# uthree/tinyvc

Measured on AMD Instinct MI355X. Metric: audio-samples/sec (16 kHz) end-to-end VC, higher is better.
Workload: dtype f32 (fp32 in / out / accumulate; channel contractions as two-term fp16 splits on v_mfma_f32_32x32x16_f16: 22-bit significands, three part-products per fp32 product)

## Files before the change

### include/tinyvc_hip.h

```cpp
#ifndef TINYVC_HIP_H
#define TINYVC_HIP_H

#include <stddef.h>
#include <stdint.h>

#ifdef __cplusplus
extern "C" {
#endif

typedef struct tvc_ctx tvc_ctx;

enum tvc_status {
    TVC_OK = 0,
    TVC_ERR_ARG = -1,
    TVC_ERR_HIP = -2,
    TVC_ERR_STATE = -3,
    TVC_ERR_WORKSPACE = -4
};

#define TVC_ABI_VERSION 1
int tvc_version(void);

int tvc_ctx_create(int hip_device, tvc_ctx** out);
void tvc_ctx_destroy(tvc_ctx* ctx);
const char* tvc_last_error(const tvc_ctx* ctx);

int tvc_load_tensor(tvc_ctx* ctx, const char* state_dict_key, const float* host_data,
                    const int64_t* shape, int ndim);
int tvc_set_pitch_table(tvc_ctx* ctx, const float* host_freqs, int n);
int tvc_finalize_weights(tvc_ctx* ctx);

int tvc_workspace_bytes(tvc_ctx* ctx, int B, int64_t L, int64_t N, size_t* out_bytes);

int tvc_stft_mag_f32(tvc_ctx* ctx, void* stream, const float* wav, float* spec, int B, int64_t L,
                     void* ws, size_t ws_bytes);
int tvc_energy_f32(tvc_ctx* ctx, void* stream, const float* wav, float* energy, int B, int64_t L,
                   void* ws, size_t ws_bytes);

int64_t tvc_resample_out_len(int64_t n, int orig_freq, int new_freq);
int tvc_resample_f32(tvc_ctx* ctx, void* stream, const float* x, float* y, int rows, int64_t n, int orig_freq,
                     int new_freq);
int tvc_pcm16_to_f32(tvc_ctx* ctx, void* stream, const int16_t* pcm, float* y, int64_t n, float gain_db);
int tvc_f32_to_pcm16(tvc_ctx* ctx, void* stream, const float* x, int16_t* pcm, int64_t n, float gain_db);

int tvc_encoder_f32(tvc_ctx* ctx, void* stream, const float* spec, float* ssl, float* f0,
                    float* logits, int B, int T, void* ws, size_t ws_bytes);

int tvc_pitch_decode_f32(tvc_ctx* ctx, void* stream, const float* logits, float* f0, int B, int T);

int64_t tvc_knn_prepared_elems(int64_t N);
int tvc_knn_prepare_index_f32(tvc_ctx* ctx, void* stream, const float* index, float* prepared,
                              int64_t N);
int64_t tvc_knn_prepared_elems_f16(int64_t N);
int tvc_knn_prepare_index_f16(tvc_ctx* ctx, void* stream, const void* rows_f16, float* prepared,
                              int64_t N);
int tvc_knn_prepare_index_cols_f32(tvc_ctx* ctx, void* stream, const float* feats, int64_t S, const int64_t* cols, int64_t N,
                                   float* prepared, float* index_out);
int tvc_knn_prepare_index_cols_f16(tvc_ctx* ctx, void* stream, const float* feats, int64_t S, const int64_t* cols, int64_t N,
                                   float* prepared, void* index_out_f16);

int tvc_knn_forget(tvc_ctx* ctx, const float* prepared);
int tvc_knn_match_f32(tvc_ctx* ctx, void* stream, const float* src, const float* prepared, int64_t N,
                      float* out, int64_t* idx_out, int B, int T, void* ws, size_t ws_bytes);

int tvc_knn_match_general_f32(tvc_ctx* ctx, void* stream, const float* src, const float* index, int64_t N, int k, int metric,
                              float* out, int64_t* idx_out, float* sim_out, int B, int T, void* ws, size_t ws_bytes);

int tvc_ctx_set_index_assign_chunk(tvc_ctx* ctx, int max_queries);
int tvc_workspace_bytes_index_compact(tvc_ctx* ctx, int64_t N, int64_t K, size_t* out_bytes);
int tvc_index_assign_f32(tvc_ctx* ctx, void* stream, const float* points_prepared, int64_t N, const float* centroids_prepared, int64_t K,
                         int64_t* assign_inout, float* sim_out, int32_t* moved_out, void* ws, size_t ws_bytes);
int tvc_index_update_f32(tvc_ctx* ctx, void* stream, const float* points_prepared, int64_t N, const int64_t* assign, int64_t K,
                         float* centroids_inout, int32_t* counts_out, void* ws, size_t ws_bytes);
int tvc_index_compact_f32(tvc_ctx* ctx, void* stream, const float* points_prepared, int64_t N, const int64_t* init_cols, int64_t K, int iters,
                          float* centroids_out, float* prepared_out, int64_t* assign_out, int32_t* counts_out, int32_t* moved_out, void* ws,
                          size_t ws_bytes);

int tvc_knn_topk_f32(tvc_ctx* ctx, void* stream, const float* src, const float* prepared, int64_t N,
                     float* sims_out, int64_t* idx_out, int B, int T, void* ws, size_t ws_bytes);
int tvc_knn_gather_slots_f32(tvc_ctx* ctx, void* stream, const float* prepared, int64_t N,
                             const int64_t* idx, float* slots, int64_t nslots);
int tvc_knn_finish_f32(tvc_ctx* ctx, void* stream, const float* slots, float* out, int B, int T);

int tvc_shift_frequency_f32(tvc_ctx* ctx, void* stream, const float* f0, float* out, int64_t n,
                            float semitones);

int tvc_noise_angle_from_uniform_f32(tvc_ctx* ctx, void* stream, float* u, int64_t n);

int tvc_decoder_f32(tvc_ctx* ctx, void* stream, const float* content, const float* f0,
                    const float* energy, const float* noise_angle, uint64_t seed, float* wave,
                    int B, int T, void* ws, size_t ws_bytes);
int tvc_decoder_stages_f32(tvc_ctx* ctx, void* stream, const float* content, const float* f0,
                           const float* energy, const float* noise_angle, uint64_t seed,
                           float* wave, float* amps, float* kernel, float* source, int B, int T,
                           void* ws, size_t ws_bytes);

int tvc_filter_net_f32(tvc_ctx* ctx, void* stream, const float* content, const float* f0, const float* energy,
                       const float* source, float* wave, float* const* skips, float* const* ups, int B, int T,
                       void* ws, size_t ws_bytes);

int tvc_dsp_f32(tvc_ctx* ctx, void* stream, const float* f0, const float* amps, const float* kernel,
                const float* noise_angle, uint64_t seed, float* source, int B, int T, void* ws,
                size_t ws_bytes);

int tvc_convert_f32(tvc_ctx* ctx, void* stream, const float* wav, const float* prepared_index,
                    int64_t N, float pitch_shift, const float* noise_angle, uint64_t seed,
                    float* wave, int B, int64_t L, void* ws, size_t ws_bytes);

int tvc_workspace_bytes_ragged(tvc_ctx* ctx, int B, int64_t Lmax, const int64_t* lens, int64_t N, size_t* out_bytes);
int tvc_ragged_plan(int B, int64_t Lmax, const int64_t* lens, int max_frames, int32_t* batch_of_row, int* n_batches);
int tvc_ctx_set_ragged_batch_frames(tvc_ctx* ctx, int max_frames);
int tvc_convert_ragged_f32(tvc_ctx* ctx, void* stream, const float* wav, int64_t Lmax, const int64_t* lens, const float* prepared_index,
                           int64_t N, float pitch_shift, const float* noise_angle, uint64_t seed, float* wave, int B, void* ws,
                           size_t ws_bytes);

int tvc_workspace_bytes_encode_ragged(tvc_ctx* ctx, int B, int64_t Lmax, const int64_t* lens, size_t* out_bytes);
int tvc_encode_ragged_f32(tvc_ctx* ctx, void* stream, const float* wav, int64_t Lmax, const int64_t* lens, float* ssl, float* f0,
                          int B, void* ws, size_t ws_bytes);

int tvc_knn_match_multi_f32(tvc_ctx* ctx, void* stream, const float* src, const float* const* prepared, const int64_t* N,
                            float* out, int64_t* idx_out, int B, int T, void* ws, size_t ws_bytes);
int tvc_workspace_bytes_multi(tvc_ctx* ctx, int B, int64_t L, const int64_t* N, size_t* out_bytes);
int tvc_convert_multi_f32(tvc_ctx* ctx, void* stream, const float* wav, const float* const* prepared, const int64_t* N,
                          float pitch_shift, const float* pitch_shifts, const float* noise_angle, uint64_t seed, float* wave,
                          int B, int64_t L, void* ws, size_t ws_bytes);
int tvc_workspace_bytes_ragged_multi(tvc_ctx* ctx, int B, int64_t Lmax, const int64_t* lens, const int64_t* N, size_t* out_bytes);
int tvc_convert_ragged_multi_f32(tvc_ctx* ctx, void* stream, const float* wav, int64_t Lmax, const int64_t* lens,
                                 const float* const* prepared, const int64_t* N, float pitch_shift, const float* pitch_shifts,
                                 const float* noise_angle, uint64_t seed, float* wave, int B, void* ws, size_t ws_bytes);

#define TVC_BLEND_MAX 4
int tvc_knn_match_blend_f32(tvc_ctx* ctx, void* stream, const float* src, const float* const* prepared, const int64_t* N, int M,
                            const float* weights, float* out, int64_t* idx_out, int B, int T, void* ws, size_t ws_bytes);
int tvc_workspace_bytes_blend(tvc_ctx* ctx, int B, int64_t L, const int64_t* N, int M, size_t* out_bytes);
int tvc_convert_blend_f32(tvc_ctx* ctx, void* stream, const float* wav, const float* const* prepared, const int64_t* N, int M,
                          const float* weights, float pitch_shift, const float* pitch_shifts, const float* noise_angle, uint64_t seed,
                          float* wave, int B, int64_t L, void* ws, size_t ws_bytes);
int tvc_workspace_bytes_ragged_blend(tvc_ctx* ctx, int B, int64_t Lmax, const int64_t* lens, const int64_t* N, int M, size_t* out_bytes);
int tvc_convert_ragged_blend_f32(tvc_ctx* ctx, void* stream, const float* wav, int64_t Lmax, const int64_t* lens,
                                 const float* const* prepared, const int64_t* N, int M, const float* weights, float pitch_shift,
                                 const float* pitch_shifts, const float* noise_angle, uint64_t seed, float* wave, int B, void* ws,
                                 size_t ws_bytes);

int tvc_pitch_match_f32(tvc_ctx* ctx, void* stream, const float* f0, const int64_t* row_start, int rows, const float* target_f0,
                        float pitch_shift, const float* pitch_shifts, float* median_out, int32_t* voiced_out, float* shift_out,
                        float* f0_shifted);
int tvc_workspace_bytes_auto(tvc_ctx* ctx, int B, int64_t L, const int64_t* N, int M, size_t* out_bytes);
int tvc_convert_auto_f32(tvc_ctx* ctx, void* stream, const float* wav, const float* const* prepared, const int64_t* N, int M,
                         const float* weights, const float* target_f0, float pitch_shift, const float* pitch_shifts, float* shift_out,
                         const float* noise_angle, uint64_t seed, float* wave, int B, int64_t L, void* ws, size_t ws_bytes);
int tvc_workspace_bytes_ragged_auto(tvc_ctx* ctx, int B, int64_t Lmax, const int64_t* lens, const int64_t* N, int M, size_t* out_bytes);
int tvc_convert_ragged_auto_f32(tvc_ctx* ctx, void* stream, const float* wav, int64_t Lmax, const int64_t* lens,
                                const float* const* prepared, const int64_t* N, int M, const float* weights, const float* target_f0,
                                float pitch_shift, const float* pitch_shifts, float* shift_out, const float* noise_angle, uint64_t seed,
                                float* wave, int B, void* ws, size_t ws_bytes);

int tvc_sola_f32(tvc_ctx* ctx, void* stream, const float* y, float* sola_buf, const float* fade_in,
                 float* out, int32_t* shift_out, int S, int64_t Ly, int block,
                 int use_phase_vocoder);

int tvc_stream_push_f32(tvc_ctx* ctx, void* stream, float* buf, const float* blocks, int S, int64_t n, int block);

int tvc_profile_enable(tvc_ctx* ctx, int on);
int tvc_profile_read(tvc_ctx* ctx, char* buf, size_t buf_bytes);

#ifdef __cplusplus
}
#endif
#endif
```

### tinyvc_amd/_lib.py

```python
import ctypes
import os
from ctypes import POINTER, c_char_p, c_float, c_int, c_int32, c_int64, c_size_t, c_uint64, c_void_p

_HERE = os.path.dirname(os.path.abspath(__file__))
LIB_PATH = os.environ.get("TVC_LIB_PATH") or os.path.join(_HERE, "libtinyvc_hip.so")

_lib = None

SIGNATURES = {
    "tvc_version": (c_int, []),
    "tvc_ctx_create": (c_int, [c_int, POINTER(c_void_p)]),
    "tvc_ctx_destroy": (None, [c_void_p]),
    "tvc_last_error": (c_char_p, [c_void_p]),
    "tvc_load_tensor": (c_int, [c_void_p, c_char_p, c_void_p, POINTER(c_int64), c_int]),
    "tvc_set_pitch_table": (c_int, [c_void_p, c_void_p, c_int]),
    "tvc_finalize_weights": (c_int, [c_void_p]),
    "tvc_workspace_bytes": (c_int, [c_void_p, c_int, c_int64, c_int64, POINTER(c_size_t)]),
    "tvc_stft_mag_f32": (c_int, [c_void_p, c_void_p, c_void_p, c_void_p, c_int, c_int64, c_void_p, c_size_t]),
    "tvc_energy_f32": (c_int, [c_void_p, c_void_p, c_void_p, c_void_p, c_int, c_int64, c_void_p, c_size_t]),
    "tvc_resample_out_len": (c_int64, [c_int64, c_int, c_int]),
    "tvc_resample_f32": (c_int, [c_void_p, c_void_p, c_void_p, c_void_p, c_int, c_int64, c_int, c_int]),
    "tvc_pcm16_to_f32": (c_int, [c_void_p, c_void_p, c_void_p, c_void_p, c_int64, c_float]),
    "tvc_f32_to_pcm16": (c_int, [c_void_p, c_void_p, c_void_p, c_void_p, c_int64, c_float]),
    "tvc_encoder_f32": (c_int, [c_void_p, c_void_p, c_void_p, c_void_p, c_void_p, c_void_p, c_int, c_int, c_void_p, c_size_t]),
    "tvc_pitch_decode_f32": (c_int, [c_void_p, c_void_p, c_void_p, c_void_p, c_int, c_int]),
    "tvc_knn_prepared_elems": (c_int64, [c_int64]),
    "tvc_knn_prepared_elems_f16": (c_int64, [c_int64]),
    "tvc_knn_prepare_index_f16": (c_int, [c_void_p, c_void_p, c_void_p, c_void_p, c_int64]),
    "tvc_knn_prepare_index_cols_f32": (c_int, [c_void_p, c_void_p, c_void_p, c_int64, c_void_p, c_int64, c_void_p, c_void_p]),
    "tvc_knn_prepare_index_cols_f16": (c_int, [c_void_p, c_void_p, c_void_p, c_int64, c_void_p, c_int64, c_void_p, c_void_p]),
    "tvc_knn_forget": (c_int, [c_void_p, c_void_p]),
    "tvc_ragged_plan": (c_int, [c_int, c_int64, POINTER(c_int64), c_int, POINTER(c_int32), POINTER(c_int)]),
    "tvc_ctx_set_ragged_batch_frames": (c_int, [c_void_p, c_int]),
    "tvc_knn_prepare_index_f32": (c_int, [c_void_p, c_void_p, c_void_p, c_void_p, c_int64]),
    "tvc_knn_match_f32": (c_int, [c_void_p, c_void_p, c_void_p, c_void_p, c_int64, c_void_p, c_void_p, c_int, c_int, c_void_p, c_size_t]),
    "tvc_knn_match_general_f32": (c_int, [c_void_p, c_void_p, c_void_p, c_void_p, c_int64, c_int, c_int, c_void_p, c_void_p, c_void_p, c_int, c_int, c_void_p, c_size_t]),
    "tvc_knn_topk_f32": (c_int, [c_void_p, c_void_p, c_void_p, c_void_p, c_int64, c_void_p, c_void_p, c_int, c_int, c_void_p, c_size_t]),
    "tvc_knn_gather_slots_f32": (c_int, [c_void_p, c_void_p, c_void_p, c_int64, c_void_p, c_void_p, c_int64]),
    "tvc_knn_finish_f32": (c_int, [c_void_p, c_void_p, c_void_p, c_void_p, c_int, c_int]),
    "tvc_shift_frequency_f32": (c_int, [c_void_p, c_void_p, c_void_p, c_void_p, c_int64, c_float]),
    "tvc_noise_angle_from_uniform_f32": (c_int, [c_void_p, c_void_p, c_void_p, c_int64]),
    "tvc_decoder_f32": (c_int, [c_void_p, c_void_p, c_void_p, c_void_p, c_void_p, c_void_p, c_uint64, c_void_p, c_int, c_int, c_void_p, c_size_t]),
    "tvc_decoder_stages_f32": (c_int, [c_void_p, c_void_p, c_void_p, c_void_p, c_void_p, c_void_p, c_uint64, c_void_p, c_void_p, c_void_p, c_void_p, c_int, c_int, c_void_p, c_size_t]),
    "tvc_filter_net_f32": (c_int, [c_void_p, c_void_p, c_void_p, c_void_p, c_void_p, c_void_p, c_void_p, POINTER(c_void_p), POINTER(c_void_p), c_int, c_int, c_void_p, c_size_t]),
    "tvc_dsp_f32": (c_int, [c_void_p, c_void_p, c_void_p, c_void_p, c_void_p, c_void_p, c_uint64, c_void_p, c_int, c_int, c_void_p, c_size_t]),
    "tvc_convert_f32": (c_int, [c_void_p, c_void_p, c_void_p, c_void_p, c_int64, c_float, c_void_p, c_uint64, c_void_p, c_int, c_int64, c_void_p, c_size_t]),
    "tvc_workspace_bytes_ragged": (c_int, [c_void_p, c_int, c_int64, POINTER(c_int64), c_int64, POINTER(c_size_t)]),
    "tvc_convert_ragged_f32": (c_int, [c_void_p, c_void_p, c_void_p, c_int64, POINTER(c_int64), c_void_p, c_int64, c_float, c_void_p, c_uint64, c_void_p, c_int, c_void_p, c_size_t]),
    "tvc_workspace_bytes_encode_ragged": (c_int, [c_void_p, c_int, c_int64, POINTER(c_int64), POINTER(c_size_t)]),
    "tvc_encode_ragged_f32": (c_int, [c_void_p, c_void_p, c_void_p, c_int64, POINTER(c_int64), c_void_p, c_void_p, c_int, c_void_p, c_size_t]),
    "tvc_knn_match_multi_f32": (c_int, [c_void_p, c_void_p, c_void_p, POINTER(c_void_p), POINTER(c_int64), c_void_p, c_void_p, c_int, c_int, c_void_p, c_size_t]),
    "tvc_workspace_bytes_multi": (c_int, [c_void_p, c_int, c_int64, POINTER(c_int64), POINTER(c_size_t)]),
    "tvc_convert_multi_f32": (c_int, [c_void_p, c_void_p, c_void_p, POINTER(c_void_p), POINTER(c_int64), c_float, POINTER(c_float), c_void_p, c_uint64,
                                      c_void_p, c_int, c_int64, c_void_p, c_size_t]),
    "tvc_workspace_bytes_ragged_multi": (c_int, [c_void_p, c_int, c_int64, POINTER(c_int64), POINTER(c_int64), POINTER(c_size_t)]),
    "tvc_convert_ragged_multi_f32": (c_int, [c_void_p, c_void_p, c_void_p, c_int64, POINTER(c_int64), POINTER(c_void_p), POINTER(c_int64), c_float,
                                             POINTER(c_float), c_void_p, c_uint64, c_void_p, c_int, c_void_p, c_size_t]),
    "tvc_knn_match_blend_f32": (c_int, [c_void_p, c_void_p, c_void_p, POINTER(c_void_p), POINTER(c_int64), c_int, c_void_p, c_void_p, c_void_p, c_int, c_int,
                                        c_void_p, c_size_t]),
    "tvc_workspace_bytes_blend": (c_int, [c_void_p, c_int, c_int64, POINTER(c_int64), c_int, POINTER(c_size_t)]),
    "tvc_convert_blend_f32": (c_int, [c_void_p, c_void_p, c_void_p, POINTER(c_void_p), POINTER(c_int64), c_int, c_void_p, c_float, POINTER(c_float), c_void_p,
                                      c_uint64, c_void_p, c_int, c_int64, c_void_p, c_size_t]),
    "tvc_workspace_bytes_ragged_blend": (c_int, [c_void_p, c_int, c_int64, POINTER(c_int64), POINTER(c_int64), c_int, POINTER(c_size_t)]),
    "tvc_convert_ragged_blend_f32": (c_int, [c_void_p, c_void_p, c_void_p, c_int64, POINTER(c_int64), POINTER(c_void_p), POINTER(c_int64), c_int, c_void_p,
                                             c_float, POINTER(c_float), c_void_p, c_uint64, c_void_p, c_int, c_void_p, c_size_t]),
    "tvc_pitch_match_f32": (c_int, [c_void_p, c_void_p, c_void_p, POINTER(c_int64), c_int, c_void_p, c_float, POINTER(c_float), c_void_p, c_void_p, c_void_p,
                                    c_void_p]),
    "tvc_workspace_bytes_auto": (c_int, [c_void_p, c_int, c_int64, POINTER(c_int64), c_int, POINTER(c_size_t)]),
    "tvc_convert_auto_f32": (c_int, [c_void_p, c_void_p, c_void_p, POINTER(c_void_p), POINTER(c_int64), c_int, c_void_p, c_void_p, c_float, POINTER(c_float),
                                     c_void_p, c_void_p, c_uint64, c_void_p, c_int, c_int64, c_void_p, c_size_t]),
    "tvc_workspace_bytes_ragged_auto": (c_int, [c_void_p, c_int, c_int64, POINTER(c_int64), POINTER(c_int64), c_int, POINTER(c_size_t)]),
    "tvc_convert_ragged_auto_f32": (c_int, [c_void_p, c_void_p, c_void_p, c_int64, POINTER(c_int64), POINTER(c_void_p), POINTER(c_int64), c_int, c_void_p,
                                            c_void_p, c_float, POINTER(c_float), c_void_p, c_void_p, c_uint64, c_void_p, c_int, c_void_p, c_size_t]),
    "tvc_ctx_set_index_assign_chunk": (c_int, [c_void_p, c_int]),
    "tvc_workspace_bytes_index_compact": (c_int, [c_void_p, c_int64, c_int64, POINTER(c_size_t)]),
    "tvc_index_assign_f32": (c_int, [c_void_p, c_void_p, c_void_p, c_int64, c_void_p, c_int64, c_void_p, c_void_p, c_void_p, c_void_p, c_size_t]),
    "tvc_index_update_f32": (c_int, [c_void_p, c_void_p, c_void_p, c_int64, c_void_p, c_int64, c_void_p, c_void_p, c_void_p, c_size_t]),
    "tvc_index_compact_f32": (c_int, [c_void_p, c_void_p, c_void_p, c_int64, c_void_p, c_int64, c_int, c_void_p, c_void_p, c_void_p, c_void_p, c_void_p,
                                      c_void_p, c_size_t]),
    "tvc_sola_f32": (c_int, [c_void_p, c_void_p, c_void_p, c_void_p, c_void_p, c_void_p, c_void_p, c_int, c_int64, c_int, c_int]),
    "tvc_stream_push_f32": (c_int, [c_void_p, c_void_p, c_void_p, c_void_p, c_int, c_int64, c_int]),
    "tvc_profile_enable": (c_int, [c_void_p, c_int]),
    "tvc_profile_read": (c_int, [c_void_p, ctypes.c_char_p, c_size_t]),
}


class TinyVCError(RuntimeError):
    pass


def load_library():
    global _lib
    if _lib is not None:
        return _lib
    import torch
    if not os.path.exists(LIB_PATH):
        raise TinyVCError(
            f"{LIB_PATH} is missing: build it with `python -m tinyvc_amd.build` (needs hipcc). "
            "tinyvc_amd has no CPU or eager-PyTorch fallback.")
    lib = ctypes.CDLL(LIB_PATH)
    for name, (res, args) in SIGNATURES.items():
        fn = getattr(lib, name)
        fn.restype = res
        fn.argtypes = args
    _lib = lib
    return lib
```

### tinyvc_amd/csrc/api.hip

```cpp
#include <atomic>
#include <cmath>
#include <mutex>

#include <cstdlib>

#include "knn_blob.h"
#include "tvc_common.h"

using namespace tvc;

static std::mutex g_blob_mu;
static std::map<const void*, int64_t> g_blobs;
constexpr size_t kMaxBlobRecords = 4096;
static void blob_record(const void* p, int64_t N) {
    std::lock_guard<std::mutex> lk(g_blob_mu);
    if (g_blobs.size() >= kMaxBlobRecords && !g_blobs.count(p)) g_blobs.clear();
    g_blobs[p] = N;
}
static void blob_forget(const void* p) {
    std::lock_guard<std::mutex> lk(g_blob_mu);
    g_blobs.erase(p);
}
static int blob_check(tvc_ctx* ctx, hipStream_t s, const void* p, int64_t N, const char* what) {
    {
// ... 562 lines not shown
    return convert_query(ctx, B, Lmax, lens, true, ConvertIndex::one(nullptr, N), out_bytes, "tvc_workspace_bytes_ragged");
}
int tvc_workspace_bytes_multi(tvc_ctx* ctx, int B, int64_t L, const int64_t* N, size_t* out_bytes) {
    return convert_query(ctx, B, L, nullptr, false, ConvertIndex::table(nullptr, N), out_bytes, "tvc_workspace_bytes_multi");
}
int tvc_workspace_bytes_ragged_multi(tvc_ctx* ctx, int B, int64_t Lmax, const int64_t* lens, const int64_t* N, size_t* out_bytes) {
    return convert_query(ctx, B, Lmax, lens, true, ConvertIndex::table(nullptr, N), out_bytes, "tvc_workspace_bytes_ragged_multi");
}

int tvc_convert_f32(tvc_ctx* ctx, void* stream, const float* wav, const float* prepared, int64_t N,
                    float pitch_shift, const float* noise_angle, uint64_t seed, float* wave, int B, int64_t L,
                    void* wsp, size_t ws_bytes) {
    const ConvertCall c{wav, wave, B, L, nullptr, ConvertIndex::one(prepared, N), pitch_shift, nullptr, noise_angle, seed};
    return convert_entry(ctx, stream, c, false, wsp, ws_bytes, "tvc_convert_f32");
}
int tvc_convert_ragged_f32(tvc_ctx* ctx, void* stream, const float* wav, int64_t Lmax, const int64_t* lens, const float* prepared, int64_t N,
                           float pitch_shift, const float* noise_angle, uint64_t seed, float* wave, int B, void* wsp, size_t ws_bytes) {
    const ConvertCall c{wav, wave, B, Lmax, lens, ConvertIndex::one(prepared, N), pitch_shift, nullptr, noise_angle, seed};
    return convert_entry(ctx, stream, c, true, wsp, ws_bytes, "tvc_convert_ragged_f32");
}
int tvc_convert_multi_f32(tvc_ctx* ctx, void* stream, const float* wav, const float* const* prepared, const int64_t* N, float pitch_shift,
                          const float* pitch_shifts, const float* noise_angle, uint64_t seed, float* wave, int B, int64_t L, void* wsp, size_t ws_bytes) {
    const ConvertCall c{wav, wave, B, L, nullptr, ConvertIndex::table(prepared, N), pitch_shift, pitch_shifts, noise_angle, seed};
    return convert_entry(ctx, stream, c, false, wsp, ws_bytes, "tvc_convert_multi_f32");
}
int tvc_convert_ragged_multi_f32(tvc_ctx* ctx, void* stream, const float* wav, int64_t Lmax, const int64_t* lens, const float* const* prepared,
                                 const int64_t* N, float pitch_shift, const float* pitch_shifts, const float* noise_angle, uint64_t seed, float* wave,
                                 int B, void* wsp, size_t ws_bytes) {
    const ConvertCall c{wav, wave, B, Lmax, lens, ConvertIndex::table(prepared, N), pitch_shift, pitch_shifts, noise_angle, seed};
    return convert_entry(ctx, stream, c, true, wsp, ws_bytes, "tvc_convert_ragged_multi_f32");
}

int tvc_knn_match_multi_f32(tvc_ctx* ctx, void* stream, const float* src, const float* const* prepared, const int64_t* N, float* out,
                            int64_t* idx_out, int B, int T, void* wsp, size_t ws_bytes) {
    if (!ctx) return TVC_ERR_ARG;
    if (!src || !out || B <= 0 || T <= 0 || (int64_t)B * T > 0x7fffffff) return fail(ctx, TVC_ERR_ARG, "tvc_knn_match_multi_f32: bad argument");
    hipStream_t s = (hipStream_t)stream;
    TVC_CHECK(rows_check(ctx, s, B, prepared, N, "tvc_knn_match_multi_f32"));
    TVC_HIP(ctx, hipSetDevice(ctx->device));
    std::vector<KnnSegIn> in((size_t)B);
    for (int b = 0; b < B; ++b) in[b] = KnnSegIn{prepared[b], N[b], b * T, T};
    return run_walks(ctx, __func__, wsp, ws_bytes, 1, [&](Ws& ws) { return run_knn_segs(ctx, s, ws, src, in.data(), B, out, idx_out, B, T); });
}

int tvc_workspace_bytes_blend(tvc_ctx* ctx, int B, int64_t L, const int64_t* N, int M, size_t* out_bytes) {
    if (!ctx) return TVC_ERR_ARG;
    TVC_CHECK(blend_check(ctx, B, M, kDryPtr, "tvc_workspace_bytes_blend"));
    return convert_query(ctx, B, L, nullptr, false, ConvertIndex::blend(nullptr, N, M, nullptr), out_bytes, "tvc_workspace_bytes_blend");
}
int tvc_workspace_bytes_ragged_blend(tvc_ctx* ctx, int B, int64_t Lmax, const int64_t* lens, const int64_t* N, int M, size_t* out_bytes) {
    if (!ctx) return TVC_ERR_ARG;
    TVC_CHECK(blend_check(ctx, B, M, kDryPtr, "tvc_workspace_bytes_ragged_blend"));
    return convert_query(ctx, B, Lmax, lens, true, ConvertIndex::blend(nullptr, N, M, nullptr), out_bytes, "tvc_workspace_bytes_ragged_blend");
}
int tvc_convert_blend_f32(tvc_ctx* ctx, void* stream, const float* wav, const float* const* prepared, const int64_t* N, int M, const float* weights,
                          float pitch_shift, const float* pitch_shifts, const float* noise_angle, uint64_t seed, float* wave, int B, int64_t L, void* wsp,
                          size_t ws_bytes) {
    if (!ctx) return TVC_ERR_ARG;
    TVC_CHECK(blend_check(ctx, B, M, weights, "tvc_convert_blend_f32"));
    const ConvertCall c{wav, wave, B, L, nullptr, ConvertIndex::blend(prepared, N, M, weights), pitch_shift, pitch_shifts, noise_angle, seed};
    return convert_entry(ctx, stream, c, false, wsp, ws_bytes, "tvc_convert_blend_f32");
}
int tvc_convert_ragged_blend_f32(tvc_ctx* ctx, void* stream, const float* wav, int64_t Lmax, const int64_t* lens, const float* const* prepared,
                                 const int64_t* N, int M, const float* weights, float pitch_shift, const float* pitch_shifts, const float* noise_angle,
                                 uint64_t seed, float* wave, int B, void* wsp, size_t ws_bytes) {
    if (!ctx) return TVC_ERR_ARG;
    TVC_CHECK(blend_check(ctx, B, M, weights, "tvc_convert_ragged_blend_f32"));
    const ConvertCall c{wav, wave, B, Lmax, lens, ConvertIndex::blend(prepared, N, M, weights), pitch_shift, pitch_shifts, noise_angle, seed};
    return convert_entry(ctx, stream, c, true, wsp, ws_bytes, "tvc_convert_ragged_blend_f32");
}

int tvc_pitch_match_f32(tvc_ctx* ctx, void* stream, const float* f0, const int64_t* row_start, int rows, const float* target_f0, float pitch_shift,
                        const float* pitch_shifts, float* median_out, int32_t* voiced_out, float* shift_out, float* f0_shifted) {
    if (!ctx) return TVC_ERR_ARG;
    if (!f0 || !row_start || rows <= 0 || (!median_out && !voiced_out && !shift_out && !f0_shifted)) return fail(ctx, TVC_ERR_ARG, "tvc_pitch_match_f32: bad argument");
    if (row_start[0] < 0 || row_start[rows] > 0x7fffffff) return fail(ctx, TVC_ERR_ARG, "tvc_pitch_match_f32: row_start beyond 32-bit indexing");
    std::vector<PitchRow> pr((size_t)rows);
    for (int b = 0; b < rows; ++b) {
        if (row_start[b + 1] < row_start[b]) return fail(ctx, TVC_ERR_ARG, "tvc_pitch_match_f32: row_start[%d] > row_start[%d] (rows + 1 ascending column numbers)", b, b + 1);
        pr[b] = PitchRow{(int)row_start[b], (int)(row_start[b + 1] - row_start[b]), b, pitch_shifts ? pitch_shifts[b] : pitch_shift};
    }
    TVC_HIP(ctx, hipSetDevice(ctx->device));
    return run_pitch_match(ctx, (hipStream_t)stream, f0, pr, target_f0, median_out, voiced_out, shift_out, f0_shifted);
}

static int auto_index(tvc_ctx* ctx, int B, const float* const* prepared, const int64_t* N, int M, const float* weights, ConvertIndex* ix, const char* what) {
    if (!ctx) return TVC_ERR_ARG;
    if (!weights) {
        if (M != 1) return fail(ctx, TVC_ERR_ARG, "%s: weights = NULL is one index per row: M must be 1, got %d", what, M);
        *ix = ConvertIndex::table(prepared, N);
        return 0;
    }
    TVC_CHECK(blend_check(ctx, B, M, weights, what));
    *ix = ConvertIndex::blend(prepared, N, M, weights);
    return 0;
}
static int auto_query(tvc_ctx* ctx, int B, int64_t L, const int64_t* lens, bool ragged, const int64_t* N, int M, size_t* out_bytes, const char* what) {
    if (!ctx) return TVC_ERR_ARG;
    TVC_CHECK(blend_check(ctx, B, M, kDryPtr, what));
    TVC_CHECK(convert_query(ctx, B, L, lens, ragged, ConvertIndex::blend(nullptr, N, M, nullptr), out_bytes, what, true));
    if (M == 1) {
        size_t table = 0;
        TVC_CHECK(convert_query(ctx, B, L, lens, ragged, ConvertIndex::table(nullptr, N), &table, what, true));
        if (table > *out_bytes) *out_bytes = table;
    }
    return TVC_OK;
}
int tvc_workspace_bytes_auto(tvc_ctx* ctx, int B, int64_t L, const int64_t* N, int M, size_t* out_bytes) {
    return auto_query(ctx, B, L, nullptr, false, N, M, out_bytes, "tvc_workspace_bytes_auto");
}
int tvc_workspace_bytes_ragged_auto(tvc_ctx* ctx, int B, int64_t Lmax, const int64_t* lens, const int64_t* N, int M, size_t* out_bytes) {
    return auto_query(ctx, B, Lmax, lens, true, N, M, out_bytes, "tvc_workspace_bytes_ragged_auto");
}
int tvc_convert_auto_f32(tvc_ctx* ctx, void* stream, const float* wav, const float* const* prepared, const int64_t* N, int M, const float* weights,
                         const float* target_f0, float pitch_shift, const float* pitch_shifts, float* shift_out, const float* noise_angle, uint64_t seed,
                         float* wave, int B, int64_t L, void* wsp, size_t ws_bytes) {
    ConvertIndex ix;
    TVC_CHECK(auto_index(ctx, B, prepared, N, M, weights, &ix, "tvc_convert_auto_f32"));
    if (!target_f0) return fail(ctx, TVC_ERR_ARG, "tvc_convert_auto_f32: target_f0 is NULL (a device array of B registers in Hz)");
    const ConvertCall c{wav, wave, B, L, nullptr, ix, pitch_shift, pitch_shifts, noise_angle, seed, target_f0, shift_out};
    return convert_entry(ctx, stream, c, false, wsp, ws_bytes, "tvc_convert_auto_f32");
}
int tvc_convert_ragged_auto_f32(tvc_ctx* ctx, void* stream, const float* wav, int64_t Lmax, const int64_t* lens, const float* const* prepared,
                                const int64_t* N, int M, const float* weights, const float* target_f0, float pitch_shift, const float* pitch_shifts,
                                float* shift_out, const float* noise_angle, uint64_t seed, float* wave, int B, void* wsp, size_t ws_bytes) {
    ConvertIndex ix;
    TVC_CHECK(auto_index(ctx, B, prepared, N, M, weights, &ix, "tvc_convert_ragged_auto_f32"));
    if (!target_f0) return fail(ctx, TVC_ERR_ARG, "tvc_convert_ragged_auto_f32: target_f0 is NULL (a device array of B registers in Hz)");
    const ConvertCall c{wav, wave, B, Lmax, lens, ix, pitch_shift, pitch_shifts, noise_angle, seed, target_f0, shift_out};
    return convert_entry(ctx, stream, c, true, wsp, ws_bytes, "tvc_convert_ragged_auto_f32");
}

int tvc_knn_match_blend_f32(tvc_ctx* ctx, void* stream, const float* src, const float* const* prepared, const int64_t* N, int M, const float* weights,
                            float* out, int64_t* idx_out, int B, int T, void* wsp, size_t ws_bytes) {
    if (!ctx) return TVC_ERR_ARG;
    if (!src || !out || B <= 0 || T <= 0) return fail(ctx, TVC_ERR_ARG, "tvc_knn_match_blend_f32: bad argument");
    TVC_CHECK(blend_check(ctx, B, M, weights, "tvc_knn_match_blend_f32"));
    if ((int64_t)B * M * T > 0x7fffffff) return fail(ctx, TVC_ERR_ARG, "tvc_knn_match_blend_f32: more than 2^31 - 1 query columns");
    hipStream_t s = (hipStream_t)stream;
    TVC_CHECK(rows_check(ctx, s, B * M, prepared, N, "tvc_knn_match_blend_f32"));
    TVC_HIP(ctx, hipSetDevice(ctx->device));
    std::vector<KnnSegIn> in;
    for (int m = 0; m < M; ++m)
        for (int b = 0; b < B; ++b) in.push_back(KnnSegIn{prepared[(size_t)b * M + m], N[(size_t)b * M + m], (m * B + b) * T, T});
    return run_walks(ctx, __func__, wsp, ws_bytes, 1, [&](Ws& ws) { return run_knn_blend(ctx, s, ws, src, in.data(), (int)in.size(), M, weights, out, idx_out, B, T); });
}

int tvc_ctx_set_ragged_batch_frames(tvc_ctx* ctx, int max_frames) {
    if (!ctx) return TVC_ERR_ARG;
    if (max_frames < 0) return fail(ctx, TVC_ERR_ARG, "tvc_ctx_set_ragged_batch_frames: the cap is a frame count (0 = the default)");
    ctx->rag_batch_frames = max_frames;
    return TVC_OK;
}
int tvc_ragged_plan(int B, int64_t Lmax, const int64_t* lens, int max_frames, int32_t* batch_of_row, int* n_batches) {
    if (!lens || !batch_of_row || !n_batches || B <= 0 || Lmax <= 0 || Lmax % kHop != 0 || max_frames < 0) return TVC_ERR_ARG;
    std::vector<RagBatchPlan> batches;
    const int rc = ragged_split(nullptr, max_frames, B, Lmax, lens, &batches);
    if (rc) return rc;
    for (size_t i = 0; i < batches.size(); ++i)
        for (int b : batches[i].rows) batch_of_row[b] = (int32_t)i;
    *n_batches = (int)batches.size();
    return TVC_OK;
}

int tvc_workspace_bytes_encode_ragged(tvc_ctx* ctx, int B, int64_t Lmax, const int64_t* lens, size_t* out_bytes) {
    TVC_CHECK(need_ready(ctx, NEED_NONE));
    if (!out_bytes || !lens || B <= 0 || Lmax <= 0 || Lmax % kHop != 0) return fail(ctx, TVC_ERR_ARG, "tvc_workspace_bytes_encode_ragged: need B>0, Lmax%%480==0, lens[B]");
    std::vector<RagBatchPlan> batches;
    std::vector<int> gpre;
    int64_t S = 0;
    TVC_CHECK(encode_ragged_plan(ctx, B, Lmax, lens, &batches, &gpre, &S));
    return measure(kRagGranule, out_bytes, [&](Ws& ws) { return encode_ragged_batches(ctx, nullptr, ws, batches, gpre, kDryPtr, Lmax, kDryPtr, kDryPtr, S); });
}

int tvc_encode_ragged_f32(tvc_ctx* ctx, void* stream, const float* wav, int64_t Lmax, const int64_t* lens, float* ssl, float* f0, int B, void* wsp,
                          size_t ws_bytes) {
    TVC_CHECK(need_ready(ctx, NEED_ENC));
    if (!wav || !lens || !ssl || !f0 || B <= 0 || Lmax <= 0 || Lmax % kHop) return fail(ctx, TVC_ERR_ARG, "tvc_encode_ragged_f32: bad argument (Lmax must be a positive multiple of 480)");
    TVC_HIP(ctx, hipSetDevice(ctx->device));
    hipStream_t s = (hipStream_t)stream;
    std::vector<RagBatchPlan> batches;
    std::vector<int> gpre;
    int64_t S = 0;
    TVC_CHECK(encode_ragged_plan(ctx, B, Lmax, lens, &batches, &gpre, &S));
    return run_walks(ctx, __func__, wsp, ws_bytes, kRagGranule, [&](Ws& ws) { return encode_ragged_batches(ctx, s, ws, batches, gpre, wav, Lmax, ssl, f0, S); });
}

static int compact_check(tvc_ctx* ctx, int64_t N, int64_t K, const char* what) {
    if (K < 4 || K > N) return fail(ctx, TVC_ERR_ARG, "%s: need 4 <= K <= N (K = %lld, N = %lld)", what, (long long)K, (long long)N);
    if (K > kIndexCompactMaxK) return fail(ctx, TVC_ERR_ARG, "%s: K = %lld is above the limit of %lld centroids", what, (long long)K, (long long)kIndexCompactMaxK);
    if (N > 0x7fffff00L) return fail(ctx, TVC_ERR_ARG, "%s: N beyond 32-bit indexing", what);
    return 0;
}

int tvc_ctx_set_index_assign_chunk(tvc_ctx* ctx, int max_queries) {
    if (!ctx) return TVC_ERR_ARG;
    if (max_queries < 0) return fail(ctx, TVC_ERR_ARG, "tvc_ctx_set_index_assign_chunk: the chunk is a count of query columns (0 = the default)");
    ctx->index_assign_chunk = max_queries;
    return TVC_OK;
}

int tvc_workspace_bytes_index_compact(tvc_ctx* ctx, int64_t N, int64_t K, size_t* out_bytes) {
    if (!ctx) return TVC_ERR_ARG;
    if (!out_bytes) return fail(ctx, TVC_ERR_ARG, "tvc_workspace_bytes_index_compact: out_bytes is NULL");
    TVC_CHECK(compact_check(ctx, N, K, "tvc_workspace_bytes_index_compact"));
    return measure(1, out_bytes, [&](Ws& ws) { return run_index_compact(ctx, nullptr, ws, kDryPtr, N, nullptr, K, 1, kDryPtr, kDryPtr, nullptr, nullptr, nullptr); });
}

int tvc_index_assign_f32(tvc_ctx* ctx, void* stream, const float* points_prepared, int64_t N, const float* centroids_prepared, int64_t K,
                         int64_t* assign_inout, float* sim_out, int32_t* moved_out, void* wsp, size_t ws_bytes) {
    if (!ctx) return TVC_ERR_ARG;
    if (!points_prepared || !centroids_prepared || !assign_inout) return fail(ctx, TVC_ERR_ARG, "tvc_index_assign_f32: bad argument");
    TVC_CHECK(compact_check(ctx, N, K, "tvc_index_assign_f32"));
    hipStream_t s = (hipStream_t)stream;
    TVC_CHECK(blob_check(ctx, s, points_prepared, N, "tvc_index_assign_f32 (points)"));
    TVC_CHECK(blob_check(ctx, s, centroids_prepared, K, "tvc_index_assign_f32 (centroids)"));
    TVC_HIP(ctx, hipSetDevice(ctx->device));
    return run_walks(ctx, __func__, wsp, ws_bytes, 1, [&](Ws& ws) { return run_index_assign(ctx, s, ws, points_prepared, N, centroids_prepared, K, assign_inout, sim_out, moved_out); });
}

int tvc_index_update_f32(tvc_ctx* ctx, void* stream, const float* points_prepared, int64_t N, const int64_t* assign, int64_t K, float* centroids_inout,
                         int32_t* counts_out, void* wsp, size_t ws_bytes) {
    if (!ctx) return TVC_ERR_ARG;
    if (!points_prepared || !assign || !centroids_inout) return fail(ctx, TVC_ERR_ARG, "tvc_index_update_f32: bad argument");
    TVC_CHECK(compact_check(ctx, N, K, "tvc_index_update_f32"));
    hipStream_t s = (hipStream_t)stream;
    TVC_CHECK(blob_check(ctx, s, points_prepared, N, "tvc_index_update_f32"));
    TVC_HIP(ctx, hipSetDevice(ctx->device));
    return run_walks(ctx, __func__, wsp, ws_bytes, 1, [&](Ws& ws) { return run_index_update(ctx, s, ws, points_prepared, N, assign, K, centroids_inout, counts_out); });
}

int tvc_index_compact_f32(tvc_ctx* ctx, void* stream, const float* points_prepared, int64_t N, const int64_t* init_cols, int64_t K, int iters,
                          float* centroids_out, float* prepared_out, int64_t* assign_out, int32_t* counts_out, int32_t* moved_out, void* wsp, size_t ws_bytes) {
    if (!ctx) return TVC_ERR_ARG;
    if (!points_prepared || !init_cols || !centroids_out || !prepared_out || iters < 1) return fail(ctx, TVC_ERR_ARG, "tvc_index_compact_f32: bad argument (iters >= 1)");
    TVC_CHECK(compact_check(ctx, N, K, "tvc_index_compact_f32"));
    hipStream_t s = (hipStream_t)stream;
    TVC_CHECK(blob_check(ctx, s, points_prepared, N, "tvc_index_compact_f32"));
    TVC_HIP(ctx, hipSetDevice(ctx->device));
    blob_forget(prepared_out);
    TVC_CHECK(run_walks(ctx, __func__, wsp, ws_bytes, 1, [&](Ws& ws) {
        return run_index_compact(ctx, s, ws, points_prepared, N, init_cols, K, iters, centroids_out, prepared_out, assign_out, counts_out, moved_out);
    }));
    blob_record(prepared_out, K);
    return TVC_OK;
}

int tvc_profile_enable(tvc_ctx* ctx, int on) {
    if (!ctx) return TVC_ERR_ARG;
    ctx->profiling = on < 0 ? 0 : (on > 2 ? 1 : on);
    return TVC_OK;
}

int tvc_profile_read(tvc_ctx* ctx, char* buf, size_t buf_bytes) {
    if (!ctx || !buf || buf_bytes < 2) return TVC_ERR_ARG;
    std::vector<std::pair<std::string, double>> agg;
    for (auto& r : ctx->regions) {
        float ms = 0.f;
        if (r.a && r.b && hipEventSynchronize(r.b) == hipSuccess && hipEventElapsedTime(&ms, r.a, r.b) == hipSuccess) {
            bool found = false;
            for (auto& a : agg)
                if (a.first == r.name) {
                    a.second += ms;
                    found = true;
                }
            if (!found) agg.push_back({r.name, ms});
        }
        if (r.a) ctx->event_pool.push_back(r.a);
        if (r.b) ctx->event_pool.push_back(r.b);
    }
    ctx->regions.clear();
    std::string out;
    for (auto& a : agg) {
        char tmp[160];
        snprintf(tmp, sizeof(tmp), "%s=%.6f;", a.first.c_str(), a.second);
        out += tmp;
    }
    snprintf(buf, buf_bytes, "%s", out.c_str());
    return TVC_OK;
}

int tvc_sola_f32(tvc_ctx* ctx, void* stream, const float* y, float* sola_buf, const float* fade_in, float* out,
                 int32_t* shift_out, int S, int64_t Ly, int block, int use_phase_vocoder) {
    if (!ctx) return TVC_ERR_ARG;
    if (!y || !sola_buf || !fade_in || !out || S <= 0 || block <= 0 || Ly < block + kSolaCross + kSolaSearch + kSolaDelay)
        return fail(ctx, TVC_ERR_ARG, "tvc_sola_f32: bad argument (Ly must cover block+1920+1920+3840)");
    TVC_HIP(ctx, hipSetDevice(ctx->device));
    return run_sola(ctx, (hipStream_t)stream, y, sola_buf, fade_in, out, shift_out, S, Ly, block, use_phase_vocoder);
}

int tvc_stream_push_f32(tvc_ctx* ctx, void* stream, float* buf, const float* blocks, int S, int64_t n, int block) {
    if (!ctx) return TVC_ERR_ARG;
    if (!buf || !blocks || S <= 0 || block <= 0 || n < block || n > INT32_MAX - 32768)
        return fail(ctx, TVC_ERR_ARG, "tvc_stream_push_f32: bad argument (block <= n <= 2^31 - 32769)");
    TVC_HIP(ctx, hipSetDevice(ctx->device));
    return run_stream_push(ctx, (hipStream_t)stream, buf, blocks, S, (int)n, block);
}

}
```

### tinyvc_amd/csrc/cnx_s3.h

```cpp
#pragma once
#include "gemm_epi.h"
#include "split_fp16.h"

namespace tvc {

struct CnxArgs {
    float* x;
    float* h;
    int T, rs;
    RagDev rg;
    const uint4* A6;
    const float* wsc;
    const float* bias;
    int MT, mt_per_wg;
    const float *dw_w, *dw_b, *ln_g, *ln_b;
    int dil;
    float* gp;
    int gp_tiles;
    int gp_sum;
    const float* grn_g;
    float* amax_y;
};

constexpr int CNX_GP_INLINE = 16;
constexpr int CNX_PD = 4;
typedef float f32x4s_t __attribute__((ext_vector_type(4)));

struct CnxNoPost {
    __device__ __forceinline__ void operator()(int) const {}
};
template <int NT, int NC, int KSL, class Post = CnxNoPost>
__device__ __forceinline__ void cnx_mma(f32x16 (&hi)[NT], f32x16 (&lo)[NT], u32x4 (&ring)[CNX_PD][2], const uint4* __restrict__ A6, int MT, int mt, int k_begin,
                                        int mt_next, int k_next, const uint4* Ys, int lane, const Post& post = Post()) {
    static_assert(KSL % CNX_PD == 0, "ring depth divides the K walk");
    const int l31 = lane & 31, lh = lane >> 5;
    const uint4* yb = Ys + lh * NC + l31;
    u32x4 bq[2][NT][2];
#pragma unroll
    for (int j = 0; j < NT; ++j)
#pragma unroll
        for (int p = 0; p < 2; ++p) bq[0][j][p] = *reinterpret_cast<const u32x4*>(yb + (p * 2) * NC + j * 32);
#pragma unroll
    for (int k0 = 0; k0 < KSL; k0 += CNX_PD) {
#pragma unroll
        for (int u = 0; u < CNX_PD; ++u) {
            const int k = k0 + u, fb = u & 1;
            const f16x8 a0 = __builtin_bit_cast(f16x8, ring[u][0]), a1 = __builtin_bit_cast(f16x8, ring[u][1]);
            int kn = k + CNX_PD, mtl = mt, kg = k_begin;
            if (kn >= KSL) {
                kn -= KSL;
                mtl = mt_next;
                kg = k_next;
            }
            const uint4* ab = A6 + ((long)(kg + kn) * MT + mtl) * kPU4;
            ring[u][0] = ldg_so4(ab, 16u * (unsigned)lane);
            ring[u][1] = ldg_so4(ab, 16u * (unsigned)(64 + lane));
            const int kb = k + 1 < KSL ? k + 1 : 0;
#pragma unroll
            for (int j = 0; j < NT; ++j)
#pragma unroll
                for (int p = 0; p < 2; ++p) bq[fb ^ 1][j][p] = *reinterpret_cast<const u32x4*>(yb + ((kb * 2 + p) * 2) * NC + j * 32);
#pragma unroll
            for (int j = 0; j < NT; ++j) lo[j] = TVC_MFMA16(a1, __builtin_bit_cast(f16x8, bq[fb][j][0]), lo[j]);
#pragma unroll
            for (int j = 0; j < NT; ++j) hi[j] = TVC_MFMA16(a0, __builtin_bit_cast(f16x8, bq[fb][j][0]), hi[j]);
#pragma unroll
            for (int j = 0; j < NT; ++j) lo[j] = TVC_MFMA16(a0, __builtin_bit_cast(f16x8, bq[fb][j][1]), lo[j]);
            post(k);
            __builtin_amdgcn_sched_barrier(0);
        }
    }
}

template <int C, int NT>
struct Cnx1 {
    static constexpr int WAVES = 8, NTHR = WAVES * 64, NC = 32 * NT, KS = C / 16, CPT = C / 16, VW = NT;
    static constexpr int YS_U4 = KS * 4 * NC;
    static constexpr int LDS_BYTES = YS_U4 * 16 + (C * 8 + 2 * C + 16 * NC) * 4;
    static_assert(LDS_BYTES <= 160 * 1024, "LDS");
};

template <int C, int NT>
__global__ __launch_bounds__((Cnx1<C, NT>::NTHR)) void cnx1_kernel(CnxArgs a) {
    using CF = Cnx1<C, NT>;
    constexpr int NC = CF::NC, KS = CF::KS, CPT = CF::CPT, VW = CF::VW, WAVES = CF::WAVES, NTHR = CF::NTHR;
    extern __shared__ __attribute__((aligned(16))) uint4 smem_c1[];
    uint4* Ys = smem_c1;
    float* scr = reinterpret_cast<float*>(smem_c1);
    float* Wl = reinterpret_cast<float*>(smem_c1 + CF::YS_U4);
    float* Gl = Wl + C * 8;
    float* red = Gl + 2 * C;
    const int tid = threadIdx.x, lane = tid & 63, l31 = lane & 31, lh = lane >> 5;
    const int wave = __builtin_amdgcn_readfirstlane(tid >> 6);
    const int b = blockIdx.y;
    int Tb = a.T;
    long xoff = (long)b * C * a.T, hoff = (long)b * 2 * C * a.T;
    if (a.rg.tb) {
        Tb = a.rg.tb[b];
        xoff = hoff = a.rg.pre[b];
    }
    const int ntu = (Tb + NC - 1) / NC;
    if ((int)blockIdx.x >= ntu) return;
    const int TW = (Tb + ntu - 1) / ntu;
    const int t0 = blockIdx.x * TW;
    const int tw = Tb - t0 < TW ? Tb - t0 : TW;
    const int rs = a.rs;
    const float* xb = a.x + xoff;

    for (int i = tid; i < C; i += NTHR) {
#pragma unroll
        for (int j = 0; j < 7; ++j) Wl[i * 8 + j] = a.dw_w[i * 7 + j];
        Wl[i * 8 + 7] = a.dw_b[i];
        Gl[i] = a.ln_g[i];
        Gl[C + i] = a.ln_b[i];
    }
    __syncthreads();

    const int col = NT == 2 ? lane : l31;
    const int tc = t0 + (col < tw ? col : tw - 1);
    unsigned tt[7];
#pragma unroll
    for (int j = 0; j < 7; ++j) {
        int q = tc + (j - 3) * a.dil;
        q = q < 0 ? 0 : (q >= Tb ? Tb - 1 : q);
        tt[j] = 4u * (unsigned)q;
    }
    float v[VW][CPT];
#pragma unroll
    for (int u = 0; u < VW; ++u) {
        const int vw = NT == 2 ? wave + 8 * u : wave + 8 * lh;
        float sum = 0.f;
#pragma unroll
        for (int i = 0; i < CPT; ++i) {
            const int c = vw + i * 16;
            const f32x4s_t w0 = *reinterpret_cast<const f32x4s_t*>(Wl + c * 8), w1 = *reinterpret_cast<const f32x4s_t*>(Wl + c * 8 + 4);
            const float wj[7] = {w0[0], w0[1], w0[2], w0[3], w1[0], w1[1], w1[2]};
            float acc = w1[3];
            if (NT == 2) {
                const float* xr = xb + (long)c * rs;
#pragma unroll
                for (int j = 0; j < 7; ++j) acc = fmaf(wj[j], ldg_so(xr, tt[j]), acc);
            } else {
                const char* xr = reinterpret_cast<const char*>(xb + (long)c * rs);
#pragma unroll
                for (int j = 0; j < 7; ++j) acc = fmaf(wj[j], *reinterpret_cast<const float*>(xr + tt[j]), acc);
            }
            v[u][i] = acc;
            sum += acc;
            scr[c * NC + col] = acc;
        }
        red[vw * NC + col] = sum;
    }
    __syncthreads();
    float tot = 0.f;
#pragma unroll
    for (int w = 0; w < 16; ++w) tot += red[w * NC + col];
    const float mean = tot / (float)C;
    __syncthreads();
#pragma unroll
    for (int u = 0; u < VW; ++u) {
        const int vw = NT == 2 ? wave + 8 * u : wave + 8 * lh;
        float sq = 0.f;
#pragma unroll
        for (int i = 0; i < CPT; ++i) {
            const float d = v[u][i] - mean;
            sq = fmaf(d, d, sq);
        }
        red[vw * NC + col] = sq;
    }
    __syncthreads();
    float tot2 = 0.f;
#pragma unroll
    for (int w = 0; w < 16; ++w) tot2 += red[w * NC + col];
    const float var = tot2 / (float)C;
    const float rstd = 1.f / sqrtf(var + 1e-5f);

    for (int i = wave; i < KS; i += WAVES) {
        constexpr int NQ = NT == 2 ? 16 : 8;
        const int c0 = 16 * i + (NT == 2 ? 0 : 8 * lh);
        float y[NQ];
#pragma unroll
        for (int q = 0; q < NQ; ++q) y[q] = scr[(c0 + q) * NC + col];
#pragma unroll
        for (int q = 0; q < NQ; ++q) y[q] = fmaf((y[q] - mean) * rstd, Gl[c0 + q], Gl[C + c0 + q]);
#pragma unroll
        for (int hh = 0; hh < NQ / 8; ++hh) {
            const float y8[8] = {y[8 * hh], y[8 * hh + 1], y[8 * hh + 2], y[8 * hh + 3], y[8 * hh + 4], y[8 * hh + 5], y[8 * hh + 6], y[8 * hh + 7]};
            uint4 p1, p2;
            split8(y8, p1, p2);
            const int half = NT == 2 ? hh : lh;
            Ys[((i * 2 + 0) * 2 + half) * NC + col] = p1;
            Ys[((i * 2 + 1) * 2 + half) * NC + col] = p2;
        }
    }
    __syncthreads();

    const int mt_lo = blockIdx.z * a.mt_per_wg;
    const int mt_hi = mt_lo + a.mt_per_wg < a.MT ? mt_lo + a.mt_per_wg : a.MT;
    int mt = mt_lo + wave;
    if (mt >= mt_hi) return;
    u32x4 ring[CNX_PD][2];
#pragma unroll
    for (int u = 0; u < CNX_PD; ++u) {
        const uint4* ab = a.A6 + ((long)u * a.MT + mt) * kPU4;
        ring[u][0] = ldg_so4(ab, 16u * (unsigned)lane);
        ring[u][1] = ldg_so4(ab, 16u * (unsigned)(64 + lane));
    }
    float* hb = a.h + hoff;
    constexpr int NPEND = NT * 16, EPS = ((NPEND + KS - 1) / KS + 1) / 2 * 2;
    float pend[NPEND];
    int pmt = mt;
    unsigned oo[NT];
#pragma unroll
    for (int j = 0; j < NT; ++j) {
        const int n = j * 32 + l31;
        oo[j] = 4u * (unsigned)(4 * lh * rs + t0 + (n < tw ? n : tw - 1));
    }
    bool live[NT];
#pragma unroll
    for (int j = 0; j < NT; ++j) live[j] = j * 32 + l31 < tw;
    float sq[16];
    float* gpb = a.gp + ((long)b * a.gp_tiles + blockIdx.x) * (2 * C) + ((l31 >> 1) & 3) + 8 * (l31 >> 3) + 4 * lh;
    auto finish2 = [&](int e) __attribute__((always_inline)) {
        const int j = e >> 4;
        f32x2e v = {pend[e], pend[e + 1]};
        asm volatile("" : "+v"(v));
        const f32x2e o = gelu_pair(v);
#pragma unroll
        for (int i = 0; i < 2; ++i) {
            const int r = (e + i) & 15;
            stg_so(hb + (long)(pmt * 32 + (r & 3) + 8 * (r >> 2)) * rs, oo[j], o[i]);
            if (j == 0) sq[r] = live[0] ? o[i] * o[i] : 0.f;
            else sq[r] = live[j] ? fmaf(o[i], o[i], sq[r]) : sq[r];
        }
        if (e == NPEND - 2) {
            const bool b4 = l31 & 16, b3 = l31 & 8, b2 = l31 & 4, b1 = l31 & 2;
            float w8[8], w4[4], w2[2];
#pragma unroll
            for (int i = 0; i < 8; ++i) w8[i] = (b4 ? sq[i + 8] : sq[i]) + __shfl_xor(b4 ? sq[i] : sq[i + 8], 16);
#pragma unroll
            for (int i = 0; i < 4; ++i) w4[i] = (b3 ? w8[i + 4] : w8[i]) + __shfl_xor(b3 ? w8[i] : w8[i + 4], 8);
#pragma unroll
            for (int i = 0; i < 2; ++i) w2[i] = (b2 ? w4[i + 2] : w4[i]) + __shfl_xor(b2 ? w4[i] : w4[i + 2], 4);
            float w1 = (b1 ? w2[1] : w2[0]) + __shfl_xor(b1 ? w2[0] : w2[1], 2);
            w1 += __shfl_xor(w1, 1);
            gpb[pmt * 32] = w1;
        }
    };
    auto post = [&](int k) __attribute__((always_inline)) {
#pragma unroll
        for (int e = EPS * k; e < EPS * k + EPS; e += 2)
            if (e < NPEND) finish2(e);
    };
    auto walk = [&](auto& poster) __attribute__((always_inline)) {
        const int mtn = mt + WAVES < mt_hi ? mt + WAVES : mt;
        float bv[16];
#pragma unroll
        for (int r = 0; r < 16; ++r) bv[r] = a.bias[mt * 32 + (r & 3) + 8 * (r >> 2) + 4 * lh];
        f32x16 hi[NT], lo[NT];
#pragma unroll
        for (int j = 0; j < NT; ++j)
#pragma unroll
            for (int r = 0; r < 16; ++r) hi[j][r] = lo[j][r] = 0.f;
        cnx_mma<NT, NC, KS>(hi, lo, ring, a.A6, a.MT, mt, 0, mtn, 0, Ys, lane, poster);
        const float cw = a.wsc[mt] * 1.f, cl = cw * kLoInv;
#pragma unroll
        for (int j = 0; j < NT; ++j)
#pragma unroll
            for (int r = 0; r < 16; ++r) pend[j * 16 + r] = comb(hi[j][r], lo[j][r], cw, cl) + bv[r];
        pmt = mt;
    };
    {
        CnxNoPost none;
        walk(none);
    }
    while (mt + WAVES < mt_hi) {
        mt += WAVES;
        walk(post);
    }
#pragma unroll
    for (int e = 0; e < NPEND; e += 2) finish2(e);
}

template <int C, int KPASS>
struct Cnx2 {
    static constexpr int K = 2 * C, NT = 2, NC = 64, KSL = K / 16 / KPASS;
    static constexpr int WAVES = KPASS == 2 ? C / 32 : 8, NTHR = WAVES * 64;
    static constexpr int YS_U4 = KSL * 4 * NC;
    static constexpr int GPP = K / 8 / KPASS;
    static constexpr int ITEMS = GPP * NC, XPER = (ITEMS + NTHR - 1) / NTHR;
    static constexpr int LDS_BYTES = YS_U4 * 16 + (K + 32) * 4;
    static_assert(ITEMS % NTHR == 0, "staging items divide");
    static_assert(LDS_BYTES <= 160 * 1024, "LDS");
};

template <int C, int KPASS>
__global__ __launch_bounds__((Cnx2<C, KPASS>::NTHR)) void cnx2_kernel(CnxArgs a) {
    using CF = Cnx2<C, KPASS>;
    constexpr int K = CF::K, NT = CF::NT, NC = CF::NC, KSL = CF::KSL, WAVES = CF::WAVES, XPER = CF::XPER;
    extern __shared__ __attribute__((aligned(16))) uint4 smem_c2[];
    uint4* Ys = smem_c2;
    float* Fl = reinterpret_cast<float*>(smem_c2 + CF::YS_U4);
    float* red = Fl + K;
    const int tid = threadIdx.x, lane = tid & 63;
    const int wave = __builtin_amdgcn_readfirstlane(tid >> 6);
    const int b = blockIdx.y;
    int Tb = a.T;
    long xoff = (long)b * C * a.T, hoff = (long)b * K * a.T;
    if (a.rg.tb) {
        Tb = a.rg.tb[b];
        xoff = hoff = a.rg.pre[b];
    }
    const int ntu = (Tb + NC - 1) / NC;
    if ((int)blockIdx.x >= ntu) return;
    const int TW = (Tb + ntu - 1) / ntu;
    const int t0 = blockIdx.x * TW;
    const int tw = Tb - t0 < TW ? Tb - t0 : TW;
    const int rs = a.rs;

    const float* g = a.gp + (long)b * a.gp_tiles * K;
    const int gtiles = a.gp_sum ? 1 : ntu;
    constexpr int GPT = K / 256;
    float gv[GPT], gm[GPT];
    if (tid < 256) {
#pragma unroll
        for (int i = 0; i < GPT; ++i) {
            float ss = g[tid + 256 * i];
            for (int t = 1; t < gtiles; ++t) ss += g[(long)t * K + tid + 256 * i];
            gv[i] = ss;
            gm[i] = a.grn_g[tid + 256 * i];
        }
    }
    const float* hb = a.h + hoff;
    const int scol = lane;
    const unsigned so = 4u * (unsigned)(t0 + (scol < tw ? scol : tw - 1));
    float xr[XPER][8];
    Bfp sx{1.f, 1.f};
    auto fetch = [&](int pass) __attribute__((always_inline)) {
#pragma unroll
        for (int i = 0; i < XPER; ++i) {
            const int gg = pass * CF::GPP + wave + i * WAVES;
#pragma unroll
            for (int q = 0; q < 8; ++q) xr[i][q] = ldg_so(hb + (long)(8 * gg + q) * rs, so);
        }
    };
    auto deposit = [&](int pass) __attribute__((always_inline)) {
#pragma unroll
        for (int i = 0; i < XPER; ++i) {
            const int gl = wave + i * WAVES, gg = pass * CF::GPP + gl;
            const f32x4s_t k0 = *reinterpret_cast<const f32x4s_t*>(Fl + 8 * gg), k1 = *reinterpret_cast<const f32x4s_t*>(Fl + 8 * gg + 4);
            xr[i][0] *= k0[0]; xr[i][1] *= k0[1]; xr[i][2] *= k0[2]; xr[i][3] *= k0[3];
            xr[i][4] *= k1[0]; xr[i][5] *= k1[1]; xr[i][6] *= k1[2]; xr[i][7] *= k1[3];
#pragma unroll
            for (int q = 0; q < 8; ++q) xr[i][q] *= sx.s;
            uint4 p1, p2;
            split8(xr[i], p1, p2);
            Ys[(((gl >> 1) * 2 + 0) * 2 + (gl & 1)) * NC + scol] = p1;
            Ys[(((gl >> 1) * 2 + 1) * 2 + (gl & 1)) * NC + scol] = p2;
        }
    };
    fetch(0);
    if (tid < 256) {
        float s = 0.f;
#pragma unroll
        for (int i = 0; i < GPT; ++i) gv[i] = sqrtf(gv[i]);
#pragma unroll
        for (int i = 0; i < GPT; ++i) s += gv[i];
#pragma unroll
        for (int o = 32; o > 0; o >>= 1) s += __shfl_xor(s, o);
        if (lane == 0) red[wave] = s;
    }
    slab_barrier();
    const float mean = (red[0] + red[1] + red[2] + red[3]) / (float)K;
    const float den = mean + 1e-6f;
    if (tid < 256) {
        float mx = 0.f;
#pragma unroll
        for (int i = 0; i < GPT; ++i) {
            const float f = fmaf(gm[i], gv[i] / den, 1.f);
            Fl[tid + 256 * i] = f;
            mx = fmaxf(mx, gv[i] * fabsf(f));
        }
#pragma unroll
        for (int o = 32; o > 0; o >>= 1) mx = fmaxf(mx, __shfl_xor(mx, o));
        if (lane == 0) red[4 + wave] = mx;
    }
    slab_barrier();
    sx = bfp_from_amax(fmaxf(fmaxf(red[4], red[5]), fmaxf(red[6], red[7])));
    sx.s = __builtin_bit_cast(float, __builtin_amdgcn_readfirstlane(__builtin_bit_cast(int, sx.s)));
    sx.inv = __builtin_bit_cast(float, __builtin_amdgcn_readfirstlane(__builtin_bit_cast(int, sx.inv)));
    deposit(0);
    if (KPASS == 2) fetch(1);
    slab_barrier();

    const int mt_lo = blockIdx.z * a.mt_per_wg;
    const int mt_hi = mt_lo + a.mt_per_wg < a.MT ? mt_lo + a.mt_per_wg : a.MT;
    int mt = mt_lo + wave;
    const bool has = mt < mt_hi;
    if (!has) mt = mt_lo;
    u32x4 ring[CNX_PD][2];
#pragma unroll
    for (int u = 0; u < CNX_PD; ++u) {
        const uint4* ab = a.A6 + ((long)u * a.MT + mt) * kPU4;
        ring[u][0] = ldg_so4(ab, 16u * (unsigned)lane);
        ring[u][1] = ldg_so4(ab, 16u * (unsigned)(64 + lane));
    }
    float* xb = a.x + xoff;
    float mx_out = 0.f;
    bool work = has;
    while (KPASS == 2 || work) {
        const int mtn = (KPASS == 1 && mt + WAVES < mt_hi) ? mt + WAVES : mt;
        f32x16 hi[NT], lo[NT];
#pragma unroll
        for (int j = 0; j < NT; ++j)
#pragma unroll
            for (int r = 0; r < 16; ++r) hi[j][r] = lo[j][r] = 0.f;
        if (KPASS == 1) {
            cnx_mma<NT, NC, KSL>(hi, lo, ring, a.A6, a.MT, mt, 0, mtn, 0, Ys, lane);
        } else {
            if (has) cnx_mma<NT, NC, KSL>(hi, lo, ring, a.A6, a.MT, mt, 0, mt, KSL, Ys, lane);
            slab_barrier();
            deposit(1);
            slab_barrier();
            if (!has) break;
            cnx_mma<NT, NC, KSL>(hi, lo, ring, a.A6, a.MT, mt, KSL, mt, KSL, Ys, lane);
        }
        const float cw = a.wsc[mt] * sx.inv, cl = cw * kLoInv;
        int el = tid;
        asm volatile("" : "+v"(el));
        const int l31 = el & 31, lh = (el >> 5) & 1;
        float bv[16];
#pragma unroll
        for (int r = 0; r < 16; ++r) bv[r] = a.bias[mt * 32 + (r & 3) + 8 * (r >> 2) + 4 * lh];
#pragma unroll
        for (int j = 0; j < NT; ++j) {
            const int n = j * 32 + l31;
            const unsigned oo = 4u * (unsigned)(4 * lh * rs + t0 + (n < tw ? n : tw - 1));
            float res[16];
#pragma unroll
            for (int r = 0; r < 16; ++r) res[r] = ldg_so(xb + (long)(mt * 32 + (r & 3) + 8 * (r >> 2)) * rs, oo);
            float mx = 0.f;
#pragma unroll
            for (int r = 0; r < 16; ++r) {
                float o = comb(hi[j][r], lo[j][r], cw, cl) + bv[r];
                o += res[r];
                res[r] = o;
                mx = fmaxf(mx, fabsf(o));
            }
            if (n < tw) {
#pragma unroll
                for (int r = 0; r < 16; ++r) stg_so(xb + (long)(mt * 32 + (r & 3) + 8 * (r >> 2)) * rs, oo, res[r]);
                mx_out = fmaxf(mx_out, mx);
            }
        }
        if (KPASS == 2) break;
        work = mt + WAVES < mt_hi;
        mt += WAVES;
    }
    if (a.amax_y) amax_flush_wg(a.amax_y + b, mx_out, red + 8);
}

}
```

### tinyvc_amd/csrc/decoder.hip

```cpp
#include "conv3s.h"
#include "conv_s2.h"
#include "film_s2.h"
#include "gemm_s2.h"
#include "small_kernels.h"
#include "tvc_common.h"

namespace tvc {


__device__ __forceinline__ float div24k(float x) {
    const float r = 1.0f / 24000.0f;
    const float q0 = __fmul_rn(x, r);
    return fmaf(fmaf(-q0, 24000.0f, x), r, q0);
}

__device__ __forceinline__ double wave_incl_scan(double v, int lane) {
#pragma unroll
    for (int o = 1; o < 64; o <<= 1) {
        double u = __shfl_up(v, o);
        if (lane >= o) v += u;
    }
    return v;
}

static __global__ __launch_bounds__(256) void harm_frame_sum_kernel(const float* __restrict__ f0, double* __restrict__ csum,
                                                                    int T, float scale, RagDev rg) {
    const int b = blockIdx.y, lane = threadIdx.x & 63;
    const int t = 4 * blockIdx.x + (threadIdx.x >> 6);
    const int rs = T;
    long fbase = (long)b * T, cbase = (long)b * kHarm * T;
    if (rg.tb) {
        T = rg.tb[b];
        fbase = cbase = rg.pre[b];
        scale = __fdiv_rn((float)T, (float)(T * kHop));
    }
    if (t >= T) return;
    const float* f = f0 + fbase;
    double acc[kHarm];
#pragma unroll
    for (int m = 0; m < kHarm; ++m) acc[m] = 0.0;
    if (lane < kHop / 8) {
#pragma unroll
        for (int k = 0; k < 8; ++k) {
            Lerp c = lerp_coord(t * kHop + 8 * lane + k, scale, T);
            float fs = lerp_eval(c, f[c.i0], f[c.i1]);
#pragma unroll
            for (int m = 0; m < kHarm; ++m) acc[m] += (double)div24k(__fmul_rn(fs, (float)(m + 1)));
        }
    }
#pragma unroll
    for (int m = 0; m < kHarm; ++m) {
        double v = acc[m];
#pragma unroll
        for (int o = 32; o > 0; o >>= 1) v += __shfl_xor(v, o);
        if (lane == m) csum[cbase + (long)m * rs + t] = v;
    }
}

static __global__ __launch_bounds__(64) void harm_frame_scan_kernel(double* __restrict__ csum, int T, RagDev rg) {
    double* p = csum + ((long)blockIdx.y * kHarm + blockIdx.x) * T;
    if (rg.tb) {
        p = csum + (long)blockIdx.x * T + rg.pre[blockIdx.y];
        T = rg.tb[blockIdx.y];
    }
    const int lane = threadIdx.x;
    double carry = 0.0;
    for (int base = 0; base < T; base += 64) {
        int i = base + lane;
        double v = i < T ? p[i] : 0.0;
        double inc = wave_incl_scan(v, lane);
        if (i < T) p[i] = carry + (inc - v);
        carry += __shfl(inc, 63);
    }
}

static __global__ __launch_bounds__(256) void harm_synth_kernel(const float* __restrict__ f0, const float* __restrict__ amps,
                                                                const double* __restrict__ coff, float* __restrict__ source,
                                                                int T, float scale_size, float scale_amp, RagDev rg) {
    const int b = blockIdx.y, lane = threadIdx.x & 63;
    const int t = 4 * blockIdx.x + (threadIdx.x >> 6);
    const int rs = T;
    const long Ls = (long)T * kHop;
    long fbase = (long)b * T, abase = (long)b * kHarm * T, sbase = (long)b * 16 * Ls;
    if (rg.tb) {
        T = rg.tb[b];
        fbase = abase = rg.pre[b];
        sbase = (long)rg.pre[b] * kHop;
        scale_size = __fdiv_rn((float)T, (float)(T * kHop));
    }
    if (t >= T) return;
    const bool act = lane < kHop / 8;
    const float* f = f0 + fbase;
    const int p0 = t * kHop + 8 * (act ? lane : 0);
    float fs[8], uv[8];
    Lerp ca[8];
#pragma unroll
    for (int e = 0; e < 8; ++e) {
        const Lerp c = lerp_coord(p0 + e, scale_size, T);
        const float a0 = f[c.i0], a1 = f[c.i1];
        fs[e] = lerp_eval(c, a0, a1);
        uv[e] = lerp_eval(c, a0 > 20.f ? 1.f : 0.f, a1 > 20.f ? 1.f : 0.f);
        ca[e] = lerp_coord(p0 + e, scale_amp, T);
    }
    for (int m = 0; m < kHarm; ++m) {
        double d[8], sum = 0.0;
#pragma unroll
        for (int e = 0; e < 8; ++e) {
            d[e] = act ? (double)div24k(__fmul_rn(fs[e], (float)(m + 1))) : 0.0;
            sum += d[e];
        }
        const double inc = wave_incl_scan(sum, lane);
        double run = coff[abase + (long)m * rs + t] + (inc - sum);
        if (act) {
            const float* am = amps + abase + (long)m * rs;
            float o[8];
#pragma unroll
            for (int e = 0; e < 8; ++e) {
                run += d[e];
                const float I = (float)run;
                const float frac = I - floorf(I);
                const float theta = __fmul_rn(6.2831854820251465f, frac);
                const float hsin = __fmul_rn(sincos_small(theta).x, uv[e]);
                const float amp = lerp_eval(ca[e], am[ca[e].i0], am[ca[e].i1]);
                o[e] = __fmul_rn(hsin, amp);
            }
            float4* dst = reinterpret_cast<float4*>(source + sbase + (long)m * Ls + p0);
            dst[0] = make_float4(o[0], o[1], o[2], o[3]);
            dst[1] = make_float4(o[4], o[5], o[6], o[7]);
        }
    }
}

static __global__ __launch_bounds__(256) void noise_ola_kernel(const float* __restrict__ frames, float* __restrict__ source, int B, int T, float* __restrict__ smax, RagDev rg) {
    __shared__ float red[4];
    const long Ls = (long)T * kHop;
    const long b = blockIdx.y;
    long fbase = b * T, sbase = (b * 16 + 15) * Ls;
    if (rg.tb) {
        T = rg.tb[b];
        fbase = rg.pre[b];
        sbase = 15 * Ls + (long)rg.pre[b] * kHop;
    }
    const long L = (long)T * kHop;
    float mx = 0.f;
    for (long i = blockIdx.x * (long)blockDim.x + threadIdx.x; i < L; i += (long)gridDim.x * blockDim.x) {
        int p = (int)i;
        int q = p + kNfft / 2;
        int f_hi = q / kHop;
        if (f_hi > T) f_hi = T;
        int f_lo = (q - (kNfft - 1) + kHop - 1) / kHop;
        if (q - (kNfft - 1) <= 0) f_lo = 0;
        float s = 0.f;
        for (int f = f_lo > 1 ? f_lo : 1; f <= f_hi; ++f)
            s = __fadd_rn(s, frames[(fbase + (f - 1)) * kNfft + (q - f * kHop)]);
        const float v = s / (float)(f_hi - f_lo + 1);
        source[sbase + p] = v;
        mx = fmaxf(mx, fabsf(v));
    }
    amax_flush_wg(smax + b, mx, red);
}

static int run_source_net(tvc_ctx* ctx, hipStream_t s, Ws& ws, const float* content, const float* f0,
                          const float* energy, float* amps, float* kern, int B, int T, const float* cmax, float* xmax_zeroed, hipEvent_t amps_ready = nullptr) {
    const int ncols = B * T;
    float* ef = ws.get<float>((size_t)B * T);
    float* x = ws.get<float>((size_t)B * kSrcCh * T);
    const int NB = ctx->rag ? ctx->rag->B : B;
    float* xmax = xmax_zeroed ? xmax_zeroed : ws.get<float>((size_t)NB);
    if (!ws.dry) {
        hipLaunchKernelGGL(window_max_kernel, dim3(grid_for((long)ncols * 64)), dim3(256), 0, s, energy, ef, (long)B, T, kHop);
        EpiSumCond ep{x, ctx->src_content_in.bias, ef, f0, ctx->src_e_w, ctx->src_e_b, ctx->src_f_w, ctx->src_f_b, kSrcCh, T, ncols};
        int rc = 0;
        if (!gemm_s2_try(&rc, ctx, s, ctx->src_content_in, content, B, kSslDim, T, 0, ep, cmax)) rc = gemm_s_launch<2, 4, 2>(ctx, s, ctx->src_content_in, content, B, kSslDim, T, 0, ep, cmax);
        TVC_CHECK(rc);
    }
    if (!ws.dry && !xmax_zeroed) TVC_HIP(ctx, hipMemsetAsync(xmax, 0, (size_t)NB * sizeof(float), s));
    for (int i = 0; i < 3; ++i) TVC_CHECK(run_convnext(ctx, s, ws, ctx->src_mid[i], x, B, T, i == 2 ? xmax : nullptr));
    if (ws.dry) return 0;
    EpiBias<ACT_ELU1, false> ea{amps, ctx->src_to_amps.bias, nullptr, kHarm, T, ncols, (long)kHarm * T, 0};
    TVC_CHECK((gemm_s_launch<1, 4, 2>(ctx, s, ctx->src_to_amps, x, B, kSrcCh, T, 0, ea, xmax)));
    if (amps_ready) TVC_HIP(ctx, hipEventRecord(amps_ready, s));
    EpiBias<ACT_ELU1, false> ek{kern, ctx->src_to_kernel.bias, nullptr, kBins, T, ncols, (long)kBins * T, 0};
    TVC_CHECK((gemm_s_launch<2, 4, 2>(ctx, s, ctx->src_to_kernel, x, B, kSrcCh, T, 0, ek, xmax)));
    return launch_check(ctx, "source_net");
}

static int run_harm_sums(tvc_ctx* ctx, hipStream_t s, const float* f0, double* csum, int B, int T) {
    const long L = (long)T * kHop;
    const int NB = ctx->rag ? ctx->rag->B : B;
    const int Tg = ctx->rag ? ctx->rag->Tlong : T;
    RagDev rg;
    TVC_CHECK(rag_view(ctx, s, 1, 0, &rg, nullptr));
    const float scale_size = (float)T / (float)L;
    hipLaunchKernelGGL(harm_frame_sum_kernel, dim3((Tg + 3) / 4, NB), dim3(256), 0, s, f0, csum, T, scale_size, rg);
    hipLaunchKernelGGL(harm_frame_scan_kernel, dim3(kHarm, NB), dim3(64), 0, s, csum, T, rg);
    return launch_check(ctx, "harm_sums");
}

int run_dsp(tvc_ctx* ctx, hipStream_t s, Ws& ws, const float* f0, const float* amps, const float* kern, const float* angle, uint64_t seed, float* source, int B, int T,
            float* smax, double* csum, const DspFork* fk) {
    const long L = (long)T * kHop;
    if (!csum) csum = ws.get<double>((size_t)B * kHarm * T);
    float* frames = ws.get<float>((size_t)B * T * kNfft);
    const int NB = ctx->rag ? ctx->rag->B : B;
    const int Tg = ctx->rag ? ctx->rag->Tlong : T;
    float* smax_own = smax ? nullptr : ws.get<float>((size_t)NB);
    if (ws.dry) return 0;
    if (!smax) {
        smax = smax_own;
        TVC_HIP(ctx, hipMemsetAsync(smax, 0, (size_t)NB * sizeof(float), s));
    }
    RagDev rg;
    TVC_CHECK(rag_view(ctx, s, 1, 0, &rg, nullptr));
    const float scale_size = (float)T / (float)L;
    const float scale_amp = (float)(1.0 / (double)kHop);
    hipStream_t sh = s;
    if (fk) {
        sh = fk->side;
        TVC_HIP(ctx, hipStreamWaitEvent(sh, fk->amps_ready, 0));
    } else {
        TVC_CHECK(run_harm_sums(ctx, s, f0, csum, B, T));
    }
    hipLaunchKernelGGL(harm_synth_kernel, dim3((Tg + 3) / 4, NB), dim3(256), 0, sh, f0, amps, csum, source, T, scale_size, scale_amp, rg);
    TVC_CHECK(run_amax_rows(ctx, sh, amps, B, kHarm, T, smax));
    TVC_CHECK(run_noise_ifft(ctx, s, kern, angle, seed, frames, B, T, ctx->rag && angle));
    hipLaunchKernelGGL(noise_ola_kernel, dim3(grid_for((long)Tg * kHop / 4, 256, NB >= 32 ? 16 : 512 / NB), NB), dim3(256), 0, s, frames, source, B, T, smax, rg);
    return launch_check(ctx, "dsp");
}

static int plain_conv(tvc_ctx* ctx, hipStream_t s, const PackedW& w, const float* x, int B, int Cin, int len, int dil, float* y, const BfpSlots& bfp, int lin = 0,
                      float lscale = 0.f) {
    int rc = 0;
    if ((lin > 0 ? conv_s2_try<true>(&rc, ctx, s, w, x, B, Cin, len, dil, y, bfp, lin, lscale) : conv_s2_try<false>(&rc, ctx, s, w, x, B, Cin, len, dil, y, bfp)))
        return rc;
    if (lin > 0)
        return conv3s_launch<true, C3EpiBias<false>, false, true>(ctx, s, w, x, B, Cin, len, dil, C3EpiBias<false>{y, w.bias, nullptr, w.M, len}, bfp, nullptr, nullptr,
                                                                   nullptr, 0, lin, lscale);
    return conv3s_launch<true>(ctx, s, w, x, B, Cin, len, dil, C3EpiBias<false>{y, w.bias, nullptr, w.M, len}, bfp);
}

static int film_conv(tvc_ctx* ctx, hipStream_t s, const PackedW& w, const PackedW& fw, const FilmU& fu, const float* h, const float* cond, int B, int C, int len, int dil,
                     float* out, const float* bsc, const float* bsh, const float* res, int res_lin, float res_scale, const BfpSlots& bfp) {
    int rc = 0;
    if (rag_min_len(ctx, len) >= FS2::BN && film_s2_try(&rc, ctx, s, fu, h, cond, B, C, len, dil, out, res, res_lin, res_scale, bfp)) return rc;
    return conv3s_launch<true, C3EpiFilmFused, true>(ctx, s, w, h, B, C, len, dil, C3EpiFilmFused{out, w.bias, bsc, bsh, res, C, len, res_lin, res_scale}, bfp, &fw, &fw,
                                                     cond, C);
}

static int conv_film_half(tvc_ctx* ctx, hipStream_t s, const PackedW& ca, const PackedW& cb, const PackedW& fw, const FilmU& fu, const float* x, int lin, float lscale,
                          int da, int db, float* h, const float* cond, int B, int C, int len, float* out, const float* bsc, const float* bsh, const float* res,
                          int res_lin, float res_scale, const float* ma_in, float* mh, const float* mcond, float* mout) {
    const bool pre = rag_min_len(ctx, len) >= FS2::BN && fu.img && fu.C == C && fu.hb_w > 0.f && C % 96 == 0 && C <= 384 && ma_in && mcond && res && db >= 1 && db <= FS2::MAXD &&
                     (long)C * len * 4 < (1L << 32) && (res_lin <= 0 || (long)C * res_lin * 4 < (1L << 32));
    if (pre) {
        int rc = 0;
        const BfpSlots in{ma_in, nullptr, nullptr};
        const bool ok = lin > 0 ? conv_s2_try<true, true>(&rc, ctx, s, ca, x, B, C, len, da, h, in, lin, lscale, fu.hb_w, fu.hb_b)
                                : conv_s2_try<false, true>(&rc, ctx, s, ca, x, B, C, len, da, h, in, 0, 0.f, fu.hb_w, fu.hb_b);
        if (ok) {
            TVC_CHECK(rc);
            if (!film_s2_try(&rc, ctx, s, fu, h, cond, B, C, len, db, out, res, res_lin, res_scale, BfpSlots{ma_in, mcond, mout}, true, fu.hb_w, fu.hb_b))
                return fail(ctx, TVC_ERR_STATE, "filter_net: the FiLM conv refused the pre-split operand its producer wrote");
            return rc;
        }
    }
    TVC_CHECK(plain_conv(ctx, s, ca, x, B, C, len, da, h, BfpSlots{ma_in, nullptr, mh}, lin, lscale));
    return film_conv(ctx, s, cb, fw, fu, h, cond, B, C, len, db, out, bsc, bsh, res, res_lin, res_scale, BfpSlots{mh, mcond, mout});
}

static __global__ void g8_to_planar_kernel(const float* __restrict__ x, float* __restrict__ y, long B, long l, int C) {
    const long n = B * C * l;
    for (long i = blockIdx.x * (long)blockDim.x + threadIdx.x; i < n; i += (long)gridDim.x * blockDim.x) {
        const long t = i % l, bc = i / l, c = bc % C, b = bc / C;
        y[i] = x[((b * (C / 8) + c / 8) * l + t) * 8 + (c & 7)];
    }
}

static int filter_input_gemm(tvc_ctx* ctx, hipStream_t s, const float* content, const float* f0, float* x, int B, int T, const float* cmax) {
    EpiSumCond ep{x, ctx->flt_content_in.bias, nullptr, f0, nullptr, nullptr, ctx->flt_f_w, ctx->flt_f_b, 384, T, B * T};
    int rc = 0;
    if (!gemm_s2_try(&rc, ctx, s, ctx->flt_content_in, content, B, kSslDim, T, 0, ep, cmax)) rc = gemm_s_launch<2, 4, 2>(ctx, s, ctx->flt_content_in, content, B, kSslDim, T, 0, ep, cmax);
    return rc;
}

int run_filter(tvc_ctx* ctx, hipStream_t s, Ws& ws, const float* content, const float* f0,
               const float* energy, const float* source, float* wave, int B, int T, const FilterTaps* taps, const float* cmax, const float* smax, float* zeroed_slots, bool x_slot_set,
               float* x_pre, bool x_pre_filled) {
    const long L = (long)T * kHop;
    static const int ch[5] = {384, 192, 96, 48, 24};
    const long len_dn[5] = {L, L / 5, L / 20, L / 80, L / 240};
    float* skip[5];
    for (int i = 0; i < 5; ++i) skip[i] = ws.get<float>((size_t)B * ch[4 - i] * len_dn[i]);
    float* x = x_pre ? x_pre : ws.get<float>((size_t)B * ch[0] * T);
    float* xi_pre[5] = {nullptr, nullptr, nullptr, nullptr, nullptr};
    for (int i = 1; i <= 4; ++i) xi_pre[i] = ws.get<float>((size_t)B * ctx->downs[i - 1].cin * len_dn[i]);
    for (int i = 1; i < 4; ++i)
        if (len_dn[i] % ctx->downs[i].factor != 0 || (ctx->downs[i].factor == 4 && len_dn[i] % 4 != 0))
            return fail(ctx, TVC_ERR_ARG, "filter_net: level lengths must divide by the next Downsample factor");

    enum { S_CONTENT = 0, S_SRC, S_X, S_SKIP0, S_DH1 = S_SKIP0 + 5, S_DH2 = S_DH1 + 4, S_UHA = S_DH2 + 4, S_UX1 = S_UHA + 5, S_UHB = S_UX1 + 5, S_UXU = S_UHB + 5,
           S_LEV = S_UXU + 5, S_COUNT = S_LEV + 5 };
    const int NB = ctx->rag ? ctx->rag->B : B;
    static_assert(S_COUNT == kFilterSlots && S_X == kFilterSlotX, "tvc_common.h kFilterSlots / kFilterSlotX");
    float* slots = zeroed_slots ? zeroed_slots : ws.get<float>((size_t)S_COUNT * NB);
    auto slot = [&](int i) { return slots + (size_t)i * NB; };

    if (!ws.dry) {
        ProfScope ps(ctx, s, ws, "filter.in+down0");
        if (!zeroed_slots) TVC_HIP(ctx, hipMemsetAsync(slots, 0, (size_t)S_COUNT * NB * sizeof(float), s));
        if (!cmax) {
            TVC_CHECK(run_amax_rows(ctx, s, content, B, kSslDim, T, slot(S_CONTENT)));
            cmax = slot(S_CONTENT);
        }
        if (!smax) {
            TVC_CHECK(run_amax_rows(ctx, s, source, B, 16, L, slot(S_SRC)));
            TVC_CHECK(run_amax_rows(ctx, s, energy, B, 1, L, slot(S_SRC)));
            smax = slot(S_SRC);
        }
        if (!x_pre_filled) TVC_CHECK(filter_input_gemm(ctx, s, content, f0, x, B, T, cmax));
        if (!(zeroed_slots && x_slot_set)) TVC_CHECK(run_slot_affine(ctx, s, slot(S_X), cmax, 1, ctx->flt_in_bw, ctx->flt_in_bb, NB));
        TVC_CHECK(run_down0_split(ctx, s, ctx->flt_down0s, source, energy, skip[0], taps ? taps->skips[0] : nullptr, xi_pre[1], B, (int)L, smax, slot(S_SKIP0)));
    }
    for (int i = 1; i <= 4; ++i) {
        const DownW& d = ctx->downs[i - 1];
        const int len = (int)len_dn[i];
        size_t mk = ws.mark();
        float* xi = xi_pre[i];
        float* h1 = d.cin == 24 ? nullptr : ws.get<float>((size_t)B * d.cin * len);
        float* h2 = d.cin == 24 ? nullptr : ws.get<float>((size_t)B * d.cin * len);
        if (!ws.dry) {
// ... 157 lines not shown
```

### tinyvc_amd/csrc/encoder.hip

```cpp
#include "conv3s.h"
#include "gemm_s2.h"
#include "cnx_s3.h"
#include "small_kernels.h"
#include "tvc_common.h"

namespace tvc {

constexpr int ENC_MTB = 4, ENC_NWV = 4, ENC_BPC = 2;

template <bool DW, int CPT>
static __global__ __launch_bounds__(1024) void dwconv_ln_kernel(const float* x, float* y,
                                                               const float* __restrict__ dw_w, const float* __restrict__ dw_b,
                                                               const float* __restrict__ g, const float* __restrict__ bta,
                                                               int C, int T, int dil, RagDev rg) {
    constexpr int NW = 16;
    const int rs = T;
    long ubase = (long)blockIdx.y * C * T;
    if (rg.tb) {
        T = rg.tb[blockIdx.y];
        ubase = rg.pre[blockIdx.y];
        if ((int)blockIdx.x * 64 >= T) return;
    }
    __shared__ float red[NW][64];
    constexpr bool STAGE = CPT >= 16;
    __shared__ __attribute__((aligned(16))) float Wl[STAGE ? 16 * CPT * 8 : 8];
    __shared__ float Gl[2][STAGE ? 16 * CPT : 1];
    if (STAGE) {
        for (int i = threadIdx.x; i < C; i += 1024) {
            if (DW) {
#pragma unroll
                for (int j = 0; j < 7; ++j) Wl[i * 8 + j] = dw_w[i * 7 + j];
                Wl[i * 8 + 7] = dw_b[i];
            }
            Gl[0][i] = g[i];
            Gl[1][i] = bta[i];
        }
        __syncthreads();
    }
    const int lane = threadIdx.x & 63, wave = threadIdx.x >> 6;
    const int t = blockIdx.x * 64 + lane;
    const bool ok = t < T;
    const int tc = ok ? t : T - 1;
    const float* xb = x + ubase;
    float* yb = y + ubase;

    int tt[7];
#pragma unroll
    for (int j = 0; j < 7; ++j) {
        int q = tc + (j - 3) * dil;
        tt[j] = q < 0 ? 0 : (q >= T ? T - 1 : q);
    }
    float v[CPT];
    float sum = 0.f;
#pragma unroll
    for (int i = 0; i < CPT; ++i) {
        const int c = wave + i * NW;
        if (DW) {
            const float* xr = xb + (long)c * rs;
            float wj[7], a;
            if (STAGE) {
                const float4 w0 = *reinterpret_cast<const float4*>(Wl + c * 8), w1 = *reinterpret_cast<const float4*>(Wl + c * 8 + 4);
                wj[0] = w0.x; wj[1] = w0.y; wj[2] = w0.z; wj[3] = w0.w; wj[4] = w1.x; wj[5] = w1.y; wj[6] = w1.z;
                a = w1.w;
            } else {
#pragma unroll
                for (int j = 0; j < 7; ++j) wj[j] = dw_w[c * 7 + j];
                a = dw_b[c];
            }
#pragma unroll
            for (int j = 0; j < 7; ++j) a = fmaf(wj[j], xr[tt[j]], a);
            v[i] = a;
        } else {
            v[i] = xb[(long)c * rs + tc];
        }
        sum += v[i];
    }
    red[wave][lane] = sum;
    __syncthreads();
    float tot = 0.f;
#pragma unroll
    for (int w = 0; w < NW; ++w) tot += red[w][lane];
    const float mean = tot / (float)C;
    __syncthreads();
    float sq = 0.f;
#pragma unroll
    for (int i = 0; i < CPT; ++i) {
        const float d = v[i] - mean;
        sq = fmaf(d, d, sq);
    }
    red[wave][lane] = sq;
    __syncthreads();
    float tot2 = 0.f;
#pragma unroll
    for (int w = 0; w < NW; ++w) tot2 += red[w][lane];
    const float var = tot2 / (float)C;
    const float rstd = 1.f / sqrtf(var + 1e-5f);
    if (!ok) return;
#pragma unroll
    for (int i = 0; i < CPT; ++i) {
        const int c = wave + i * NW;
        yb[(long)c * rs + t] = fmaf((v[i] - mean) * rstd, STAGE ? Gl[0][c] : g[c], STAGE ? Gl[1][c] : bta[c]);
    }
}
template <bool DW>
static int dwconv_ln_launch(tvc_ctx* ctx, hipStream_t s, const float* x, float* y, const float* dw_w, const float* dw_b, const float* g,
                            const float* bta, int B, int C, int T, int dil) {
    RagDev rg;
    TVC_CHECK(rag_view(ctx, s, 1, 0, &rg, nullptr));
    const dim3 grid(((ctx->rag ? ctx->rag->Tlong : T) + 63) / 64, ctx->rag ? ctx->rag->B : B), blk(1024);
    if (C == 384) hipLaunchKernelGGL((dwconv_ln_kernel<DW, 24>), grid, blk, 0, s, x, y, dw_w, dw_b, g, bta, C, T, dil, rg);
    else if (C == 128) hipLaunchKernelGGL((dwconv_ln_kernel<DW, 8>), grid, blk, 0, s, x, y, dw_w, dw_b, g, bta, C, T, dil, rg);
    else return fail(ctx, TVC_ERR_ARG, "dwconv_ln: unsupported channel count %d", C);
    return 0;
}

static __global__ void grn_norm_kernel(const float* __restrict__ h, float* __restrict__ gx, long rows, int T, RagDev rg, int C2) {
    const int lane = threadIdx.x & 63;
    long wave = (blockIdx.x * (long)blockDim.x + threadIdx.x) >> 6;
    long nwaves = ((long)gridDim.x * blockDim.x) >> 6;
    for (long r = wave; r < rows; r += nwaves) {
        const float* p = h + r * T;
        int n = T;
        if (rg.tb) {
            const int b = (int)(r / C2), c = (int)(r - (long)b * C2);
            p = h + (long)c * T + rg.pre[b];
            n = rg.tb[b];
        }
        float s = 0.f;
        for (int t = lane; t < n; t += 64) s = fmaf(p[t], p[t], s);
#pragma unroll
        for (int o = 32; o > 0; o >>= 1) s += __shfl_xor(s, o);
        if (lane == 0) gx[r] = sqrtf(s);
    }
}

static __global__ __launch_bounds__(256) void grn_finalize_kernel(const float* __restrict__ gx, const float* __restrict__ gamma,
                                                                  float* __restrict__ nx, int C2, float* __restrict__ hmax) {
    __shared__ float red[4];
    __shared__ float redm[4];
    const int b = blockIdx.x;
    const float* g = gx + (long)b * C2;
    float s = 0.f;
    for (int c = threadIdx.x; c < C2; c += 256) s += g[c];
#pragma unroll
    for (int o = 32; o > 0; o >>= 1) s += __shfl_xor(s, o);
    if ((threadIdx.x & 63) == 0) red[threadIdx.x >> 6] = s;
    __syncthreads();
    const float mean = (red[0] + red[1] + red[2] + red[3]) / (float)C2;
    const float den = mean + 1e-6f;
    float mx = 0.f;
    for (int c = threadIdx.x; c < C2; c += 256) {
        const float f = fmaf(gamma[c], g[c] / den, 1.f);
        nx[(long)b * C2 + c] = f;
        mx = fmaxf(mx, g[c] * fabsf(f));
    }
#pragma unroll
    for (int o = 32; o > 0; o >>= 1) mx = fmaxf(mx, __shfl_xor(mx, o));
    if ((threadIdx.x & 63) == 0) redm[threadIdx.x >> 6] = mx;
    __syncthreads();
    if (threadIdx.x == 0) hmax[b] = fmaxf(fmaxf(redm[0], redm[1]), fmaxf(redm[2], redm[3]));
}

int run_layernorm(tvc_ctx* ctx, hipStream_t s, float* x, const float* g, const float* b, int B, int C, int T) {
    TVC_CHECK(dwconv_ln_launch<false>(ctx, s, x, x, nullptr, nullptr, g, b, B, C, T, 1));
    return launch_check(ctx, "layernorm");
}

static __global__ void grn_tiles_kernel(float* __restrict__ gp, int gp_tiles, int K, int T, RagDev rg) {
    const int b = blockIdx.y, c = blockIdx.x * blockDim.x + threadIdx.x;
    if (c >= K) return;
    const int Tb = rg.tb ? rg.tb[b] : T, n = (Tb + 63) / 64;
    float* g = gp + (long)b * gp_tiles * K + c;
    float s = g[0];
    for (int t = 1; t < n; ++t) s += g[(long)t * K];
    g[0] = s;
}

template <int C>
static bool cnx_try(int* rc, tvc_ctx* ctx, hipStream_t s, const ConvNeXtW& w, float* x, float* h, float* gx, int B, int T, float* amax_out) {
    if (w.C != C || !(w.ln_bound < 32768.f) || w.c2.MT6 != 2 * C / 32 || w.c3.MT6 != C / 32 || w.c2.S6 < C / 16 || w.c3.S6 < 2 * C / 16) return false;
    const int NB = ctx->rag ? ctx->rag->B : B, Tl = ctx->rag ? ctx->rag->Tlong : T, rs = T;
    if ((long)rs * 8 * 4 >= (1L << 31)) return false;
    constexpr int KP = C == 384 ? 2 : 1;
    if ((*rc = lds_optin<cnx1_kernel<C, 1>>(ctx, Cnx1<C, 1>::LDS_BYTES, "cnx")) ||
        (*rc = lds_optin<cnx1_kernel<C, 2>>(ctx, Cnx1<C, 2>::LDS_BYTES, "cnx")) ||
        (*rc = lds_optin<cnx2_kernel<C, KP>>(ctx, Cnx2<C, KP>::LDS_BYTES, "cnx")))
        return true;
    CnxArgs a{};
    a.x = x;
    a.h = h;
    a.T = T;
    a.rs = rs;
    if ((*rc = rag_view(ctx, s, 1, 0, &a.rg, nullptr)) != 0) return true;
    auto split = [&](int MT, int tiles) {
        int d = 1;
        for (int c = 1; c <= MT; ++c)
            if (MT % c == 0 && (long)tiles * c <= ctx->ncu) d = c;
        return d;
    };
    {
        a.A6 = reinterpret_cast<const uint4*>(w.c2.A6);
        a.wsc = w.c2.wscale;
        a.bias = w.c2.bias;
        a.MT = w.c2.MT6;
        a.dw_w = w.dw_w;
        a.dw_b = w.dw_b;
        a.ln_g = w.ln_g;
        a.ln_b = w.ln_b;
        a.dil = w.dilation;
        const int nt = Tl <= 32 ? 1 : 2, tx = (Tl + 32 * nt - 1) / (32 * nt);
        a.gp = gx;
        a.gp_tiles = tx;
        const int d = split(a.MT, tx * NB);
        a.mt_per_wg = a.MT / d;
        const dim3 grid((unsigned)tx, (unsigned)NB, (unsigned)d);
        constexpr int nthr = Cnx1<C, 2>::NTHR, lds1 = Cnx1<C, 1>::LDS_BYTES, lds2 = Cnx1<C, 2>::LDS_BYTES;
        if (nt == 1) hipLaunchKernelGGL((cnx1_kernel<C, 1>), grid, dim3(nthr), lds1, s, a);
        else hipLaunchKernelGGL((cnx1_kernel<C, 2>), grid, dim3(nthr), lds2, s, a);
    }
    a.gp_sum = a.gp_tiles > CNX_GP_INLINE;
    if (a.gp_sum) hipLaunchKernelGGL(grn_tiles_kernel, dim3((2 * C + 255) / 256, (unsigned)NB), dim3(256), 0, s, gx, a.gp_tiles, 2 * C, T, a.rg);
    {
        a.A6 = reinterpret_cast<const uint4*>(w.c3.A6);
        a.wsc = w.c3.wscale;
        a.bias = w.c3_bias_grn;
        a.MT = w.c3.MT6;
        a.grn_g = w.grn_g;
        a.amax_y = amax_out;
        const int tx = (Tl + 63) / 64;
        const int d = split(a.MT, tx * NB);
        a.mt_per_wg = a.MT / d;
        constexpr int nthr = Cnx2<C, KP>::NTHR, lds = Cnx2<C, KP>::LDS_BYTES;
        hipLaunchKernelGGL((cnx2_kernel<C, KP>), dim3((unsigned)tx, (unsigned)NB, (unsigned)d), dim3(nthr), lds, s, a);
    }
    *rc = launch_check(ctx, "convnext (fused)");
    return true;
}

int run_convnext(tvc_ctx* ctx, hipStream_t s, Ws& ws, const ConvNeXtW& w, float* x, int B, int T, float* amax_out) {
    const int C = w.C, C2 = 2 * w.C, ncols = B * T;
    const int NB = ctx->rag ? ctx->rag->B : B;
    size_t mk = ws.mark();
    float* y = ws.get<float>((size_t)B * C * T);
    float* h = ws.get<float>((size_t)B * C2 * T);
    const int Tlong = ctx->rag ? ctx->rag->Tlong : T;
    float* gx = ws.get<float>((size_t)NB * C2 * ((Tlong + 63) / 64));
    float* nx = ws.get<float>((size_t)NB * C2);
    float* ymax = ws.get<float>((size_t)NB);
    float* hmax = ws.get<float>((size_t)NB);
    ws.release(mk);
    if (ws.dry) return 0;
    {
        int rc = 0;
        if (C == 384 ? cnx_try<384>(&rc, ctx, s, w, x, h, gx, B, T, amax_out) : (C == 128 && cnx_try<128>(&rc, ctx, s, w, x, h, gx, B, T, amax_out))) return rc;
    }
    {
        TVC_CHECK(dwconv_ln_launch<true>(ctx, s, x, y, w.dw_w, w.dw_b, w.ln_g, w.ln_b, B, C, T, w.dilation));
    }
    {
        const float* ym = nullptr;
        if (!(w.ln_bound < 32768.f)) {
            TVC_HIP(ctx, hipMemsetAsync(ymax, 0, (size_t)NB * sizeof(float), s));
            TVC_CHECK(run_amax_rows(ctx, s, y, B, C, T, ymax));
            ym = ymax;
        }
        EpiBias<ACT_GELU, false> ep{h, w.c2.bias, nullptr, C2, T, ncols, (long)C2 * T, 0};
        int rc = 0;
        if (!gemm_s2_try(&rc, ctx, s, w.c2, y, B, C, T, 0, ep, ym)) rc = gemm_s_launch<ENC_MTB, ENC_NWV, ENC_BPC>(ctx, s, w.c2, y, B, C, T, 0, ep, ym);
        TVC_CHECK(rc);
    }
    {
        RagDev rg;
        TVC_CHECK(rag_view(ctx, s, 1, 0, &rg, nullptr));
        hipLaunchKernelGGL(grn_norm_kernel, dim3(grid_for((long)NB * C2 * 64)), dim3(256), 0, s, h, gx, (long)NB * C2, T, rg, C2);
        hipLaunchKernelGGL(grn_finalize_kernel, dim3(NB), dim3(256), 0, s, gx, w.grn_g, nx, C2, hmax);
    }
    {
        EpiBias<ACT_NONE, true> ep{x, w.c3_bias_grn, x, C, T, ncols, (long)C * T, (long)C * T};
        int rc = 0;
        if (!gemm_s2_try<EpiBias<ACT_NONE, true>, true>(&rc, ctx, s, w.c3, h, B, C2, T, 0, ep, hmax, nx))
            rc = gemm_s_launch<ENC_MTB, ENC_NWV, ENC_BPC, EpiBias<ACT_NONE, true>, true>(ctx, s, w.c3, h, B, C2, T, 0, ep, hmax, nx);
        TVC_CHECK(rc);
    }
    if (amax_out) TVC_CHECK(run_amax_rows(ctx, s, x, B, C, T, amax_out));
    return launch_check(ctx, "convnext");
}

struct EpiSplit {
    static constexpr bool kIgemm = true;
    float* y0;
    float* y1;
    const float* bias;
    int M0, M1, T, ncols;
    __device__ __forceinline__ void store(int n, int m, const float v[4]) const {
        if (n >= ncols) return;
        int b = n / T, t = n - b * T;
#pragma unroll
        for (int r = 0; r < 4; ++r) {
            int mm = m + r;
            float o = v[r] + bias[mm < M0 + M1 ? mm : 0];
            if (mm < M0)
                y0[((long)b * M0 + mm) * T + t] = o;
            else if (mm < M0 + M1)
                y1[((long)b * M1 + mm - M0) * T + t] = o;
        }
    }
};

struct PTop4 {
    float v[4];
    int i[4];
    __device__ __forceinline__ void init() {
#pragma unroll
        for (int j = 0; j < 4; ++j) { v[j] = -INFINITY; i[j] = 0x7fffffff; }
    }
    __device__ __forceinline__ static bool better(float a, int ia, float b, int ib) { return a > b || (a == b && ia < ib); }
    __device__ __forceinline__ void insert(float x, int ix) {
        if (!better(x, ix, v[3], i[3])) return;
        if (better(x, ix, v[0], i[0])) { v[3] = v[2]; i[3] = i[2]; v[2] = v[1]; i[2] = i[1]; v[1] = v[0]; i[1] = i[0]; v[0] = x; i[0] = ix; }
        else if (better(x, ix, v[1], i[1])) { v[3] = v[2]; i[3] = i[2]; v[2] = v[1]; i[2] = i[1]; v[1] = x; i[1] = ix; }
        else if (better(x, ix, v[2], i[2])) { v[3] = v[2]; i[3] = i[2]; v[2] = x; i[2] = ix; }
        else { v[3] = x; i[3] = ix; }
    }
};

constexpr int kPdWaves = 16;
static __global__ __launch_bounds__(kPdWaves * 64) void pitch_decode_kernel(const float* __restrict__ logits, const float* __restrict__ freq,
                                                                  float* __restrict__ f0, int B, int T, float* __restrict__ f0s, float shift,
                                                                  const float* __restrict__ shifts, const int* __restrict__ col2b) {
    __shared__ float sv[kPdWaves][4][64];
    __shared__ int si[kPdWaves][4][64];
    const int lane = threadIdx.x & 63, wave = threadIdx.x >> 6;
    const long ncols = (long)B * T;
    const long n = blockIdx.x * 64L + lane;
    const bool ok = n < ncols;
    const long nn = ok ? n : ncols - 1;
    const int b = (int)(nn / T), t = (int)(nn - (long)b * T);
    const float* p = logits + (long)b * kPitchClasses * T + t;
    PTop4 top;
    top.init();
    constexpr int CPW = kPitchClasses / kPdWaves;
    float xv[CPW];
#pragma unroll
    for (int j = 0; j < CPW; ++j) xv[j] = p[(long)(wave * CPW + j) * T];
#pragma unroll
    for (int j = 0; j < CPW; ++j) {
        const float x = xv[j];
        top.insert(x != x ? INFINITY : x, wave * CPW + j);
    }
#pragma unroll
    for (int e = 0; e < 4; ++e) { sv[wave][e][lane] = top.v[e]; si[wave][e][lane] = top.i[e]; }
    __syncthreads();
    if (wave != 0 || !ok) return;
    for (int w = 1; w < kPdWaves; ++w)
#pragma unroll
        for (int e = 0; e < 4; ++e) top.insert(sv[w][e][lane], si[w][e][lane]);
#pragma unroll
    for (int e = 0; e < 4; ++e) top.i[e] = (unsigned)top.i[e] < (unsigned)kPitchClasses ? top.i[e] : 0;
    const float v0 = top.v[0];
    float e0 = 1.f, e1 = (float)exp((double)(top.v[1] - v0)), e2 = (float)exp((double)(top.v[2] - v0)), e3 = (float)exp((double)(top.v[3] - v0));
    float den = ((e0 + e1) + e2) + e3;
    float acc = __fmul_rn(e0 / den, freq[top.i[0]]);
    acc = __fadd_rn(acc, __fmul_rn(e1 / den, freq[top.i[1]]));
    acc = __fadd_rn(acc, __fmul_rn(e2 / den, freq[top.i[2]]));
    acc = __fadd_rn(acc, __fmul_rn(e3 / den, freq[top.i[3]]));
    const float fv = acc <= 20.f ? 0.f : acc;
    f0[n] = fv;
    if (f0s) f0s[n] = shift_frequency_one(fv, shifts ? shifts[col2b ? col2b[n] : b] : shift);
}

int run_pitch_decode(tvc_ctx* ctx, hipStream_t s, const float* logits, float* f0, int B, int T) {
    if (!ctx->pitch_freq) return fail(ctx, TVC_ERR_STATE, "pitch table not uploaded (tvc_set_pitch_table + tvc_finalize_weights)");
    const long ncols = (long)B * T;
    hipLaunchKernelGGL(pitch_decode_kernel, dim3((unsigned)((ncols + 63) / 64)), dim3(kPdWaves * 64), 0, s, logits, ctx->pitch_freq, f0, B, T, (float*)nullptr, 0.f, (const float*)nullptr, (const int*)nullptr);
    return launch_check(ctx, "pitch_decode");
}

int run_encoder(tvc_ctx* ctx, hipStream_t s, Ws& ws, const float* spec, float* ssl, float* f0,
                float* logits, int B, int T, const float* spec_bound, float* zeroed_slots, float* f0_shifted, float shift, const float* shifts) {
    const int ncols = B * T;
    float* xs = ws.get<float>((size_t)B * kSslCh * T);
    float* xp = ws.get<float>((size_t)B * kPitchCh * T);
    float* lg = logits ? logits : ws.get<float>((size_t)B * kPitchClasses * T);
    const int NB = ctx->rag ? ctx->rag->B : B;
    float* slots = zeroed_slots ? zeroed_slots : ws.get<float>((size_t)3 * NB);
    float *spec_max = slots, *xs_max = slots + NB, *xp_max = slots + 2 * NB;
    if (!ws.dry) {
        if (!zeroed_slots) TVC_HIP(ctx, hipMemsetAsync(slots, 0, (size_t)3 * NB * sizeof(float), s));
        if (spec_bound) spec_max = const_cast<float*>(spec_bound);
        else TVC_CHECK(run_amax_rows(ctx, s, spec, B, kBins, T, spec_max));
        EpiSplit ep{xs, xp, ctx->enc_in.bias, kSslCh, kPitchCh, T, ncols};
        TVC_CHECK((gemm_s_launch_ragged<ENC_MTB, ENC_NWV, ENC_BPC>(ctx, s, ctx->enc_in, spec, B, kBins, T, (long)kBins * T, ep, spec_max)));
        TVC_CHECK(run_layernorm(ctx, s, xs, ctx->ssl_ln_g, ctx->ssl_ln_b, B, kSslCh, T));
        TVC_CHECK(run_layernorm(ctx, s, xp, ctx->pit_ln_g, ctx->pit_ln_b, B, kPitchCh, T));
    }
    const int gtiles = ((ctx->rag ? ctx->rag->Tlong : T) + 63) / 64;
    const size_t ssl_scratch = ((size_t)B * kSslCh * T * 3 + (size_t)NB * kSslCh * 2 * (gtiles + 1)) * sizeof(float) + (size_t)NB * 8 + 4096;
    char* ssl_blk = ws.get<char>(ssl_scratch);
    Ws wssl(ssl_blk, ssl_scratch, ws.dry);
    SideFork fk(ctx, s);
    TVC_CHECK(fk.fork(ws, ctx->ev_fork, ctx->ev_join));
    const hipStream_t sp = fk.side;
    for (int i = 0; i < 4; ++i) TVC_CHECK(run_convnext(ctx, sp, ws, ctx->pit_mid[i], xp, B, T, i == 3 ? xp_max : nullptr));
    if (!ws.dry) {
        EpiBias<ACT_NONE, false> ep{lg, ctx->pit_out.bias, nullptr, kPitchClasses, T, ncols, (long)kPitchClasses * T, 0};
        int rc = 0;
        if (!gemm_s2_try(&rc, ctx, sp, ctx->pit_out, xp, B, kPitchCh, T, 0, ep, xp_max)) rc = gemm_s_launch<ENC_MTB, ENC_NWV, ENC_BPC>(ctx, sp, ctx->pit_out, xp, B, kPitchCh, T, 0, ep, xp_max);
        TVC_CHECK(rc);
        hipLaunchKernelGGL(pitch_decode_kernel, dim3((ncols + 63) / 64), dim3(kPdWaves * 64), 0, sp, lg, ctx->pitch_freq, f0, B, T, f0_shifted, shift, shifts,
                           shifts && ctx->rag ? ctx->rag->d_col2b : (const int*)nullptr);
    }
    TVC_CHECK(fk.end());
    for (int i = 0; i < 6; ++i) TVC_CHECK(run_convnext(ctx, s, wssl, ctx->ssl_mid[i], xs, B, T, i == 5 ? xs_max : nullptr));
    if (wssl.peak > wssl.cap) return fail(ctx, TVC_ERR_WORKSPACE, "encoder: SSL scratch block too small");
    if (ws.dry) return 0;
    {
        EpiBias<ACT_NONE, false> ep{ssl, ctx->ssl_out.bias, nullptr, kSslDim, T, ncols, (long)kSslDim * T, 0};
        int rc = 0;
        if (!gemm_s2_try(&rc, ctx, s, ctx->ssl_out, xs, B, kSslCh, T, 0, ep, xs_max)) rc = gemm_s_launch<ENC_MTB, ENC_NWV, ENC_BPC>(ctx, s, ctx->ssl_out, xs, B, kSslCh, T, 0, ep, xs_max);
        TVC_CHECK(rc);
    }
    TVC_CHECK(fk.join());
    return launch_check(ctx, "encoder");
}

}
```

### tinyvc_amd/csrc/tvc_common.h

```cpp
#pragma once
#include <hip/hip_runtime.h>

#include <atomic>
#include <cstdarg>
#include <cstdint>
#include <cstdio>
#include <cstring>
#include <map>
#include <string>
#include <vector>

#include "../../include/tinyvc_hip.h"
#include "ragged.h"

namespace tvc {

constexpr int kSampleRate = 24000;
constexpr int kNfft = 1920;
constexpr int kHop = 480;
constexpr int kBins = 961;
constexpr int kSslDim = 768;
constexpr int kSslCh = 384;
constexpr int kPitchCh = 128;
constexpr int kPitchClasses = 512;
constexpr int kSrcCh = 128;
constexpr int kHarm = 15;
constexpr int kSolaCross = 1920, kSolaSearch = 1920, kSolaDelay = 3840;
constexpr int kSolaGroups = 8, kSolaPartFloats = 16384;

struct PackedW {
    const float* bias = nullptr;
    const float* A6 = nullptr;
    const float* wscale = nullptr;
    const float* wjoint = nullptr;
    int M = 0, K = 0, Mpad = 0, Kpad = 0, cin = 0, taps = 1, MT6 = 0, S6 = 0;
};

struct ConvNeXtW {
    const float* dw_w = nullptr;
    const float* dw_b = nullptr;
    const float* ln_g = nullptr;
    const float* ln_b = nullptr;
    PackedW c2, c3;
    const float* grn_g = nullptr;
    const float* grn_b = nullptr;
    const float* c3_bias_grn = nullptr;
    float ln_bound = 0.f;
    int C = 0, dilation = 1;
};

constexpr int K24_PIECES = 10;
struct Up24sBlob {
    static constexpr int PIECES = 28;
    static constexpr int BA = 0, BB = 32, BSC = 64, BSH = 96;
    static constexpr int W75 = 128, B75 = 296;
    static constexpr int SA = 297, SB = 298, SSC = 299, SSH = 300;
    static constexpr int L1A = 301, BMA = 302;
    static constexpr int FLOATS = 304;
};
struct Down0sBlob {
    static constexpr int PIECES = K24_PIECES;
    static constexpr int BIAS = 0;
    static constexpr int BW = 29, BB = 30;
    static constexpr int SCALE = 31;
    static constexpr int FLOATS = 32;
};
struct Conv24sBlob {
    static constexpr int BIAS = 0;
    static constexpr int SCALE = 62;
    static constexpr int FLOATS = 64;
};

struct DownW {
    PackedW res, c1, c2, c3;
    const float* c3res_bias = nullptr;
    const float* s24c1 = nullptr;
    const float* s24c2 = nullptr;
    const float* s24c3r = nullptr;
    float b1_w = 0.f, b1_b = 0.f, b2_w = 0.f, b2_b = 0.f;
    int cin = 0, cout = 0, factor = 1;
};
struct FilmU {
    static constexpr int TAB_BIAS = 0, TAB_SCALE = 1, TAB_BSC = 2, TAB_BSH = 3, TAB_SSC = 4, TAB_SSH = 5;
    const float* img = nullptr;
    const float* tab = nullptr;
    int C = 0;
    float hb_w = 0.f, hb_b = 0.f;
};
struct UpW {
    PackedW c1, c2, c3, c4, c5, film1, film2;
    FilmU fu1, fu2;
    const float* s24a = nullptr;
    const float* s24b = nullptr;
    float c5_bw = 0.f, c5_bb = 0.f;
    int cin = 0, cout = 0, factor = 1;
};

struct HostTensor {
    std::vector<float> data;
    std::vector<int64_t> shape;
};

struct ArenaBuilder {
    std::vector<float> buf;
    std::vector<std::pair<const float**, size_t>> fix;
    size_t put(const float** slot, const float* v, size_t n);
    size_t put(const float** slot, const std::vector<float>& v) { return put(slot, v.data(), v.size()); }
    void resolve(const float* arena) const {
        for (auto& f : fix) *f.first = arena + f.second;
    }
};

}

struct tvc_prof_region {
    std::string name;
    hipEvent_t a = nullptr, b = nullptr;
};

struct tvc_ctx {
    int device = 0;
    int ncu = 0;
    int profiling = 0;
    std::vector<tvc_prof_region> regions;
    std::vector<hipEvent_t> event_pool;
    hipStream_t side = nullptr;
    hipEvent_t ev_fork = nullptr, ev_join = nullptr;
    hipEvent_t ev_fork2 = nullptr, ev_join2 = nullptr, ev_amps = nullptr;
    tvc::RagHost* rag = nullptr;
    int rag_batch_frames = 0;
    int index_assign_chunk = 0;
    bool enc_ready = false, dec_ready = false;
    char enc_missing[160] = {0}, dec_missing[160] = {0};
    std::map<std::string, tvc::HostTensor> host;
    std::vector<float> pitch_table;
    float* arena = nullptr;
    float* const_arena = nullptr;
    size_t arena_floats = 0;
    char err[512] = {0};

    const float* fft_tw960 = nullptr;
    const float* fft_tw1920 = nullptr;
    const float* fft_hann = nullptr;
    const float* pitch_freq = nullptr;
    const float* sola_part = nullptr;

    tvc::PackedW enc_in;
    const float* ssl_ln_g = nullptr;
    const float* ssl_ln_b = nullptr;
    const float* pit_ln_g = nullptr;
    const float* pit_ln_b = nullptr;
    tvc::ConvNeXtW ssl_mid[6], pit_mid[4], src_mid[3];
    tvc::PackedW ssl_out, pit_out;
    tvc::PackedW src_content_in, src_to_amps, src_to_kernel;
    const float* src_e_w = nullptr;
    const float* src_e_b = nullptr;
    const float* src_f_w = nullptr;
    const float* src_f_b = nullptr;
    tvc::PackedW flt_content_in;
    const float* flt_down0s = nullptr;
    float down0_bw = 0.f, down0_bb = 0.f;
    float flt_in_bw = 0.f, flt_in_bb = 0.f;
    const float* flt_f_w = nullptr;
    const float* flt_f_b = nullptr;
    tvc::DownW downs[4];
    tvc::UpW ups[5];
};

namespace tvc {

inline int fail(tvc_ctx* ctx, int code, const char* fmt, ...) {
    if (ctx) {
        va_list ap;
        va_start(ap, fmt);
        vsnprintf(ctx->err, sizeof(ctx->err), fmt, ap);
        va_end(ap);
    }
    return code;
}

#define TVC_HIP(ctx, call)                                                                       \
    do {                                                                                         \
        hipError_t e_ = (call);                                                                  \
        if (e_ != hipSuccess)                                                                    \
            return tvc::fail(ctx, TVC_ERR_HIP, "%s failed: %s (%s:%d)", #call, hipGetErrorString(e_), \
                             __FILE__, __LINE__);                                                \
    } while (0)

#define TVC_CHECK(expr)        \
    do {                       \
        int rc_ = (expr);      \
        if (rc_ != 0) return rc_; \
    } while (0)

struct Ws {
    char* base;
    size_t cap, off = 0, peak = 0;
    bool dry;
    Ws(void* p, size_t c, bool d) : base((char*)p), cap(c), dry(d) {}
    template <class T>
    T* get(size_t n) {
        size_t bytes = (n * sizeof(T) + 255) & ~size_t(255);
        size_t o = off;
        off += bytes;
        if (off > peak) peak = off;
        if (dry) return (T*)(uintptr_t)256;
        return (T*)(base + o);
    }
    size_t mark() const { return off; }
    void release(size_t m) { off = m; }
};

struct ProfScope {
    tvc_ctx* ctx;
    hipStream_t s;
    int idx = -1;
    ProfScope(tvc_ctx* c, hipStream_t st, const Ws& ws, const char* name) : ctx(c), s(st) {
        if (!c || !c->profiling || ws.dry) return;
        if (c->profiling == 2 && std::strncmp(name, "filter_net", 10) != 0) return;
        tvc_prof_region r;
        r.name = name;
        auto take = [&](hipEvent_t* e) {
            if (!c->event_pool.empty()) {
                *e = c->event_pool.back();
                c->event_pool.pop_back();
                return true;
            }
            return hipEventCreate(e) == hipSuccess;
        };
        if (!take(&r.a) || !take(&r.b)) return;
        (void)hipEventRecord(r.a, s);
        c->regions.push_back(r);
        idx = (int)c->regions.size() - 1;
    }
    ~ProfScope() {
        if (idx >= 0) (void)hipEventRecord(ctx->regions[idx].b, s);
    }
};

struct SideFork {
    tvc_ctx* ctx;
    hipStream_t s, side;
    hipEvent_t ev_join = nullptr;
    bool ended = false;
    SideFork(tvc_ctx* c, hipStream_t st) : ctx(c), s(st), side(st) {}
    bool forked() const { return ev_join != nullptr; }
    int fork(const Ws& ws, hipEvent_t ev_fork, hipEvent_t join) {
        hipStreamCaptureStatus cap = hipStreamCaptureStatusNone;
        if (ws.dry || !ctx->side || !ev_fork || !join || hipStreamIsCapturing(s, &cap) != hipSuccess || cap != hipStreamCaptureStatusNone) return 0;
        TVC_HIP(ctx, hipEventRecord(ev_fork, s));
        TVC_HIP(ctx, hipStreamWaitEvent(ctx->side, ev_fork, 0));
        side = ctx->side;
        ev_join = join;
        return 0;
    }
    int end() {
        if (forked() && !ended) TVC_HIP(ctx, hipEventRecord(ev_join, side));
        ended = true;
        return 0;
    }
    hipError_t record_and_wait() {
        hipEvent_t e = ev_join;
        ev_join = nullptr;
        const hipError_t r = e && !ended ? hipEventRecord(e, side) : hipSuccess;
        return e && r == hipSuccess ? hipStreamWaitEvent(s, e, 0) : r;
    }
    int join() { TVC_HIP(ctx, record_and_wait()); return 0; }
    ~SideFork() { (void)record_and_wait(); }
};

inline int launch_check(tvc_ctx* ctx, const char* what) {
    hipError_t e = hipGetLastError();
    if (e != hipSuccess) return fail(ctx, TVC_ERR_HIP, "launch %s: %s", what, hipGetErrorString(e));
    return 0;
}

template <auto... K>
int lds_optin(tvc_ctx* ctx, int bytes, const char* what) {
    static std::atomic<bool> ready_dev[64];
    std::atomic<bool>& ready = ready_dev[ctx->device & 63];
    if (ready.load(std::memory_order_acquire)) return 0;
    for (const void* k : {(const void*)K...}) {
        const hipError_t e = hipFuncSetAttribute(k, hipFuncAttributeMaxDynamicSharedMemorySize, bytes);
        if (e != hipSuccess) return fail(ctx, TVC_ERR_HIP, "%s setup: %s", what, hipGetErrorString(e));
    }
    ready.store(true, std::memory_order_release);
    return 0;
}

void pack_constants(tvc_ctx*, ArenaBuilder*);
void pack_checkpoint(tvc_ctx*, ArenaBuilder*, std::string* missing_enc, std::string* missing_dec);

int run_stft(tvc_ctx*, hipStream_t, Ws&, const float* wav, float* spec, int B, int64_t L);
int run_stft_fft(tvc_ctx*, hipStream_t, const float* wav, float* spec, int B, int64_t L);
int run_noise_ifft(tvc_ctx*, hipStream_t, const float* kern, const float* angle, uint64_t seed, float* frames, int B, int T, bool angle_padded = false);
int run_energy(tvc_ctx*, hipStream_t, Ws&, const float* wav, float* energy, int B, int64_t L, float* emax = nullptr, float* spec_bound = nullptr,
               float* zero = nullptr, int nz = 0);
int run_knn_amax_rows(tvc_ctx*, hipStream_t, const std::vector<const float*>& blobs, float* out);
int run_slot_affine(tvc_ctx*, hipStream_t, float* out, const float* in, int in_stride, float a, float c, int n);
int run_slot_prep(tvc_ctx*, hipStream_t, float* zero, int nz, float* o1, const float* in1, int s1, float a1, float c1, float* o2, const float* in2, int s2, float a2,
                  float c2, float* o3, float a3, float c3, int n);
constexpr int kBlobMagic = 0x54564B4E, kBlobVersion = 2;
constexpr int kFilterSlotX = 2;
constexpr int kFilterSlots = 41;
int run_encoder(tvc_ctx*, hipStream_t, Ws&, const float* spec, float* ssl, float* f0,
                float* logits, int B, int T, const float* spec_bound = nullptr, float* zeroed_slots = nullptr,
                float* f0_shifted = nullptr, float shift = 0.f,
                const float* shifts = nullptr);
int run_pitch_decode(tvc_ctx*, hipStream_t, const float* logits, float* f0, int B, int T);
int run_knn(tvc_ctx*, hipStream_t, Ws&, const float* src, const float* prepared, int64_t N,
            float* out, int64_t* idx_out, int B, int T);
struct KnnSegIn {
    const float* blob;
    int64_t N;
    int col0, ncols;
};
int run_knn_segs(tvc_ctx*, hipStream_t, Ws&, const float* src, const KnnSegIn* in, int nin, float* out, int64_t* idx_out, int B, int T);
int run_knn_blend(tvc_ctx*, hipStream_t, Ws&, const float* src, const KnnSegIn* in, int nin, int M, const float* weights, float* out, int64_t* idx_out,
                  int B, int T);
int run_knn_blend_bound(tvc_ctx*, hipStream_t, const std::vector<const float*>& blobs, const std::vector<int>& rows, int M, const float* weights, float* out);

struct ConvertIndex {
    const float* blob = nullptr;
    int64_t N = 0;
    const float* const* blobs = nullptr;
    const int64_t* Ns = nullptr;
    bool per_row = false;
    int M = 0;
    const float* weights = nullptr;
    static ConvertIndex one(const float* blob, int64_t N) { return {blob, N, nullptr, nullptr, false, 0, nullptr}; }
    static ConvertIndex table(const float* const* blobs, const int64_t* Ns) { return {nullptr, 0, blobs, Ns, true, 0, nullptr}; }
    static ConvertIndex blend(const float* const* blobs, const int64_t* Ns, int M, const float* weights) { return {nullptr, 0, blobs, Ns, true, M, weights}; }
};
struct ConvertCall {
    const float* wav = nullptr;
    float* wave = nullptr;
    int B = 0;
    int64_t L = 0;
    const int64_t* lens = nullptr;
    ConvertIndex index;
    float shift = 0.f;
    const float* shifts = nullptr;
    const float* angle = nullptr;
    uint64_t seed = 0;
    const float* target_f0 = nullptr;
    float* shift_out = nullptr;
};
int convert_impl(tvc_ctx*, hipStream_t, Ws&, const ConvertCall& c);
int run_knn_topk(tvc_ctx*, hipStream_t, Ws&, const float* src, const float* prepared, int64_t N,
                 float* sims_out, int64_t* idx_out, int B, int T);
int run_knn_general(tvc_ctx*, hipStream_t, Ws&, const float* src, const float* index, int64_t N, int k, int metric, float* out, int64_t* idx_out,
                    float* val_out, int B, int T);
int run_knn_slots(tvc_ctx*, hipStream_t, const float* prepared, int64_t N, const int64_t* idx, float* slots, int64_t nslots);
int run_knn_finish(tvc_ctx*, hipStream_t, const float* slots, float* out, int B, int T);
int run_shift(tvc_ctx*, hipStream_t, const float* f0, float* out, int64_t n, float semitones);
struct PitchRow {
    int start, len, idx;
    float offset;
};
int run_pitch_match(tvc_ctx*, hipStream_t, const float* f0, const std::vector<PitchRow>& rows, const float* target, float* median_out, int* voiced_out,
                    float* shift_out, float* f0s);
int run_uniform_to_angle(tvc_ctx*, hipStream_t, float* u, int64_t n);
int run_decoder(tvc_ctx*, hipStream_t, Ws&, const float* content, const float* f0,
                const float* energy, const float* angle, uint64_t seed, float* wave, float* amps_out,
                float* kernel_out, float* source_out, int B, int T, const float* content_bound = nullptr, const float* energy_bound = nullptr,
                int content_bound_stride = 0);
struct FilterTaps {
    float* skips[5] = {nullptr, nullptr, nullptr, nullptr, nullptr};
    float* ups[4] = {nullptr, nullptr, nullptr, nullptr};
};
int run_filter(tvc_ctx*, hipStream_t, Ws&, const float* content, const float* f0, const float* energy,
               const float* source, float* wave, int B, int T, const FilterTaps* taps = nullptr, const float* cmax = nullptr, const float* smax = nullptr,
               float* zeroed_slots = nullptr, bool x_slot_set = false, float* x_pre = nullptr, bool x_pre_filled = false);
struct DspFork {
    hipStream_t side;
    hipEvent_t amps_ready;
};
int run_dsp(tvc_ctx*, hipStream_t, Ws&, const float* f0, const float* amps, const float* kern, const float* angle, uint64_t seed, float* source, int B, int T,
            float* smax = nullptr, double* csum = nullptr, const DspFork* fk = nullptr);
int run_sola(tvc_ctx*, hipStream_t, const float* y, float* sola_buf, const float* fade_in, float* out, int32_t* shift_out,
             int S, int64_t Ly, int block, int use_pv);
int run_stream_push(tvc_ctx* ctx, hipStream_t s, float* buf, const float* blocks, int S, int n, int m);
int64_t resample_out_len(int64_t n, int orig_freq, int new_freq);
int run_resample(tvc_ctx*, hipStream_t, const float* x, float* y, int rows, int64_t n, int orig_freq, int new_freq);
int run_pcm16_to_f32(tvc_ctx*, hipStream_t, const int16_t* pcm, float* y, int64_t n, float gain_db);
int run_f32_to_pcm16(tvc_ctx*, hipStream_t, const float* x, int16_t* pcm, int64_t n, float gain_db);
void frontdoor_release(tvc_ctx*);
int run_prepare_index(tvc_ctx*, hipStream_t, const float* index, float* prepared, int64_t N);
int run_prepare_index_f16(tvc_ctx*, hipStream_t, const void* rows_f16, float* prepared, int64_t N);
int run_prepare_index_cols(tvc_ctx*, hipStream_t, const float* feats, int64_t S, const int64_t* cols, int64_t N, float* prepared, float* index_out);
int run_prepare_index_cols_f16(tvc_ctx*, hipStream_t, const float* feats, int64_t S, const int64_t* cols, int64_t N, float* prepared, void* index_out_f16);

constexpr int kIndexAssignChunk = 32768;
constexpr int64_t kIndexCompactMaxK = 1 << 20;
int run_index_assign(tvc_ctx*, hipStream_t, Ws&, const float* points, int64_t N, const float* cent_blob, int64_t K, int64_t* assign, float* sim_out, int32_t* moved);
int run_index_update(tvc_ctx*, hipStream_t, Ws&, const float* points, int64_t N, const int64_t* assign, int64_t K, float* centroids, int32_t* counts_out);
int run_index_compact(tvc_ctx*, hipStream_t, Ws&, const float* points, int64_t N, const int64_t* init_cols, int64_t K, int iters, float* centroids, float* prepared_out,
                      int64_t* assign_out, int32_t* counts_out, int32_t* moved_out);

int run_up24_split(tvc_ctx*, hipStream_t, const UpW& u, const float* x, const float* cond_planes, float cbw, float cbb, float* x1, float* out, int B, int len,
                   const float* amax_x, const float* amax_c, float* amax_x1);
int run_down0_split(tvc_ctx*, hipStream_t, const float* blob, const float* source, const float* energy, float* planes, float* out_fp32, float* y2, int B, int len,
                    const float* amax_x, float* amax_y);
int run_down24_fused(tvc_ctx*, hipStream_t, const DownW& d, const float* xi, float* out, float* y2, int B, int len, const float* amax_xi, float* amax_out);
int run_conv48s(tvc_ctx*, hipStream_t, const PackedW& w, const float* x, const PackedW* film, const float* bsc, const float* bsh, const float* cond,
                const float* res, float* out, int B, int len, int dil, const float* amax_x, const float* amax_c, float* amax_y,
                const PackedW* c5 = nullptr, float* out5 = nullptr);

int run_conv48_pair(tvc_ctx*, hipStream_t, const PackedW& wa, const PackedW& wb, const float* x, int lin, float lscale, const PackedW* film, const float* bsc,
                    const float* bsh, const float* cond, float* out, int B, int len, int da, int db, const float* amax_x, const float* amax_c,
                    float* amax_y);

int run_convnext(tvc_ctx*, hipStream_t, Ws&, const ConvNeXtW& w, float* x, int B, int T, float* amax_out = nullptr);

}
```

### tinyvc_amd/engine.py

```python
import ctypes
import math
import threading
import weakref

import torch

from . import _lib, spec

_F32 = torch.float32


def _ptr(t):
    return ctypes.c_void_p(t.data_ptr()) if t is not None else None


def _floats(xs):
    return (ctypes.c_float * len(xs))(*xs) if xs is not None else None


def _check_dev(t, name, device):
    if not isinstance(t, torch.Tensor):
        raise TypeError(f"{name} must be a torch.Tensor")
    if t.device.type != "cuda":
        raise _lib.TinyVCError(
            f"{name} is on {t.device}: tinyvc_amd runs on an AMD GPU only (no CPU fallback). "
            "Move the model and inputs to 'cuda'.")
    if device is not None and t.device != device:
        raise _lib.TinyVCError(f"{name} is on {t.device}, engine is on {device}")


def _prep(t, name, device):
    _check_dev(t, name, device)
    if t.dtype != _F32:
        t = t.float()
    return t.contiguous()


def pitch_shifts(pitch_shift, B):
    if isinstance(pitch_shift, torch.Tensor):
        if pitch_shift.dim() == 0:
            return float(pitch_shift), None
        if pitch_shift.dim() != 1:
            raise ValueError("pitch_shift: a float or a 1-D sequence of one shift per row")
        pitch_shift = pitch_shift.detach().cpu().tolist()
    if not hasattr(pitch_shift, "__len__"):
        return float(pitch_shift), None
    sh = [float(x) for x in pitch_shift]
    if len(sh) != B:
        raise ValueError(f"pitch_shift: {len(sh)} shifts for a batch of {B}")
    return 0.0, sh


_CONVERT = {
    ("shared", False): ("tvc_workspace_bytes", "tvc_convert_f32"),
    ("shared", True): ("tvc_workspace_bytes_ragged", "tvc_convert_ragged_f32"),
    ("table", False): ("tvc_workspace_bytes_multi", "tvc_convert_multi_f32"),
    ("table", True): ("tvc_workspace_bytes_ragged_multi", "tvc_convert_ragged_multi_f32"),
    ("blend", False): ("tvc_workspace_bytes_blend", "tvc_convert_blend_f32"),
    ("blend", True): ("tvc_workspace_bytes_ragged_blend", "tvc_convert_ragged_blend_f32"),
    ("auto", False): ("tvc_workspace_bytes_auto", "tvc_convert_auto_f32"),
    ("auto", True): ("tvc_workspace_bytes_ragged_auto", "tvc_convert_ragged_auto_f32"),
}
_MATCH = {
    "shared": ("tvc_workspace_bytes", "tvc_knn_match_f32"),
    "table": ("tvc_workspace_bytes_multi", "tvc_knn_match_multi_f32"),
    "blend": ("tvc_workspace_bytes_blend", "tvc_knn_match_blend_f32"),
}


def pitch_class_table():
    ids = torch.arange(spec.PITCH_CLASSES).to(torch.float)
    x = spec.PITCH_FMIN * (2 ** (ids / spec.PITCH_CPO))
    x[x <= spec.PITCH_FMIN] = 0
    return x.contiguous()


def _forget_blob(engine_ref, ptr):
    eng = engine_ref()
    if eng is not None and getattr(eng, "ctx", None):
        eng.lib.tvc_knn_forget(eng.ctx, ctypes.c_void_p(ptr))


class Engine:

    def __init__(self, device):
        device = torch.device(device)
        if device.type != "cuda":
            raise _lib.TinyVCError(f"tinyvc_amd needs a GPU device, got {device}")
        if device.index is None:
            device = torch.device("cuda", torch.cuda.current_device())
        self.device = device
        self.lib = _lib.load_library()
        h = ctypes.c_void_p()
        rc = self.lib.tvc_ctx_create(device.index, ctypes.byref(h))
        if rc != 0 or not h:
            raise _lib.TinyVCError(f"tvc_ctx_create(device={device.index}) failed with {rc}")
        self.ctx = h
        self._ws = None
        self._seed = 0x1234ABCD
        self.weights_key = None

    def __del__(self):
        try:
            if getattr(self, "ctx", None):
                self.lib.tvc_ctx_destroy(self.ctx)
                self.ctx = None
        except Exception:
            pass

    def _ok(self, rc, what):
        if rc != 0:
            msg = self.lib.tvc_last_error(self.ctx)
            raise _lib.TinyVCError(f"{what} failed ({rc}): {msg.decode() if msg else ''}")

    def _stream(self):
        return ctypes.c_void_p(torch.cuda.current_stream(self.device).cuda_stream)

    def _grow_ws(self, nbytes):
        if self._ws is None or self._ws.numel() < nbytes:
            self._ws = None
            self._ws = torch.empty(nbytes, dtype=torch.uint8, device=self.device)
        return self._ws

    def _query_ws(self, query, *args):
        need = ctypes.c_size_t()
        self._ok(getattr(self.lib, query)(self.ctx, *args, ctypes.byref(need)), query)
        ws = self._grow_ws(need.value)
        return _ptr(ws), ctypes.c_size_t(ws.numel())

    def workspace(self, B, L, N):
        self._query_ws("tvc_workspace_bytes", int(B), int(L), int(max(N, 4)))
        return self._ws

    def _wsargs(self, B, L, N=4):
        ws = self.workspace(B, L, N)
        return _ptr(ws), ctypes.c_size_t(ws.numel())

    def set_ragged_batch_frames(self, max_frames):
        self._ok(self.lib.tvc_ctx_set_ragged_batch_frames(self.ctx, int(max_frames)), "tvc_ctx_set_ragged_batch_frames")

    def set_index_assign_chunk(self, max_queries):
        self._ok(self.lib.tvc_ctx_set_index_assign_chunk(self.ctx, int(max_queries)), "tvc_ctx_set_index_assign_chunk")

    def next_seed(self):
        self._seed = (self._seed * 6364136223846793005 + 1442695040888963407) & 0xFFFFFFFFFFFFFFFF
        return self._seed

    def profile(self, on=True):
        self._ok(self.lib.tvc_profile_enable(self.ctx, int(on)), "tvc_profile_enable")

    def profile_read(self):
        buf = ctypes.create_string_buffer(8192)
        self._ok(self.lib.tvc_profile_read(self.ctx, buf, len(buf)), "tvc_profile_read")
        out = {}
        for item in buf.value.decode().split(";"):
            if "=" in item:
                k, v = item.split("=")
                out[k] = float(v)
        return out

    def load_weights(self, tensors):
        keep = []
        for k, v in tensors.items():
            t = v.detach().to("cpu", _F32).contiguous()
            keep.append(t)
            shape = (ctypes.c_int64 * t.dim())(*t.shape)
            self._ok(self.lib.tvc_load_tensor(self.ctx, k.encode(), ctypes.c_void_p(t.data_ptr()), shape, t.dim()), f"tvc_load_tensor({k})")
        tab = pitch_class_table()
        self._ok(self.lib.tvc_set_pitch_table(self.ctx, ctypes.c_void_p(tab.data_ptr()), tab.numel()), "tvc_set_pitch_table")
        self._ok(self.lib.tvc_finalize_weights(self.ctx), "tvc_finalize_weights")

    def stft_mag(self, wav):
        wav = _prep(wav, "wave", self.device)
        B, L = wav.shape
        if L % spec.HOP:
            raise ValueError("waveform length must be a multiple of 480 (autopad_waveform)")
        out = torch.empty(B, spec.FFT_BIN, L // spec.HOP, dtype=_F32, device=self.device)
        p, n = self._wsargs(B, L)
        self._ok(self.lib.tvc_stft_mag_f32(self.ctx, self._stream(), _ptr(wav), _ptr(out), B, L, p, n), "tvc_stft_mag_f32")
        return out

    def energy(self, wav):
        wav = _prep(wav, "wave", self.device)
        B, L = wav.shape
        out = torch.empty(B, 1, L, dtype=_F32, device=self.device)
        p, n = self._wsargs(B, max(L - L % spec.HOP, spec.HOP))
        self._ok(self.lib.tvc_energy_f32(self.ctx, self._stream(), _ptr(wav), _ptr(out), B, L, p, n), "tvc_energy_f32")
        return out

    def resample(self, wav, orig_freq, new_freq):
        orig_freq, new_freq = int(orig_freq), int(new_freq)
        wav = _prep(wav, "wave", self.device)
        if orig_freq == new_freq:
            return wav
        shape = wav.shape
        x = wav.reshape(-1, shape[-1])
        n_out = self.lib.tvc_resample_out_len(x.shape[1], orig_freq, new_freq)
        y = torch.empty(x.shape[0], n_out, dtype=_F32, device=self.device)
        self._ok(self.lib.tvc_resample_f32(self.ctx, self._stream(), _ptr(x), _ptr(y), x.shape[0], x.shape[1], orig_freq, new_freq), "tvc_resample_f32")
        return y.reshape(shape[:-1] + (n_out,))

    def pcm16_to_f32(self, pcm, gain_db=0.0):
        _check_dev(pcm, "pcm", self.device)
        if pcm.dtype != torch.int16:
            raise ValueError("pcm must be int16")
        pcm = pcm.contiguous()
        y = torch.empty(pcm.shape, dtype=_F32, device=self.device)
        if pcm.numel():
            self._ok(self.lib.tvc_pcm16_to_f32(self.ctx, self._stream(), _ptr(pcm), _ptr(y), pcm.numel(), float(gain_db)), "tvc_pcm16_to_f32")
        return y

    def f32_to_pcm16(self, x, gain_db=0.0):
        x = _prep(x, "wave", self.device)
        pcm = torch.empty(x.shape, dtype=torch.int16, device=self.device)
        if x.numel():
            self._ok(self.lib.tvc_f32_to_pcm16(self.ctx, self._stream(), _ptr(x), _ptr(pcm), x.numel(), float(gain_db)), "tvc_f32_to_pcm16")
        return pcm

    def encoder(self, spec_t, want_logits=False):
        x = _prep(spec_t, "spec", self.device)
        B, C, T = x.shape
        if C != spec.FFT_BIN:
            raise ValueError(f"spec must have {spec.FFT_BIN} bins, got {C}")
        ssl = torch.empty(B, spec.SSL_DIM, T, dtype=_F32, device=self.device)
        f0 = torch.empty(B, 1, T, dtype=_F32, device=self.device)
        logits = torch.empty(B, spec.PITCH_CLASSES, T, dtype=_F32, device=self.device) if want_logits else None
        p, n = self._wsargs(B, T * spec.HOP)
        self._ok(self.lib.tvc_encoder_f32(self.ctx, self._stream(), _ptr(x), _ptr(ssl), _ptr(f0), _ptr(logits), B, T, p, n), "tvc_encoder_f32")
        return ssl, f0, logits

    def pitch_decode(self, logits):
        lg = _prep(logits, "logits", self.device)
        B, C, T = lg.shape
        if C != spec.PITCH_CLASSES:
            raise ValueError(f"logits must have {spec.PITCH_CLASSES} classes")
        f0 = torch.empty(B, 1, T, dtype=_F32, device=self.device)
        self._ok(self.lib.tvc_pitch_decode_f32(self.ctx, self._stream(), _ptr(lg), _ptr(f0), B, T), "tvc_pitch_decode_f32")
        return f0

    def knn_prepare(self, index):
        _check_dev(index, "index", self.device)
        half = index.dtype == torch.float16
        idx = index if half else _prep(index, "index", self.device)
        if idx.dim() == 3:
            if idx.shape[0] != 1:
                raise ValueError("knn_prepare takes one index ([1, 768, N])")
            idx = idx[0]
        if idx.shape[0] != spec.SSL_DIM:
            raise ValueError(f"index must be [768, N], got {tuple(idx.shape)}")
        N = idx.shape[1]
        if N < 4:
            raise RuntimeError("selected index k out of range")
        if half:
            rows = idx.t().contiguous()
            blob = torch.empty(self.lib.tvc_knn_prepared_elems_f16(N), dtype=_F32, device=self.device)
            self._ok(self.lib.tvc_knn_prepare_index_f16(self.ctx, self._stream(), _ptr(rows), _ptr(blob), N), "tvc_knn_prepare_index_f16")
            return self._owned(blob), N
        blob = torch.empty(self.lib.tvc_knn_prepared_elems(N), dtype=_F32, device=self.device)
        self._ok(self.lib.tvc_knn_prepare_index_f32(self.ctx, self._stream(), _ptr(idx.contiguous()), _ptr(blob), N), "tvc_knn_prepare_index_f32")
        return self._owned(blob), N

    def knn_prepare_columns(self, feats, cols, half=False, want_index=True):
        feats = _prep(feats, "feats", self.device)
        if feats.dim() != 2 or feats.shape[0] != spec.SSL_DIM:
            raise ValueError(f"feats must be [768, S], got {tuple(feats.shape)}")
        cols = cols.to(device=self.device, dtype=torch.int64).contiguous()
        if cols.dim() != 1:
            raise ValueError("cols must be a 1-D list of columns")
        S, N = feats.shape[1], cols.numel()
        if N < 1:
            raise ValueError("cols selects no vector")
        index = torch.empty(1, spec.SSL_DIM, N, dtype=torch.float16 if half else _F32, device=self.device) if want_index else None
        if half:
            blob = torch.empty(self.lib.tvc_knn_prepared_elems_f16(N), dtype=_F32, device=self.device)
            self._ok(self.lib.tvc_knn_prepare_index_cols_f16(self.ctx, self._stream(), _ptr(feats), S, _ptr(cols), N, _ptr(blob), _ptr(index)),
                     "tvc_knn_prepare_index_cols_f16")
        else:
            blob = torch.empty(self.lib.tvc_knn_prepared_elems(N), dtype=_F32, device=self.device)
            self._ok(self.lib.tvc_knn_prepare_index_cols_f32(self.ctx, self._stream(), _ptr(feats), S, _ptr(cols), N, _ptr(blob), _ptr(index)),
                     "tvc_knn_prepare_index_cols_f32")
        return self._owned(blob), N, index

    def encode_ragged(self, wav, lengths):
        wav, B, Lmax = self._rows(wav, ragged=True)
        lens = self._lens(lengths, B)
        p, n = self._query_ws("tvc_workspace_bytes_encode_ragged", B, Lmax, lens)
        pre = [0]
        for length in lengths:
            pre.append(pre[-1] + int(length) // spec.HOP)
        ssl = torch.empty(spec.SSL_DIM, pre[-1], dtype=_F32, device=self.device)
        f0 = torch.empty(pre[-1], dtype=_F32, device=self.device)
        self._ok(self.lib.tvc_encode_ragged_f32(self.ctx, self._stream(), _ptr(wav), Lmax, lens, _ptr(ssl), _ptr(f0), B, p, n), "tvc_encode_ragged_f32")
# ... 379 lines not shown
```

Before: 728.2 million.

## Fuse ConvNeXt layer boundaries into a single kernel across encoder chains

Replaces per-layer ConvNeXt dispatch with a chain runner that fuses each layer's second pointwise/GRN stage with the next layer's depthwise conv, LayerNorm and first pointwise stage in one boundary kernel. The input tile stays resident in LDS, and the h and GRN-partial buffers are double-buffered. The aim is to drop one launch and one full activation round-trip per layer boundary. A heuristic limits fusion to cases with enough tiles and dilation halos that fit, and a context knob plus API can turn it off. The cost is larger workspace and more complex kernels, with possible occupancy and register pressure.

```diff
diff --git a/include/tinyvc_hip.h b/include/tinyvc_hip.h
--- a/include/tinyvc_hip.h
+++ b/include/tinyvc_hip.h
@@ -110,6 +110,8 @@
 int tvc_workspace_bytes_ragged(tvc_ctx* ctx, int B, int64_t Lmax, const int64_t* lens, int64_t N, size_t* out_bytes);
 int tvc_ragged_plan(int B, int64_t Lmax, const int64_t* lens, int max_frames, int32_t* batch_of_row, int* n_batches);
 int tvc_ctx_set_ragged_batch_frames(tvc_ctx* ctx, int max_frames);
+int tvc_ctx_set_cnx_fuse(tvc_ctx* ctx, int on);
+int tvc_cnx_boundary_fuses(const int32_t* frames, int n, int dilation);
 int tvc_convert_ragged_f32(tvc_ctx* ctx, void* stream, const float* wav, int64_t Lmax, const int64_t* lens, const float* prepared_index,
                            int64_t N, float pitch_shift, const float* noise_angle, uint64_t seed, float* wave, int B, void* ws,
                            size_t ws_bytes);
diff --git a/tinyvc_amd/_lib.py b/tinyvc_amd/_lib.py
--- a/tinyvc_amd/_lib.py
+++ b/tinyvc_amd/_lib.py
@@ -32,6 +32,8 @@
     "tvc_knn_forget": (c_int, [c_void_p, c_void_p]),
     "tvc_ragged_plan": (c_int, [c_int, c_int64, POINTER(c_int64), c_int, POINTER(c_int32), POINTER(c_int)]),
     "tvc_ctx_set_ragged_batch_frames": (c_int, [c_void_p, c_int]),
+    "tvc_ctx_set_cnx_fuse": (c_int, [c_void_p, c_int]),
+    "tvc_cnx_boundary_fuses": (c_int, [POINTER(c_int32), c_int, c_int]),
     "tvc_knn_prepare_index_f32": (c_int, [c_void_p, c_void_p, c_void_p, c_void_p, c_int64]),
     "tvc_knn_match_f32": (c_int, [c_void_p, c_void_p, c_void_p, c_void_p, c_int64, c_void_p, c_void_p, c_int, c_int, c_void_p, c_size_t]),
     "tvc_knn_match_general_f32": (c_int, [c_void_p, c_void_p, c_void_p, c_void_p, c_int64, c_int, c_int, c_void_p, c_void_p, c_void_p, c_int, c_int, c_void_p, c_size_t]),
diff --git a/tinyvc_amd/csrc/api.hip b/tinyvc_amd/csrc/api.hip
--- a/tinyvc_amd/csrc/api.hip
+++ b/tinyvc_amd/csrc/api.hip
@@ -738,6 +738,18 @@
     ctx->rag_batch_frames = max_frames;
     return TVC_OK;
 }
+int tvc_ctx_set_cnx_fuse(tvc_ctx* ctx, int on) {
+    if (!ctx) return TVC_ERR_ARG;
+    if (on < 0 || on > 2) return fail(ctx, TVC_ERR_ARG, "tvc_ctx_set_cnx_fuse: 0 = off, 1 = where it pays (the default), 2 = wherever it fits");
+    ctx->cnx_fuse = on;
+    return TVC_OK;
+}
+int tvc_cnx_boundary_fuses(const int32_t* frames, int n, int dilation) {
+    if (!frames || n <= 0 || dilation < 1) return TVC_ERR_ARG;
+    for (int i = 0; i < n; ++i)
+        if (frames[i] < 1) return TVC_ERR_ARG;
+    return cnx_fuse_fits(frames, n, dilation) ? 1 : 0;
+}
 int tvc_ragged_plan(int B, int64_t Lmax, const int64_t* lens, int max_frames, int32_t* batch_of_row, int* n_batches) {
     if (!lens || !batch_of_row || !n_batches || B <= 0 || Lmax <= 0 || Lmax % kHop != 0 || max_frames < 0) return TVC_ERR_ARG;
     std::vector<RagBatchPlan> batches;
diff --git a/tinyvc_amd/csrc/cnx_s3.h b/tinyvc_amd/csrc/cnx_s3.h
--- a/tinyvc_amd/csrc/cnx_s3.h
+++ b/tinyvc_amd/csrc/cnx_s3.h
@@ -4,22 +4,51 @@
 
 namespace tvc {
 
-struct CnxArgs {
-    float* x;
-    float* h;
-    int T, rs;
-    RagDev rg;
+struct CnxMat {
     const uint4* A6;
     const float* wsc;
     const float* bias;
     int MT, mt_per_wg;
+};
+
+struct CnxArgs {
+    const float* xi;
+    float* xo;
+    const float* hi;
+    float* ho;
+    int T, rs;
+    RagDev rg;
+    CnxMat c2, c3;
     const float *dw_w, *dw_b, *ln_g, *ln_b;
     int dil;
-    float* gp;
+    const float* gpi;
+    float* gpo;
     int gp_tiles;
     int gp_sum;
     const float* grn_g;
     float* amax_y;
+};
+
+struct CnxTile {
+    int Tb, ntu, t0, tw;
+    long xoff, hoff;
+    template <int C>
+    __device__ __forceinline__ bool set(const CnxArgs& a, int NC) {
+        const int b = blockIdx.y;
+        Tb = a.T;
+        xoff = (long)b * C * a.T;
+        hoff = (long)b * 2 * C * a.T;
+        if (a.rg.tb) {
+            Tb = a.rg.tb[b];
+            xoff = hoff = a.rg.pre[b];
+        }
+        ntu = (Tb + NC - 1) / NC;
+        if ((int)blockIdx.x >= ntu) return false;
+        const int TW = (Tb + ntu - 1) / ntu;
+        t0 = blockIdx.x * TW;
+        tw = Tb - t0 < TW ? Tb - t0 : TW;
+        return true;
+    }
 };
 
 constexpr int CNX_GP_INLINE = 16;
@@ -76,37 +105,13 @@
 struct Cnx1 {
     static constexpr int WAVES = 8, NTHR = WAVES * 64, NC = 32 * NT, KS = C / 16, CPT = C / 16, VW = NT;
     static constexpr int YS_U4 = KS * 4 * NC;
-    static constexpr int LDS_BYTES = YS_U4 * 16 + (C * 8 + 2 * C + 16 * NC) * 4;
+    static constexpr int SIDE_FLOATS = C * 8 + 2 * C + 16 * NC;
+    static constexpr int LDS_BYTES = YS_U4 * 16 + SIDE_FLOATS * 4;
     static_assert(LDS_BYTES <= 160 * 1024, "LDS");
 };
 
-template <int C, int NT>
-__global__ __launch_bounds__((Cnx1<C, NT>::NTHR)) void cnx1_kernel(CnxArgs a) {
-    using CF = Cnx1<C, NT>;
-    constexpr int NC = CF::NC, KS = CF::KS, CPT = CF::CPT, VW = CF::VW, WAVES = CF::WAVES, NTHR = CF::NTHR;
-    extern __shared__ __attribute__((aligned(16))) uint4 smem_c1[];
-    uint4* Ys = smem_c1;
-    float* scr = reinterpret_cast<float*>(smem_c1);
-    float* Wl = reinterpret_cast<float*>(smem_c1 + CF::YS_U4);
-    float* Gl = Wl + C * 8;
-    float* red = Gl + 2 * C;
-    const int tid = threadIdx.x, lane = tid & 63, l31 = lane & 31, lh = lane >> 5;
-    const int wave = __builtin_amdgcn_readfirstlane(tid >> 6);
-    const int b = blockIdx.y;
-    int Tb = a.T;
-    long xoff = (long)b * C * a.T, hoff = (long)b * 2 * C * a.T;
-    if (a.rg.tb) {
-        Tb = a.rg.tb[b];
-        xoff = hoff = a.rg.pre[b];
-    }
-    const int ntu = (Tb + NC - 1) / NC;
-    if ((int)blockIdx.x >= ntu) return;
-    const int TW = (Tb + ntu - 1) / ntu;
-    const int t0 = blockIdx.x * TW;
-    const int tw = Tb - t0 < TW ? Tb - t0 : TW;
-    const int rs = a.rs;
-    const float* xb = a.x + xoff;
-
+template <int C, int NTHR>
+__device__ __forceinline__ void cnx1_stage_weights(const CnxArgs& a, float* Wl, float* Gl, int tid) {
     for (int i = tid; i < C; i += NTHR) {
 #pragma unroll
         for (int j = 0; j < 7; ++j) Wl[i * 8 + j] = a.dw_w[i * 7 + j];
@@ -114,7 +119,21 @@
         Gl[i] = a.ln_g[i];
         Gl[C + i] = a.ln_b[i];
     }
-    __syncthreads();
+}
+
+template <int C, int NT, bool LTAP>
+__device__ __forceinline__ void cnx1_body(const CnxArgs& a, const CnxTile& t, uint4* Ys, float* Wl, float* Gl, float* red, int cb) {
+    using CF = Cnx1<C, NT>;
+    constexpr int NC = CF::NC, KS = CF::KS, CPT = CF::CPT, VW = CF::VW, WAVES = CF::WAVES;
+    static_assert(!LTAP || NT == 2, "the resident input tile is 64 columns wide");
+    float* scr = reinterpret_cast<float*>(Ys);
+    const int tid = threadIdx.x, lane = tid & 63, l31 = lane & 31, lh = lane >> 5;
+    const int wave = __builtin_amdgcn_readfirstlane(tid >> 6);
+    const int b = blockIdx.y;
+    const int Tb = t.Tb, t0 = t.t0, tw = t.tw;
+    const long hoff = t.hoff;
+    const int rs = a.rs;
+    const float* xb = a.xi + t.xoff;
 
     const int col = NT == 2 ? lane : l31;
     const int tc = t0 + (col < tw ? col : tw - 1);
@@ -123,7 +142,7 @@
     for (int j = 0; j < 7; ++j) {
         int q = tc + (j - 3) * a.dil;
         q = q < 0 ? 0 : (q >= Tb ? Tb - 1 : q);
-        tt[j] = 4u * (unsigned)q;
+        tt[j] = 4u * (unsigned)(LTAP ? q - cb : q);
     }
     float v[VW][CPT];
 #pragma unroll
@@ -136,7 +155,11 @@
             const f32x4s_t w0 = *reinterpret_cast<const f32x4s_t*>(Wl + c * 8), w1 = *reinterpret_cast<const f32x4s_t*>(Wl + c * 8 + 4);
             const float wj[7] = {w0[0], w0[1], w0[2], w0[3], w1[0], w1[1], w1[2]};
             float acc = w1[3];
-            if (NT == 2) {
+            if (LTAP) {
+                const char* xr = reinterpret_cast<const char*>(scr + c * NC);
+#pragma unroll
+                for (int j = 0; j < 7; ++j) acc = fmaf(wj[j], *reinterpret_cast<const float*>(xr + tt[j]), acc);
+            } else if (NT == 2) {
                 const float* xr = xb + (long)c * rs;
 #pragma unroll
                 for (int j = 0; j < 7; ++j) acc = fmaf(wj[j], ldg_so(xr, tt[j]), acc);
@@ -147,11 +170,17 @@
             }
             v[u][i] = acc;
             sum += acc;
-            scr[c * NC + col] = acc;
+            if (!LTAP) scr[c * NC + col] = acc;
         }
         red[vw * NC + col] = sum;
     }
     __syncthreads();
+    if (LTAP) {
+#pragma unroll
+        for (int u = 0; u < VW; ++u)
+#pragma unroll
+            for (int i = 0; i < CPT; ++i) scr[(wave + 8 * u + i * 16) * NC + col] = v[u][i];
+    }
     float tot = 0.f;
 #pragma unroll
     for (int w = 0; w < 16; ++w) tot += red[w * NC + col];
@@ -195,18 +224,19 @@
     }
     __syncthreads();
 
-    const int mt_lo = blockIdx.z * a.mt_per_wg;
-    const int mt_hi = mt_lo + a.mt_per_wg < a.MT ? mt_lo + a.mt_per_wg : a.MT;
+    const CnxMat& m = a.c2;
+    const int mt_lo = blockIdx.z * m.mt_per_wg;
+    const int mt_hi = mt_lo + m.mt_per_wg < m.MT ? mt_lo + m.mt_per_wg : m.MT;
     int mt = mt_lo + wave;
     if (mt >= mt_hi) return;
     u32x4 ring[CNX_PD][2];
 #pragma unroll
     for (int u = 0; u < CNX_PD; ++u) {
-        const uint4* ab = a.A6 + ((long)u * a.MT + mt) * kPU4;
+        const uint4* ab = m.A6 + ((long)u * m.MT + mt) * kPU4;
         ring[u][0] = ldg_so4(ab, 16u * (unsigned)lane);
         ring[u][1] = ldg_so4(ab, 16u * (unsigned)(64 + lane));
     }
-    float* hb = a.h + hoff;
+    float* hb = a.ho + hoff;
     constexpr int NPEND = NT * 16, EPS = ((NPEND + KS - 1) / KS + 1) / 2 * 2;
     float pend[NPEND];
     int pmt = mt;
@@ -220,7 +250,7 @@
 #pragma unroll
     for (int j = 0; j < NT; ++j) live[j] = j * 32 + l31 < tw;
     float sq[16];
-    float* gpb = a.gp + ((long)b * a.gp_tiles + blockIdx.x) * (2 * C) + ((l31 >> 1) & 3) + 8 * (l31 >> 3) + 4 * lh;
+    float* gpb = a.gpo + ((long)b * a.gp_tiles + blockIdx.x) * (2 * C) + ((l31 >> 1) & 3) + 8 * (l31 >> 3) + 4 * lh;
     auto finish2 = [&](int e) __attribute__((always_inline)) {
         const int j = e >> 4;
         f32x2e v = {pend[e], pend[e + 1]};
@@ -256,14 +286,14 @@
         const int mtn = mt + WAVES < mt_hi ? mt + WAVES : mt;
         float bv[16];
 #pragma unroll
-        for (int r = 0; r < 16; ++r) bv[r] = a.bias[mt * 32 + (r & 3) + 8 * (r >> 2) + 4 * lh];
+        for (int r = 0; r < 16; ++r) bv[r] = m.bias[mt * 32 + (r & 3) + 8 * (r >> 2) + 4 * lh];
         f32x16 hi[NT], lo[NT];
 #pragma unroll
         for (int j = 0; j < NT; ++j)
 #pragma unroll
             for (int r = 0; r < 16; ++r) hi[j][r] = lo[j][r] = 0.f;
-        cnx_mma<NT, NC, KS>(hi, lo, ring, a.A6, a.MT, mt, 0, mtn, 0, Ys, lane, poster);
-        const float cw = a.wsc[mt] * 1.f, cl = cw * kLoInv;
+        cnx_mma<NT, NC, KS>(hi, lo, ring, m.A6, m.MT, mt, 0, mtn, 0, Ys, lane, poster);
+        const float cw = m.wsc[mt] * 1.f, cl = cw * kLoInv;
 #pragma unroll
         for (int j = 0; j < NT; ++j)
 #pragma unroll
@@ -282,10 +312,26 @@
     for (int e = 0; e < NPEND; e += 2) finish2(e);
 }
 
-template <int C, int KPASS>
+template <int C, int NT>
+__global__ __launch_bounds__((Cnx1<C, NT>::NTHR)) void cnx1_kernel(CnxArgs a) {
+    using CF = Cnx1<C, NT>;
+    extern __shared__ __attribute__((aligned(16))) uint4 smem_c1[];
+    uint4* Ys = smem_c1;
+    float* Wl = reinterpret_cast<float*>(smem_c1 + CF::YS_U4);
+    float* Gl = Wl + C * 8;
+    float* red = Gl + 2 * C;
+    CnxTile t;
+    if (!t.set<C>(a, CF::NC)) return;
+    cnx1_stage_weights<C, CF::NTHR>(a, Wl, Gl, threadIdx.x);
+    __syncthreads();
+    cnx1_body<C, NT, false>(a, t, Ys, Wl, Gl, red, 0);
+}
+
+template <int C, int KPASS, int WV = (KPASS == 2 ? C / 32 : 8)>
 struct Cnx2 {
     static constexpr int K = 2 * C, NT = 2, NC = 64, KSL = K / 16 / KPASS;
-    static constexpr int WAVES = KPASS == 2 ? C / 32 : 8, NTHR = WAVES * 64;
+    static constexpr int WAVES = WV, NTHR = WAVES * 64;
+    static constexpr int R = KPASS == 2 ? (C / 32 + WAVES - 1) / WAVES : 1;
     static constexpr int YS_U4 = KSL * 4 * NC;
     static constexpr int GPP = K / 8 / KPASS;
     static constexpr int ITEMS = GPP * NC, XPER = (ITEMS + NTHR - 1) / NTHR;
@@ -294,31 +340,21 @@
     static_assert(LDS_BYTES <= 160 * 1024, "LDS");
 };
 
-template <int C, int KPASS>
-__global__ __launch_bounds__((Cnx2<C, KPASS>::NTHR)) void cnx2_kernel(CnxArgs a) {
-    using CF = Cnx2<C, KPASS>;
-    constexpr int K = CF::K, NT = CF::NT, NC = CF::NC, KSL = CF::KSL, WAVES = CF::WAVES, XPER = CF::XPER;
-    extern __shared__ __attribute__((aligned(16))) uint4 smem_c2[];
-    uint4* Ys = smem_c2;
-    float* Fl = reinterpret_cast<float*>(smem_c2 + CF::YS_U4);
+template <int C, int KPASS, int WV, bool KEEP, bool OUT>
+__device__ __forceinline__ void cnx2_body(const CnxArgs& a, const CnxTile& t, uint4* Ys, float* Fl, int cb, int cn, int mt_lo, int mt_hi,
+                                          f32x16 (&keep)[Cnx2<C, KPASS, WV>::R][2]) {
+    using CF = Cnx2<C, KPASS, WV>;
+    constexpr int K = CF::K, NT = CF::NT, NC = CF::NC, KSL = CF::KSL, WAVES = CF::WAVES, XPER = CF::XPER, R = CF::R;
     float* red = Fl + K;
     const int tid = threadIdx.x, lane = tid & 63;
     const int wave = __builtin_amdgcn_readfirstlane(tid >> 6);
     const int b = blockIdx.y;
-    int Tb = a.T;
-    long xoff = (long)b * C * a.T, hoff = (long)b * K * a.T;
-    if (a.rg.tb) {
-        Tb = a.rg.tb[b];
-        xoff = hoff = a.rg.pre[b];
-    }
-    const int ntu = (Tb + NC - 1) / NC;
-    if ((int)blockIdx.x >= ntu) return;
-    const int TW = (Tb + ntu - 1) / ntu;
-    const int t0 = blockIdx.x * TW;
-    const int tw = Tb - t0 < TW ? Tb - t0 : TW;
+    const int ntu = t.ntu, own = t.t0 - cb, tw = t.tw;
+    const long xoff = t.xoff, hoff = t.hoff;
     const int rs = a.rs;
-
-    const float* g = a.gp + (long)b * a.gp_tiles * K;
+    const CnxMat& m = a.c3;
+
+    const float* g = a.gpi + (long)b * a.gp_tiles * K;
     const int gtiles = a.gp_sum ? 1 : ntu;
     constexpr int GPT = K / 256;
     float gv[GPT], gm[GPT];
@@ -331,14 +367,15 @@
             gm[i] = a.grn_g[tid + 256 * i];
         }
     }
-    const float* hb = a.h + hoff;
+    const float* hb = a.hi + hoff;
     const int scol = lane;
-    const unsigned so = 4u * (unsigned)(t0 + (scol < tw ? scol : tw - 1));
+    const unsigned so = 4u * (unsigned)(cb + (scol < cn ? scol : cn - 1));
     float xr[XPER][8];
     Bfp sx{1.f, 1.f};
-    auto fetch = [&](int pass) __attribute__((always_inline)) {
-#pragma unroll
-        for (int i = 0; i < XPER; ++i) {
+    constexpr int XEARLY = R > 1 ? XPER * 2 / 3 : XPER;
+    auto fetch = [&](int pass, int i0, int i1) __attribute__((always_inline)) {
+#pragma unroll
+        for (int i = i0; i < i1; ++i) {
             const int gg = pass * CF::GPP + wave + i * WAVES;
 #pragma unroll
             for (int q = 0; q < 8; ++q) xr[i][q] = ldg_so(hb + (long)(8 * gg + q) * rs, so);
@@ -359,7 +396,7 @@
             Ys[(((gl >> 1) * 2 + 1) * 2 + (gl & 1)) * NC + scol] = p2;
         }
     };
-    fetch(0);
+    fetch(0, 0, XPER);
     if (tid < 256) {
         float s = 0.f;
 #pragma unroll
@@ -390,52 +427,34 @@
     sx.s = __builtin_bit_cast(float, __builtin_amdgcn_readfirstlane(__builtin_bit_cast(int, sx.s)));
     sx.inv = __builtin_bit_cast(float, __builtin_amdgcn_readfirstlane(__builtin_bit_cast(int, sx.inv)));
     deposit(0);
-    if (KPASS == 2) fetch(1);
+    if (KPASS == 2) fetch(1, 0, XEARLY);
     slab_barrier();
 
-    const int mt_lo = blockIdx.z * a.mt_per_wg;
-    const int mt_hi = mt_lo + a.mt_per_wg < a.MT ? mt_lo + a.mt_per_wg : a.MT;
     int mt = mt_lo + wave;
     const bool has = mt < mt_hi;
     if (!has) mt = mt_lo;
     u32x4 ring[CNX_PD][2];
 #pragma unroll
     for (int u = 0; u < CNX_PD; ++u) {
-        const uint4* ab = a.A6 + ((long)u * a.MT + mt) * kPU4;
+        const uint4* ab = m.A6 + ((long)u * m.MT + mt) * kPU4;
         ring[u][0] = ldg_so4(ab, 16u * (unsigned)lane);
         ring[u][1] = ldg_so4(ab, 16u * (unsigned)(64 + lane));
     }
-    float* xb = a.x + xoff;
     float mx_out = 0.f;
-    bool work = has;
-    while (KPASS == 2 || work) {
-        const int mtn = (KPASS == 1 && mt + WAVES < mt_hi) ? mt + WAVES : mt;
-        f32x16 hi[NT], lo[NT];
-#pragma unroll
-        for (int j = 0; j < NT; ++j)
-#pragma unroll
-            for (int r = 0; r < 16; ++r) hi[j][r] = lo[j][r] = 0.f;
-        if (KPASS == 1) {
-            cnx_mma<NT, NC, KSL>(hi, lo, ring, a.A6, a.MT, mt, 0, mtn, 0, Ys, lane);
-        } else {
-            if (has) cnx_mma<NT, NC, KSL>(hi, lo, ring, a.A6, a.MT, mt, 0, mt, KSL, Ys, lane);
-            slab_barrier();
-            deposit(1);
-            slab_barrier();
-            if (!has) break;
-            cnx_mma<NT, NC, KSL>(hi, lo, ring, a.A6, a.MT, mt, KSL, mt, KSL, Ys, lane);
-        }
-        const float cw = a.wsc[mt] * sx.inv, cl = cw * kLoInv;
+    auto epilogue = [&](int mt, f32x16 (&hi)[NT], f32x16 (&lo)[NT], f32x16 (&kp)[NT]) __attribute__((always_inline)) {
+        const float* xb = a.xi + xoff;
+        float* yb = OUT ? a.xo + xoff : const_cast<float*>(xb);
+        const float cw = m.wsc[mt] * sx.inv, cl = cw * kLoInv;
         int el = tid;
         asm volatile("" : "+v"(el));
         const int l31 = el & 31, lh = (el >> 5) & 1;
         float bv[16];
 #pragma unroll
-        for (int r = 0; r < 16; ++r) bv[r] = a.bias[mt * 32 + (r & 3) + 8 * (r >> 2) + 4 * lh];
+        for (int r = 0; r < 16; ++r) bv[r] = m.bias[mt * 32 + (r & 3) + 8 * (r >> 2) + 4 * lh];
 #pragma unroll
         for (int j = 0; j < NT; ++j) {
             const int n = j * 32 + l31;
-            const unsigned oo = 4u * (unsigned)(4 * lh * rs + t0 + (n < tw ? n : tw - 1));
+            const unsigned oo = 4u * (unsigned)(4 * lh * rs + cb + (n < cn ? n : cn - 1));
             float res[16];
 #pragma unroll
             for (int r = 0; r < 16; ++r) res[r] = ldg_so(xb + (long)(mt * 32 + (r & 3) + 8 * (r >> 2)) * rs, oo);
@@ -447,17 +466,121 @@
                 res[r] = o;
                 mx = fmaxf(mx, fabsf(o));
             }
-            if (n < tw) {
-#pragma unroll
-                for (int r = 0; r < 16; ++r) stg_so(xb + (long)(mt * 32 + (r & 3) + 8 * (r >> 2)) * rs, oo, res[r]);
+            if (n >= own && n < own + tw) {
+#pragma unroll
+                for (int r = 0; r < 16; ++r) stg_so(yb + (long)(mt * 32 + (r & 3) + 8 * (r >> 2)) * rs, oo, res[r]);
                 mx_out = fmaxf(mx_out, mx);
             }
-        }
-        if (KPASS == 2) break;
-        work = mt + WAVES < mt_hi;
-        mt += WAVES;
+            if (KEEP) {
+#pragma unroll
+                for (int r = 0; r < 16; ++r) kp[j][r] = res[r];
+            }
+        }
+    };
+    if (KPASS == 1) {
+        bool work = has;
+        while (work) {
+            const int mtn = mt + WAVES < mt_hi ? mt + WAVES : mt;
+            f32x16 hi[NT], lo[NT];
+#pragma unroll
+            for (int j = 0; j < NT; ++j)
+#pragma unroll
+                for (int r = 0; r < 16; ++r) hi[j][r] = lo[j][r] = 0.f;
+            cnx_mma<NT, NC, KSL>(hi, lo, ring, m.A6, m.MT, mt, 0, mtn, 0, Ys, lane);
+            epilogue(mt, hi, lo, keep[0]);
+            work = mt + WAVES < mt_hi;
+            mt += WAVES;
+        }
+    } else {
+        f32x16 hi[R][NT], lo[R][NT];
+#pragma unroll
+        for (int q = 0; q < R; ++q)
+#pragma unroll
+            for (int j = 0; j < NT; ++j)
+#pragma unroll
+                for (int r = 0; r < 16; ++r) hi[q][j][r] = lo[q][j][r] = 0.f;
+#pragma unroll
+        for (int q = 0; q < R; ++q) {
+            const bool more = q + 1 < R && mt + (q + 1) * WAVES < mt_hi;
+            if (q == 0 ? has : mt + q * WAVES < mt_hi) cnx_mma<NT, NC, KSL>(hi[q], lo[q], ring, m.A6, m.MT, mt + q * WAVES, 0, more ? mt + (q + 1) * WAVES : mt, more ? 0 : KSL, Ys, lane);
+        }
+        if (XEARLY < XPER) fetch(1, XEARLY, XPER);
+        slab_barrier();
+        deposit(1);
+        slab_barrier();
+        if (has) {
+#pragma unroll
+        for (int q = 0; q < R; ++q) {
+            const bool more = q + 1 < R && mt + (q + 1) * WAVES < mt_hi;
+            if (q == 0 || mt + q * WAVES < mt_hi)
+                cnx_mma<NT, NC, KSL>(hi[q], lo[q], ring, m.A6, m.MT, mt + q * WAVES, KSL, more ? mt + (q + 1) * WAVES : mt + q * WAVES, KSL, Ys, lane);
+        }
+#pragma unroll
+        for (int q = 0; q < R; ++q)
+            if (q == 0 || mt + q * WAVES < mt_hi) epilogue(mt + q * WAVES, hi[q], lo[q], keep[q]);
+        }
     }
     if (a.amax_y) amax_flush_wg(a.amax_y + b, mx_out, red + 8);
 }
 
-}
+template <int C, int KPASS, bool OUT>
+__global__ __launch_bounds__((Cnx2<C, KPASS>::NTHR)) void cnx2_kernel(CnxArgs a) {
+    using CF = Cnx2<C, KPASS>;
+    extern __shared__ __attribute__((aligned(16))) uint4 smem_c2[];
+    uint4* Ys = smem_c2;
+    float* Fl = reinterpret_cast<float*>(smem_c2 + CF::YS_U4);
+    CnxTile t;
+    if (!t.set<C>(a, CF::NC)) return;
+    const int mt_lo = blockIdx.z * a.c3.mt_per_wg;
+    const int mt_hi = mt_lo + a.c3.mt_per_wg < a.c3.MT ? mt_lo + a.c3.mt_per_wg : a.c3.MT;
+    f32x16 keep[CF::R][2];
+    cnx2_body<C, KPASS, CF::WAVES, false, OUT>(a, t, Ys, Fl, t.t0, t.tw, mt_lo, mt_hi, keep);
+}
+
+template <int C, int KPASS>
+struct Cnxf {
+    using C1 = Cnx1<C, 2>;
+    static constexpr int WAVES = C1::WAVES, NTHR = WAVES * 64, NC = 64;
+    using C2 = Cnx2<C, KPASS, WAVES>;
+    static constexpr int TILE_U4 = C2::YS_U4 > C1::YS_U4 ? C2::YS_U4 : C1::YS_U4;
+    static constexpr int LDS_BYTES = TILE_U4 * 16 + C1::SIDE_FLOATS * 4 + (2 * C + 32) * 4;
+    static_assert(C / 32 <= C2::R * WAVES, "a wave walks each of its m-tiles of c3 once");
+    static_assert(LDS_BYTES <= 160 * 1024, "LDS");
+};
+
+template <int C, int KPASS>
+__global__ __launch_bounds__((Cnxf<C, KPASS>::NTHR)) void cnxf_kernel(CnxArgs a) {
+    using CF = Cnxf<C, KPASS>;
+    constexpr int NC = CF::NC, WAVES = CF::WAVES, R = CF::C2::R;
+    extern __shared__ __attribute__((aligned(16))) uint4 smem_cf[];
+    uint4* Ys = smem_cf;
+    float* scr = reinterpret_cast<float*>(smem_cf);
+    float* Wl = reinterpret_cast<float*>(smem_cf + CF::TILE_U4);
+    float* Gl = Wl + C * 8;
+    float* red = Gl + 2 * C;
+    float* Fl = red + 16 * NC;
+    CnxTile t;
+    if (!t.set<C>(a, NC)) return;
+    const int lo3 = t.t0 - 3 * a.dil, hi3 = t.t0 + t.tw + 3 * a.dil;
+    const int cb = lo3 < 0 ? 0 : lo3, cn = (hi3 > t.Tb ? t.Tb : hi3) - cb;
+    cnx1_stage_weights<C, CF::NTHR>(a, Wl, Gl, threadIdx.x);
+    f32x16 keep[R][2];
+    cnx2_body<C, KPASS, WAVES, true, true>(a, t, Ys, Fl, cb, cn, 0, C / 32, keep);
+    __syncthreads();
+    {
+        const int lane = threadIdx.x & 63, l31 = lane & 31, lh = lane >> 5;
+        const int wave = __builtin_amdgcn_readfirstlane(threadIdx.x >> 6);
+#pragma unroll
+        for (int q = 0; q < R; ++q)
+            if (wave + q * WAVES < C / 32) {
+#pragma unroll
+                for (int j = 0; j < 2; ++j)
+#pragma unroll
+                    for (int r = 0; r < 16; ++r) scr[((wave + q * WAVES) * 32 + (r & 3) + 8 * (r >> 2) + 4 * lh) * NC + j * 32 + l31] = keep[q][j][r];
+            }
+    }
+    __syncthreads();
+    cnx1_body<C, 2, true>(a, t, Ys, Wl, Gl, red, cb);
+}
+
+}
diff --git a/tinyvc_amd/csrc/decoder.hip b/tinyvc_amd/csrc/decoder.hip
--- a/tinyvc_amd/csrc/decoder.hip
+++ b/tinyvc_amd/csrc/decoder.hip
@@ -175,7 +175,7 @@
         TVC_CHECK(rc);
     }
     if (!ws.dry && !xmax_zeroed) TVC_HIP(ctx, hipMemsetAsync(xmax, 0, (size_t)NB * sizeof(float), s));
-    for (int i = 0; i < 3; ++i) TVC_CHECK(run_convnext(ctx, s, ws, ctx->src_mid[i], x, B, T, i == 2 ? xmax : nullptr));
+    TVC_CHECK(run_convnext_chain(ctx, s, ws, &ctx->src_mid[0], 3, x, B, T, xmax));
     if (ws.dry) return 0;
     EpiBias<ACT_ELU1, false> ea{amps, ctx->src_to_amps.bias, nullptr, kHarm, T, ncols, (long)kHarm * T, 0};
     TVC_CHECK((gemm_s_launch<1, 4, 2>(ctx, s, ctx->src_to_amps, x, B, kSrcCh, T, 0, ea, xmax)));
diff --git a/tinyvc_amd/csrc/encoder.hip b/tinyvc_amd/csrc/encoder.hip
--- a/tinyvc_amd/csrc/encoder.hip
+++ b/tinyvc_amd/csrc/encoder.hip
@@ -176,84 +176,76 @@
     g[0] = s;
 }
 
+bool cnx_fuse_fits(const int* frames, int n, int dil) {
+    if (dil < 1) return false;
+    for (int i = 0; i < n; ++i) {
+        const int Tb = frames[i];
+        if (Tb < 1) return false;
+        if (Tb <= 64) continue;
+        const int ntu = (Tb + 63) / 64, TW = (Tb + ntu - 1) / ntu;
+        if (TW + 6 * dil > 64) return false;
+    }
+    return true;
+}
+
 template <int C>
-static bool cnx_try(int* rc, tvc_ctx* ctx, hipStream_t s, const ConvNeXtW& w, float* x, float* h, float* gx, int B, int T, float* amax_out) {
+static bool cnx_ok(const ConvNeXtW& w, int rs) {
     if (w.C != C || !(w.ln_bound < 32768.f) || w.c2.MT6 != 2 * C / 32 || w.c3.MT6 != C / 32 || w.c2.S6 < C / 16 || w.c3.S6 < 2 * C / 16) return false;
-    const int NB = ctx->rag ? ctx->rag->B : B, Tl = ctx->rag ? ctx->rag->Tlong : T, rs = T;
-    if ((long)rs * 8 * 4 >= (1L << 31)) return false;
+    return (long)rs * 8 * 4 < (1L << 31);
+}
+
+enum CnxKind { CNX_FIRST, CNX_SECOND, CNX_BOUNDARY };
+
+static void cnx_set_c2(CnxArgs& a, const ConvNeXtW& w) {
+    a.c2 = CnxMat{reinterpret_cast<const uint4*>(w.c2.A6), w.c2.wscale, w.c2.bias, w.c2.MT6, w.c2.MT6};
+    a.dw_w = w.dw_w;
+    a.dw_b = w.dw_b;
+    a.ln_g = w.ln_g;
+    a.ln_b = w.ln_b;
+    a.dil = w.dilation;
+}
+static void cnx_set_c3(CnxArgs& a, const ConvNeXtW& w) {
+    a.c3 = CnxMat{reinterpret_cast<const uint4*>(w.c3.A6), w.c3.wscale, w.c3_bias_grn, w.c3.MT6, w.c3.MT6};
+    a.grn_g = w.grn_g;
+}
+
+template <int C>
+static int cnx_launch(tvc_ctx* ctx, hipStream_t s, CnxKind kind, CnxArgs a, int NB, int Tl) {
     constexpr int KP = C == 384 ? 2 : 1;
-    if ((*rc = lds_optin<cnx1_kernel<C, 1>>(ctx, Cnx1<C, 1>::LDS_BYTES, "cnx")) ||
-        (*rc = lds_optin<cnx1_kernel<C, 2>>(ctx, Cnx1<C, 2>::LDS_BYTES, "cnx")) ||
-        (*rc = lds_optin<cnx2_kernel<C, KP>>(ctx, Cnx2<C, KP>::LDS_BYTES, "cnx")))
-        return true;
-    CnxArgs a{};
-    a.x = x;
-    a.h = h;
-    a.T = T;
-    a.rs = rs;
-    if ((*rc = rag_view(ctx, s, 1, 0, &a.rg, nullptr)) != 0) return true;
+    TVC_CHECK((lds_optin<cnx1_kernel<C, 1>>(ctx, Cnx1<C, 1>::LDS_BYTES, "cnx")));
+    TVC_CHECK((lds_optin<cnx1_kernel<C, 2>>(ctx, Cnx1<C, 2>::LDS_BYTES, "cnx")));
+    TVC_CHECK((lds_optin<cnx2_kernel<C, KP, false>>(ctx, Cnx2<C, KP>::LDS_BYTES, "cnx")));
+    TVC_CHECK((lds_optin<cnx2_kernel<C, KP, true>>(ctx, Cnx2<C, KP>::LDS_BYTES, "cnx")));
+    TVC_CHECK((lds_optin<cnxf_kernel<C, KP>>(ctx, Cnxf<C, KP>::LDS_BYTES, "cnx")));
     auto split = [&](int MT, int tiles) {
         int d = 1;
         for (int c = 1; c <= MT; ++c)
             if (MT % c == 0 && (long)tiles * c <= ctx->ncu) d = c;
         return d;
     };
-    {
-        a.A6 = reinterpret_cast<const uint4*>(w.c2.A6);
-        a.wsc = w.c2.wscale;
-        a.bias = w.c2.bias;
-        a.MT = w.c2.MT6;
-        a.dw_w = w.dw_w;
-        a.dw_b = w.dw_b;
-        a.ln_g = w.ln_g;
-        a.ln_b = w.ln_b;
-        a.dil = w.dilation;
-        const int nt = Tl <= 32 ? 1 : 2, tx = (Tl + 32 * nt - 1) / (32 * nt);
-        a.gp = gx;
-        a.gp_tiles = tx;
-        const int d = split(a.MT, tx * NB);
-        a.mt_per_wg = a.MT / d;
-        const dim3 grid((unsigned)tx, (unsigned)NB, (unsigned)d);
-        constexpr int nthr = Cnx1<C, 2>::NTHR, lds1 = Cnx1<C, 1>::LDS_BYTES, lds2 = Cnx1<C, 2>::LDS_BYTES;
-        if (nt == 1) hipLaunchKernelGGL((cnx1_kernel<C, 1>), grid, dim3(nthr), lds1, s, a);
-        else hipLaunchKernelGGL((cnx1_kernel<C, 2>), grid, dim3(nthr), lds2, s, a);
-    }
-    a.gp_sum = a.gp_tiles > CNX_GP_INLINE;
-    if (a.gp_sum) hipLaunchKernelGGL(grn_tiles_kernel, dim3((2 * C + 255) / 256, (unsigned)NB), dim3(256), 0, s, gx, a.gp_tiles, 2 * C, T, a.rg);
-    {
-        a.A6 = reinterpret_cast<const uint4*>(w.c3.A6);
-        a.wsc = w.c3.wscale;
-        a.bias = w.c3_bias_grn;
-        a.MT = w.c3.MT6;
-        a.grn_g = w.grn_g;
-        a.amax_y = amax_out;
-        const int tx = (Tl + 63) / 64;
-        const int d = split(a.MT, tx * NB);
-        a.mt_per_wg = a.MT / d;
-        constexpr int nthr = Cnx2<C, KP>::NTHR, lds = Cnx2<C, KP>::LDS_BYTES;
-        hipLaunchKernelGGL((cnx2_kernel<C, KP>), dim3((unsigned)tx, (unsigned)NB, (unsigned)d), dim3(nthr), lds, s, a);
-    }
-    *rc = launch_check(ctx, "convnext (fused)");
-    return true;
-}
-
-int run_convnext(tvc_ctx* ctx, hipStream_t s, Ws& ws, const ConvNeXtW& w, float* x, int B, int T, float* amax_out) {
+    const int nt = kind == CNX_FIRST && Tl <= 32 ? 1 : 2, tx = (Tl + 32 * nt - 1) / (32 * nt);
+    CnxMat& m = kind == CNX_SECOND ? a.c3 : a.c2;
+    const int d = kind == CNX_BOUNDARY ? 1 : split(m.MT, tx * NB);
+    m.mt_per_wg = m.MT / d;
+    const dim3 grid((unsigned)tx, (unsigned)NB, (unsigned)d);
+    constexpr int nthr1 = Cnx1<C, 2>::NTHR, lds11 = Cnx1<C, 1>::LDS_BYTES, lds12 = Cnx1<C, 2>::LDS_BYTES;
+    constexpr int nthr2 = Cnx2<C, KP>::NTHR, lds2 = Cnx2<C, KP>::LDS_BYTES, nthrf = Cnxf<C, KP>::NTHR, ldsf = Cnxf<C, KP>::LDS_BYTES;
+    if (kind == CNX_FIRST) {
+        if (nt == 1) hipLaunchKernelGGL((cnx1_kernel<C, 1>), grid, dim3(nthr1), lds11, s, a);
+        else hipLaunchKernelGGL((cnx1_kernel<C, 2>), grid, dim3(nthr1), lds12, s, a);
+    } else if (kind == CNX_SECOND) {
+        if (a.xo == a.xi) hipLaunchKernelGGL((cnx2_kernel<C, KP, false>), grid, dim3(nthr2), lds2, s, a);
+        else hipLaunchKernelGGL((cnx2_kernel<C, KP, true>), grid, dim3(nthr2), lds2, s, a);
+    } else {
+        hipLaunchKernelGGL((cnxf_kernel<C, KP>), grid, dim3(nthrf), ldsf, s, a);
+    }
+    return 0;
+}
+
+static int convnext_five_launches(tvc_ctx* ctx, hipStream_t s, const ConvNeXtW& w, float* x, float* y, float* h, float* gx, float* nx, float* ymax, float* hmax,
+                                  int B, int T, float* amax_out) {
     const int C = w.C, C2 = 2 * w.C, ncols = B * T;
     const int NB = ctx->rag ? ctx->rag->B : B;
-    size_t mk = ws.mark();
-    float* y = ws.get<float>((size_t)B * C * T);
-    float* h = ws.get<float>((size_t)B * C2 * T);
-    const int Tlong = ctx->rag ? ctx->rag->Tlong : T;
-    float* gx = ws.get<float>((size_t)NB * C2 * ((Tlong + 63) / 64));
-    float* nx = ws.get<float>((size_t)NB * C2);
-    float* ymax = ws.get<float>((size_t)NB);
-    float* hmax = ws.get<float>((size_t)NB);
-    ws.release(mk);
-    if (ws.dry) return 0;
-    {
-        int rc = 0;
-        if (C == 384 ? cnx_try<384>(&rc, ctx, s, w, x, h, gx, B, T, amax_out) : (C == 128 && cnx_try<128>(&rc, ctx, s, w, x, h, gx, B, T, amax_out))) return rc;
-    }
     {
         TVC_CHECK(dwconv_ln_launch<true>(ctx, s, x, y, w.dw_w, w.dw_b, w.ln_g, w.ln_b, B, C, T, w.dilation));
     }
@@ -284,6 +276,74 @@
     }
     if (amax_out) TVC_CHECK(run_amax_rows(ctx, s, x, B, C, T, amax_out));
     return launch_check(ctx, "convnext");
+}
+
+int run_convnext_chain(tvc_ctx* ctx, hipStream_t s, Ws& ws, const ConvNeXtW* layers, int n, float* x, int B, int T, float* amax_out) {
+    const int C = layers[0].C, C2 = 2 * C;
+    const int NB = ctx->rag ? ctx->rag->B : B;
+    const int Tl = ctx->rag ? ctx->rag->Tlong : T;
+    const int gtiles = (Tl + 63) / 64;
+    size_t mk = ws.mark();
+    float* y = ws.get<float>((size_t)B * C * T);
+    float* h[2] = {ws.get<float>((size_t)B * C2 * T), ws.get<float>((size_t)B * C2 * T)};
+    float* gx[2] = {ws.get<float>((size_t)NB * C2 * gtiles), ws.get<float>((size_t)NB * C2 * gtiles)};
+    float* nx = ws.get<float>((size_t)NB * C2);
+    float* ymax = ws.get<float>((size_t)NB);
+    float* hmax = ws.get<float>((size_t)NB);
+    ws.release(mk);
+    if (ws.dry) return 0;
+    auto ok = [&](int i) { return C == 384 ? cnx_ok<384>(layers[i], T) : (C == 128 && cnx_ok<128>(layers[i], T)); };
+    auto launch = [&](CnxKind kind, const CnxArgs& a) { return C == 384 ? cnx_launch<384>(ctx, s, kind, a, NB, Tl) : cnx_launch<128>(ctx, s, kind, a, NB, Tl); };
+    CnxArgs base{};
+    base.T = T;
+    base.rs = T;
+    base.gp_tiles = gtiles;
+    base.gp_sum = gtiles > CNX_GP_INLINE;
+    float* cur = x;
+    int p = 0;
+    bool first_done = false;
+    for (int i = 0; i < n; ++i) {
+        const ConvNeXtW& w = layers[i];
+        if (w.C != C) return fail(ctx, TVC_ERR_STATE, "convnext chain: layers of different widths");
+        if (!ok(i)) {
+            TVC_CHECK(convnext_five_launches(ctx, s, w, x, y, h[0], gx[0], nx, ymax, hmax, B, T, i == n - 1 ? amax_out : nullptr));
+            continue;
+        }
+        CnxArgs a = base;
+        TVC_CHECK(rag_view(ctx, s, 1, 0, &a.rg, nullptr));
+        if (!first_done) {
+            cnx_set_c2(a, w);
+            a.xi = cur;
+            a.ho = h[p];
+            a.gpo = gx[p];
+            TVC_CHECK(launch(CNX_FIRST, a));
+        }
+        if (a.gp_sum) hipLaunchKernelGGL(grn_tiles_kernel, dim3((C2 + 255) / 256, (unsigned)NB), dim3(256), 0, s, gx[p], gtiles, C2, T, a.rg);
+        cnx_set_c3(a, w);
+        a.xi = cur;
+        a.hi = h[p];
+        a.gpi = gx[p];
+        bool fuse = ctx->cnx_fuse && i + 1 < n && ok(i + 1);
+        if (fuse && ctx->cnx_fuse == 1) fuse = Tl > 32 && 2L * gtiles * NB > ctx->ncu;
+        if (fuse) fuse = ctx->rag ? cnx_fuse_fits(ctx->rag->tb.data(), NB, layers[i + 1].dilation) : cnx_fuse_fits(&T, 1, layers[i + 1].dilation);
+        if (fuse) {
+            cnx_set_c2(a, layers[i + 1]);
+            a.xo = cur == x ? y : x;
+            a.ho = h[p ^ 1];
+            a.gpo = gx[p ^ 1];
+            TVC_CHECK(launch(CNX_BOUNDARY, a));
+            cur = a.xo;
+            p ^= 1;
+        } else {
+            a.xo = x;
+            a.amax_y = i == n - 1 ? amax_out : nullptr;
+            TVC_CHECK(launch(CNX_SECOND, a));
+            cur = x;
+        }
+        first_done = fuse;
+        TVC_CHECK(launch_check(ctx, "convnext (cnx)"));
+    }
+    return 0;
 }
 
 struct EpiSplit {
@@ -395,13 +455,13 @@
         TVC_CHECK(run_layernorm(ctx, s, xp, ctx->pit_ln_g, ctx->pit_ln_b, B, kPitchCh, T));
     }
     const int gtiles = ((ctx->rag ? ctx->rag->Tlong : T) + 63) / 64;
-    const size_t ssl_scratch = ((size_t)B * kSslCh * T * 3 + (size_t)NB * kSslCh * 2 * (gtiles + 1)) * sizeof(float) + (size_t)NB * 8 + 4096;
+    const size_t ssl_scratch = ((size_t)B * kSslCh * T * 5 + (size_t)NB * kSslCh * 2 * (2 * gtiles + 1)) * sizeof(float) + (size_t)NB * 8 + 4096;
     char* ssl_blk = ws.get<char>(ssl_scratch);
     Ws wssl(ssl_blk, ssl_scratch, ws.dry);
     SideFork fk(ctx, s);
     TVC_CHECK(fk.fork(ws, ctx->ev_fork, ctx->ev_join));
     const hipStream_t sp = fk.side;
-    for (int i = 0; i < 4; ++i) TVC_CHECK(run_convnext(ctx, sp, ws, ctx->pit_mid[i], xp, B, T, i == 3 ? xp_max : nullptr));
+    TVC_CHECK(run_convnext_chain(ctx, sp, ws, &ctx->pit_mid[0], 4, xp, B, T, xp_max));
     if (!ws.dry) {
         EpiBias<ACT_NONE, false> ep{lg, ctx->pit_out.bias, nullptr, kPitchClasses, T, ncols, (long)kPitchClasses * T, 0};
         int rc = 0;
@@ -411,7 +471,7 @@
                            shifts && ctx->rag ? ctx->rag->d_col2b : (const int*)nullptr);
     }
     TVC_CHECK(fk.end());
-    for (int i = 0; i < 6; ++i) TVC_CHECK(run_convnext(ctx, s, wssl, ctx->ssl_mid[i], xs, B, T, i == 5 ? xs_max : nullptr));
+    TVC_CHECK(run_convnext_chain(ctx, s, wssl, &ctx->ssl_mid[0], 6, xs, B, T, xs_max));
     if (wssl.peak > wssl.cap) return fail(ctx, TVC_ERR_WORKSPACE, "encoder: SSL scratch block too small");
     if (ws.dry) return 0;
     {
diff --git a/tinyvc_amd/csrc/tvc_common.h b/tinyvc_amd/csrc/tvc_common.h
--- a/tinyvc_amd/csrc/tvc_common.h
+++ b/tinyvc_amd/csrc/tvc_common.h
@@ -129,6 +129,7 @@
     hipEvent_t ev_fork2 = nullptr, ev_join2 = nullptr, ev_amps = nullptr;
     tvc::RagHost* rag = nullptr;
     int rag_batch_frames = 0;
+    int cnx_fuse = 1;
     int index_assign_chunk = 0;
     bool enc_ready = false, dec_ready = false;
     char enc_missing[160] = {0}, dec_missing[160] = {0};
@@ -411,6 +412,7 @@
                     const float* bsh, const float* cond, float* out, int B, int len, int da, int db, const float* amax_x, const float* amax_c,
                     float* amax_y);
 
-int run_convnext(tvc_ctx*, hipStream_t, Ws&, const ConvNeXtW& w, float* x, int B, int T, float* amax_out = nullptr);
+int run_convnext_chain(tvc_ctx*, hipStream_t, Ws&, const ConvNeXtW* layers, int n, float* x, int B, int T, float* amax_out = nullptr);
+bool cnx_fuse_fits(const int* frames, int n, int dil);
 
 }
diff --git a/tinyvc_amd/engine.py b/tinyvc_amd/engine.py
--- a/tinyvc_amd/engine.py
+++ b/tinyvc_amd/engine.py
@@ -138,6 +138,9 @@
 
     def set_ragged_batch_frames(self, max_frames):
         self._ok(self.lib.tvc_ctx_set_ragged_batch_frames(self.ctx, int(max_frames)), "tvc_ctx_set_ragged_batch_frames")
+
+    def set_cnx_fuse(self, on, small_calls=False):
+        self._ok(self.lib.tvc_ctx_set_cnx_fuse(self.ctx, (2 if small_calls else 1) if on else 0), "tvc_ctx_set_cnx_fuse")
 
     def set_index_assign_chunk(self, max_queries):
         self._ok(self.lib.tvc_ctx_set_index_assign_chunk(self.ctx, int(max_queries)), "tvc_ctx_set_index_assign_chunk")
```

Result: no change. 731.1 million, median of 5 (+0.4%).
